# adamjorr/kbbq-py

Measured on AMD Instinct MI355X. Metric: bases/sec recalibrated (2x150 bp), higher is better.
Workload: dtype u8

## Files before the change

include/kbbq_hip.h:

```cpp
#ifndef KBBQ_HIP_H
#define KBBQ_HIP_H

#include <stddef.h>
#include <stdint.h>

#ifdef __cplusplus
extern "C" {
#endif

#define KBBQ_OK          0
#define KBBQ_E_HIP      -1
#define KBBQ_E_INDEX    -2
#define KBBQ_E_TYPE     -3
#define KBBQ_E_ARG      -4
#define KBBQ_E_RANGE    -5
#define KBBQ_E_NAME     -6
#define KBBQ_E_LUT      -7
#define KBBQ_E_MEANQ    -8
#define KBBQ_E_FULL     -9

#define KBBQ_APPLY_CHECKED 0
#define KBBQ_APPLY_FAST    1

#define KBBQ_NQ         43
// ... 131 lines not shown
                           uint8_t* d_flagplane, int R, int minscore, int dinuc_minscore, int64_t* d_tables);
int kbbq_count_q_dev(kbbq_ctx* ctx, const uint8_t* d_qual, const uint8_t* d_err, const uint8_t* d_skip,
                     const uint32_t* d_len, int64_t nreads, int pitch, int qoffset, int64_t* d_counts512);
#define KBBQ_CONFUSION_MAX_BASES 4294967295ull
int kbbq_flag_confusion_dev(kbbq_ctx* ctx, const uint8_t* d_qual, const uint8_t* d_truth, const uint8_t* d_kflags,
                            const uint32_t* d_len, int64_t nreads, int pitch, int qoffset, int64_t* d_counts1536);

int    kbbq_pair_pitch(int S2);
size_t kbbq_pair_lut_bytes(int R, int Qt, int S2);
int    kbbq_pack_pairs_dev(kbbq_ctx* ctx, const uint8_t* d_seq, const uint8_t* d_cseq, const uint8_t* d_qual,
                           const uint32_t* d_meta, int64_t npairs, int pitch, int S2,
                           uint8_t* d_pseq, uint8_t* d_pcseq, uint8_t* d_pqual, uint32_t* d_pmeta);
int    kbbq_unpack_pairs_dev(kbbq_ctx* ctx, const uint8_t* d_pplane, int64_t npairs, int S2, int pitch, uint8_t* d_plane);
int    kbbq_accumulate_pairs_dev(kbbq_ctx* ctx, const uint8_t* d_pseq, const uint8_t* d_pcseq, const uint8_t* d_pqual,
                                 const uint32_t* d_pmeta, int64_t npairs, int R, int S2, int minscore,
                                 int dinuc_minscore, int64_t* d_tables);
int    kbbq_pair_lut_dev(kbbq_ctx* ctx, const void* d_lut_blob, int R, int S2, int minscore, void* d_pair_lut);
int    kbbq_pair_lut_rows_dev(kbbq_ctx* ctx, const void* d_lut_blob, int R, int S2, int minscore, int flags, void* d_pair_lut);
int    kbbq_apply_pairs_dev(kbbq_ctx* ctx, const uint8_t* d_pseq, const uint8_t* d_pqual, const uint32_t* d_pmeta,
                            int64_t npairs, int R, int S2, int minscore, const void* d_lut_blob,
                            const void* d_pair_lut, uint8_t* d_pout);

int    kbbq_accumulate_grouped_dev(kbbq_ctx* ctx, const uint8_t* d_seq, const uint8_t* d_cseq, const uint8_t* d_qual,
                                   const uint32_t* d_meta, int64_t nrows, int pitch, int pairs, int R, int S2,
                                   int S_band, int S_min, int minscore, int dinuc_minscore, const int64_t* d_seg,
                                   int64_t* d_tables);
int    kbbq_apply_grouped_dev(kbbq_ctx* ctx, const uint8_t* d_seq, const uint8_t* d_qual, const uint32_t* d_meta,
                              int64_t nrows, int pitch, int pairs, int R, int S2, int minscore,
                              const void* d_lut_blob, const void* d_pair_lut, const int64_t* d_seg, uint8_t* d_out);

#define KBBQ_ROWS_PAIRS    1
#define KBBQ_ROWS_NIBBLES  2
#define KBBQ_ROWS_TWINS    4
int    kbbq_accumulate_rows_dev(kbbq_ctx* ctx, const uint8_t* d_seq, const uint8_t* d_cseq, const uint8_t* d_qual,
                                const uint32_t* d_meta, int64_t nrows, int pitch, int flags, int R, int S2, int S_band,
                                int S_min, int minscore, int dinuc_minscore, const int64_t* d_seg, int64_t* d_tables);
int    kbbq_apply_rows_dev(kbbq_ctx* ctx, const uint8_t* d_seq, const uint8_t* d_qual, const uint32_t* d_meta, int64_t nrows,
                           int pitch, int flags, int R, int S2, int minscore, const void* d_lut_blob, const void* d_pair_lut,
                           const int64_t* d_seg, const int64_t* d_perm, uint8_t* d_out);
int    kbbq_meta_stats_dev(kbbq_ctx* ctx, const uint32_t* d_meta, int64_t nreads, int32_t* h_stats8);
typedef struct kbbq_band {
    const uint8_t* d_seq; const uint8_t* d_cseq; const uint8_t* d_qual; const uint32_t* d_meta;
    int64_t nrows; int32_t pitch; int32_t flags;
    int32_t S_band; int32_t S_min;
    const int64_t* d_seg; const int64_t* d_perm;
    uint8_t* d_out; const void* d_pair_lut;
} kbbq_band;
int    kbbq_accumulate_bands_dev(kbbq_ctx* ctx, const kbbq_band* bands, int nbands, int R, int S2, int minscore,
                                 int dinuc_minscore, int64_t* d_tables);
int    kbbq_apply_bands_dev(kbbq_ctx* ctx, const kbbq_band* bands, int nbands, int R, int S2, int minscore, const void* d_lut_blob);
size_t kbbq_group_rows_work_bytes(int64_t nrows, int R);
int    kbbq_group_rows_dev(kbbq_ctx* ctx, const uint32_t* d_meta, int64_t nrows, int pairs, int R, void* d_work,
                           int64_t* d_perm, int64_t* d_seg);
int    kbbq_lay_out_dev(kbbq_ctx* ctx, const uint8_t* d_seq, const uint8_t* d_cseq, const uint8_t* d_qual,
                        const uint32_t* d_meta, int64_t nreads, int pitch, int flags, int S2, const int64_t* d_perm,
                        uint8_t* d_lseq, uint8_t* d_lcseq, uint8_t* d_lqual, uint32_t* d_lmeta);
int    kbbq_unpack_nibbles_dev(kbbq_ctx* ctx, const uint8_t* d_nib, int64_t nbases, uint8_t* d_chars);
int    kbbq_tables_add_dev(kbbq_ctx* ctx, int64_t* d_dst, const int64_t* d_src, size_t n);

#define KBBQ_COMM_ID_BYTES 128
typedef struct kbbq_comm kbbq_comm;
int kbbq_comm_library(const char* path);
int kbbq_comm_unique_id(void* id128);
int kbbq_comm_create(kbbq_ctx* ctx, const void* id128, int nranks, int rank, kbbq_comm** out);
int kbbq_allreduce_tables(kbbq_comm* comm, int64_t* d_buf, size_t n);
int kbbq_comm_destroy(kbbq_comm* comm);
// ... 200 lines not shown
```

kbbq-py_amd/csrc/fastq_host.cpp:

```cpp
#include "../../include/kbbq_hip.h"
#include "host_threads.h"
#include "bam_host.h"
#include "fastq_host.h"

#include <algorithm>
#include <atomic>
#include <mutex>
#include <cstdio>
#include <cstdlib>
#include <cstring>
#include <string>
#include <thread>
#include <unordered_map>
#include <vector>

#include <fcntl.h>
#include <sys/mman.h>
#include <sys/stat.h>
#include <unistd.h>
#include <zlib.h>
#if defined(__x86_64__)
#include <immintrin.h>
#endif

// ... 645 lines not shown
    const unsigned nt = nthreads_for((size_t)nrows * 64);
    const int64_t per = (nrows + nt - 1) / std::max(nt, 1u);
    std::vector<std::vector<int64_t>> cnt(nt, std::vector<int64_t>((size_t)R, 0));
    std::atomic<int> bad(0);
    auto key = [&](int64_t i) { return (int)((meta[pairs ? 2 * i : i] >> 16) & 0x7FFFu); };
    auto over = [&](auto body) {
        kbbq_parallel(nt, [&](unsigned t) {
            const int64_t lo = std::min<int64_t>(nrows, (int64_t)t * per), hi = std::min<int64_t>(nrows, lo + per);
            body(t, lo, hi);
        });
    };
    over([&](unsigned t, int64_t lo, int64_t hi) {
        auto& c = cnt[t];
        for (int64_t i = lo; i < hi; ++i) { const int k = key(i); if (k >= R) { bad = 1; continue; } ++c[(size_t)k]; }
    });
    if (bad.load()) return kbbq_set_error_(KBBQ_E_RANGE, "kbbq_group_rows_host: a row carries a read group >= R");
    int64_t run = 0;
    for (int g = 0; g < R; ++g) {
        seg[g] = run;
        for (unsigned t = 0; t < nt; ++t) { const int64_t c = cnt[t][(size_t)g]; cnt[t][(size_t)g] = run; run += c; }
    }
    seg[R] = nrows;
    over([&](unsigned t, int64_t lo, int64_t hi) {
        auto& c = cnt[t];
        for (int64_t i = lo; i < hi; ++i) perm[c[(size_t)key(i)]++] = i;
    });
    return KBBQ_OK;
}

int kbbq_fastq_fill_rows(const kbbq_fastq* a, const kbbq_fastq* b, int64_t first, int64_t n, const uint32_t* meta, int flags,
                         int S2, int pitch, const int64_t* perm, int64_t row_lo, int64_t nrows,
                         uint8_t* seq, uint8_t* cseq, uint8_t* qual, uint32_t* dmeta, int* foreign)
{
    if (!a || (nrows > 0 && (!seq || !qual || !dmeta || !meta || (b && !cseq)))) return kbbq_set_error_(KBBQ_E_ARG, "kbbq_fastq_fill_rows: NULL argument");
    if (first < 0 || n < 0 || first + n > (int64_t)a->h0.size() || (b && first + n > (int64_t)b->h0.size()))
        return kbbq_set_error_(KBBQ_E_ARG, "kbbq_fastq_fill_rows: range out of bounds");
    if (flags & ~(KBBQ_ROWS_PAIRS | KBBQ_ROWS_NIBBLES | KBBQ_ROWS_TWINS)) return kbbq_set_error_(KBBQ_E_ARG, "kbbq_fastq_fill_rows: unknown layout flags");
    const bool pairs = (flags & KBBQ_ROWS_PAIRS) != 0, nib = (flags & KBBQ_ROWS_NIBBLES) != 0;
    const int S = S2 / 2;
    if (pairs) {
        if (S2 <= 0 || (S2 & 1) || S2 > 65534) return kbbq_set_error_(KBBQ_E_ARG, "kbbq_fastq_fill_rows: S2 must be positive and even");
        pitch = (S2 + 1 + 15) & ~15;
    }
    if (pitch <= 0 || (pitch & 15)) return kbbq_set_error_(KBBQ_E_ARG, "kbbq_fastq_fill_rows: pitch must be a positive multiple of 16");
    const int64_t total = pairs ? (n + 1) / 2 : n;
    if (row_lo < 0 || nrows < 0 || row_lo + nrows > total) return kbbq_set_error_(KBBQ_E_ARG, "kbbq_fastq_fill_rows: rows out of bounds");
    const size_t sp = nib ? (size_t)pitch / 2 : (size_t)pitch;
    std::atomic<int> bad(0); std::atomic<unsigned> odd(0);
    parallel_for(nrows, nthreads_for((size_t)nrows * (size_t)pitch * 3), [&](int64_t lo, int64_t hi) {
        std::vector<uint8_t> tmp(nib ? (size_t)pitch : 0);
        unsigned foreign_here = 0;
        for (int64_t row = lo; row < hi; ++row) {
            const int64_t s = perm ? perm[row_lo + row] : row_lo + row;
            if (s < 0 || s >= total) { bad = 3; continue; }
            uint8_t* q = qual + (size_t)row * pitch;
            uint8_t* planes[2] = {seq + (size_t)row * sp, b ? cseq + (size_t)row * sp : nullptr};
            const kbbq_fastq* src[2] = {a, b};
            if (pairs) {
                const int64_t i1 = first + 2 * s; const bool lone = 2 * s + 1 >= n; const int64_t i2 = lone ? i1 : i1 + 1;
                if ((int)a->slen[i1] != S || (int)a->slen[i2] != S || (b && ((int)b->slen[i1] != S || (int)b->slen[i2] != S))) { bad = 1; continue; }
                memcpy(q, a->buf + a->q0[i1], (size_t)S);
                if (lone) memset(q + S, 0, (size_t)(pitch - S));
                else { q[S] = 0; memcpy(q + S + 1, a->buf + a->q0[i2], (size_t)S); memset(q + 2 * S + 1, 0, (size_t)(pitch - 2 * S - 1)); }
                for (int pl = 0; pl < 2; ++pl) {
                    if (!planes[pl]) continue;
                    uint8_t* c = nib ? tmp.data() : planes[pl];
                    memcpy(c, src[pl]->buf + src[pl]->s0[i1], (size_t)S);
                    if (lone) memset(c + S, 'N', (size_t)(pitch - S));
                    else { c[S] = 'N'; memcpy(c + S + 1, src[pl]->buf + src[pl]->s0[i2], (size_t)S); memset(c + 2 * S + 1, 'N', (size_t)(pitch - 2 * S - 1)); }
                    if (nib) foreign_here |= pack_row(c, pitch, planes[pl]);
                }
                dmeta[row] = (uint32_t)(2 * S + 1) | (meta[2 * s] & 0x7FFF0000u);
            } else {
                const int64_t i = first + s;
                const uint32_t L = a->slen[i];
                if ((int)L > pitch || (b && b->slen[i] != L)) { bad = 1; continue; }
                memcpy(q, a->buf + a->q0[i], L); memset(q + L, 0, (size_t)pitch - L);
                for (int pl = 0; pl < 2; ++pl) {
                    if (!planes[pl]) continue;
                    uint8_t* c = nib ? tmp.data() : planes[pl];
                    memcpy(c, src[pl]->buf + src[pl]->s0[i], L); memset(c + L, 'N', (size_t)pitch - L);
                    if (nib) foreign_here |= pack_row(c, pitch, planes[pl]);
                }
                dmeta[row] = meta[s];
            }
        }
        if (foreign_here) odd = 1;
    });
    if (bad.load()) return kbbq_set_error_(KBBQ_E_ARG, bad.load() == 3 ? "kbbq_fastq_fill_rows: perm holds a row out of range"
                                                      : "kbbq_fastq_fill_rows: a read does not fit the layout (lengths differ from what the statistics said)");
    if (odd.load() && foreign) *foreign = 1;
    return KBBQ_OK;
}

int64_t kbbq_fastq_format(const kbbq_fastq* a, int64_t first, int64_t n, int pitch, const uint8_t* newqual,
                          char* out, int64_t cap)
{
    return kbbq_fastq_format_rows(a, first, n, 0, 0, pitch, newqual, out, cap);
}

int64_t kbbq_fastq_format_rows(const kbbq_fastq* a, int64_t first, int64_t n, int flags, int S2, int pitch,
                               const uint8_t* newqual, char* out, int64_t cap)
{
    if (!a || first < 0 || n < 0 || first + n > (int64_t)a->h0.size()) { kbbq_set_error_(KBBQ_E_ARG, "kbbq_fastq_format: bad range"); return 0; }
// ... 27 lines not shown
```

kbbq-py_amd/csrc/kbbq_hip.hip:

```cpp
#include "kbbq_kernels.h"
#include "kbbq_kernels_v3.h"
#include "kbbq_k2_tile.h"
#include "kbbq_solve_kernels.h"
#include "kbbq_lut_kernels.h"
#include "kbbq_aligned_kernels.h"
#include "kbbq_layout_kernels.h"
#include "kbbq_apply_aligned.h"
#include "kbbq_kmer.h"
#include "kbbq_kmer_set.h"
#include "kbbq_bgzf.h"
#include "kbbq_bam_out.h"
#include "../../include/kbbq_hip.h"
#include "host_threads.h"

#include <rocprim/rocprim.hpp>

#include <algorithm>
#include <climits>
#include <cstdint>
#include <cstdarg>
#include <cstdio>
#include <cstring>
#include <functional>
#include <string>
// ... 32 lines not shown
    hipStream_t own_stream = nullptr;
    hipStream_t stream = nullptr;
    u64* d_status = nullptr;
    int* d_stats = nullptr;
    DevScratch wgplan;
    DevScratch ops4;
    DevScratch tally;
    DevScratch rowlut;
    DevScratch bgzf_tok;
    DevScratch bgzf_off;
    DevScratch bgzf_blocks;
    DevScratch bam_words;
    void* stage_host[2] = {nullptr, nullptr}; void* stage_dev[2] = {nullptr, nullptr}; size_t stage_bytes = 0;
    hipStream_t stage_stream = nullptr;
    hipStream_t stage_down_stream = nullptr;
    hipEvent_t stage_up[2] = {nullptr, nullptr}, stage_used[2] = {nullptr, nullptr}, stage_down[2] = {nullptr, nullptr};
    bool timing = false;
    std::vector<std::pair<hipEvent_t, hipEvent_t>> ev[2];
    double ms_acc[2] = {0.0, 0.0};
    int64_t launches[2] = {0, 0};
};

#define KBBQ_NSTATUS 8

constexpr size_t K2T_ROW_LUT_MAX = 52 << 10;
constexpr int K2V3_FRONTS = 8;
constexpr int K2T_XCD_TILES = 1;
constexpr int K2T_XCD = 8;
constexpr int K7_FRONTS = 8;
constexpr int TALLY_K4_SHARE = 8;
static const u64 ST_INIT[KBBQ_NSTATUS] = {~0ull, ~0ull, ~0ull, ~0ull, ~0ull, ~0ull, ~0ull, ~0ull};

enum K1Form { K1_ROWS, K1_ALIGNED, K1_ALIGNED_REF, K1_BANDS };
struct K1Variant { K1Form form; int dn, nib, kj; const void* kernel[2]; };
#define K1_SPLITS(K, ...) {(const void*)(K<false, __VA_ARGS__>), (const void*)(K<true, __VA_ARGS__>)}
static const K1Variant K1_VARIANTS[] = {
    {K1_ROWS, K1V3_DNREP, 0, 0, K1_SPLITS(k1v3_accumulate, K1V3_DNREP)},
    {K1_ROWS, 8, 0, 0, K1_SPLITS(k1v3_accumulate, 8)},
    {K1_ROWS, K1V3_DNREP, 1, 0, K1_SPLITS(k1v3_accumulate, K1V3_DNREP, true)},
    {K1_ROWS, 8, 1, 0, K1_SPLITS(k1v3_accumulate, 8, true)},
    {K1_ROWS, K1V3_DNREP, 1, 13, K1_SPLITS(k1v3_accumulate, K1V3_DNREP, true, 13)},
    {K1_ROWS, K1V3_DNREP, 1, 19, K1_SPLITS(k1v3_accumulate, K1V3_DNREP, true, 19)},
    {K1_ALIGNED, K1V3_DNREP, 0, 0, K1_SPLITS(k1v3_aligned, K1V3_DNREP)},
    {K1_ALIGNED, 8, 0, 0, K1_SPLITS(k1v3_aligned, 8)},
    {K1_ALIGNED_REF, K1V3_DNREP, 0, 0, K1_SPLITS(k1v3_aligned_ref, K1V3_DNREP)},
    {K1_ALIGNED_REF, 8, 0, 0, K1_SPLITS(k1v3_aligned_ref, 8)},
    {K1_BANDS, 0, 0, 0, K1_SPLITS(k1v3_bands, false)},
    {K1_BANDS, 0, 1, 0, K1_SPLITS(k1v3_bands, true)},
};
#undef K1_SPLITS

static const void* k1_kernel(K1Form form, bool split, int dn, int nib, int kj)
{
    for (const K1Variant& v : K1_VARIANTS)
        if (v.form == form && v.dn == dn && v.nib == nib && v.kj == kj) return v.kernel[split];
    return nullptr;
}

enum LdsKernel { LK_K1_PLAIN, LK_K1_PLAIN_SPLIT, LK_K1_TILED, LK_K1_TILED_SPLIT, LK_K2V3, LK_K2V3_NIB, LK_K2T, LK_K2T_NIB, LK_K2T_BANDS, LK_K2T_PAIR19, LK_K2T_PAIR13, LK_K2_LDS16, LK_K2_LDS8, LK_BGZF, LK_COUNT };
static const void* const LDS_KERNELS[LK_COUNT] = {
    (const void*)k1_accumulate<false>, (const void*)k1_accumulate<true>,
    (const void*)k1_accumulate_tiled<false>, (const void*)k1_accumulate_tiled<true>,
    (const void*)k2v3_apply<false>, (const void*)k2v3_apply<true>,
    (const void*)k2t_apply<false>, (const void*)k2t_apply<true>, (const void*)k2t_bands,
    (const void*)k2t_apply_pair<19>, (const void*)k2t_apply_pair<13>,
    (const void*)k2_apply<int16_t, true, true>, (const void*)k2_apply<int8_t, true, false>,
    (const void*)bz_deflate,
};

extern "C" {

int kbbq_abi_version(void) { return KBBQ_ABI_VERSION; }
const char* kbbq_last_error(void) { return g_err.c_str(); }

int kbbq_device_count(int* count)
{
    int n = 0;
    hipError_t e = hipGetDeviceCount(&n);
    if (e != hipSuccess) { *count = 0; return fail(KBBQ_E_HIP, "hipGetDeviceCount: %s", hipGetErrorString(e)); }
    *count = n;
    return KBBQ_OK;
}

int kbbq_bind_host_to_device(int device, int* numa_node, int* ncpus)
{
    char busid[64] = {0};
    HIPCHK(hipDeviceGetPCIBusId(busid, (int)sizeof busid, device));
    return kbbq_bind_host_to_pci(busid, numa_node, ncpus);
}

int kbbq_ctx_create(int device, kbbq_ctx** out)
{
    if (!out) return fail(KBBQ_E_ARG, "kbbq_ctx_create: out is NULL");
    *out = nullptr;
    const bool dbg = getenv("KBBQ_CTX_DBG") != nullptr;
    auto t_prev = std::chrono::steady_clock::now();
    auto lap = [&](const char* what) {
        if (!dbg) return;
// ... 297 lines not shown
};

static int launch_lds(kbbq_ctx* c, int which, const void* kernel, dim3 grid, dim3 block, size_t lds, const void* params)
{
    if (!kernel) return fail(KBBQ_E_HIP, "libkbbq_hip has no instance of K1 for this launch (K1_VARIANTS)");
    void* args[] = {const_cast<void*>(params)};
    {
        Timed t(c, which);
        (void)hipLaunchKernel(kernel, grid, block, args, lds, c->stream);
    }
    HIPCHK(hipGetLastError());
    return KBBQ_OK;
}

static int grow_scratch(kbbq_ctx* c, DevScratch& s, size_t need)
{
    if (s.bytes >= need) return KBBQ_OK;
    if (s.p) { HIPCHK(hipStreamSynchronize(c->stream)); (void)hipFree(s.p); s.p = nullptr; s.bytes = 0; }
    HIPCHK(hipMalloc(&s.p, need));
    s.bytes = need;
    return KBBQ_OK;
}

extern "C" {

int kbbq_accumulate_dev(kbbq_ctx* c, const uint8_t* d_seq, const uint8_t* d_cseq,
                        const uint8_t* d_qual, const uint32_t* d_meta,
                        int64_t nreads, int pitch, int R, int S2, int minscore, int64_t* d_tables)
{
    return kbbq_accumulate_ex_dev(c, d_seq, d_cseq, d_qual, d_meta, nreads, pitch, R, S2,
                                  minscore, minscore, d_tables);
}

struct K1Setup { K1v3Params q; int dn = 0; int kj = 0; size_t lds = 0; };
static int accumulate_rows(kbbq_ctx* c, const char* who, const uint8_t* d_seq, const uint8_t* d_cseq, const uint8_t* d_qual,
                           const uint32_t* d_meta, int64_t nrows, int pitch, int pairs, int R, int S2, int minscore,
                           int dinuc_minscore, const int64_t* d_seg, int64_t* d_tables, bool* fits, int S_band = 0, int S_min = 0, int nib = 0,
                           int twins = 0, K1Setup* setup_only = nullptr);

int kbbq_accumulate_ex_dev(kbbq_ctx* c, const uint8_t* d_seq, const uint8_t* d_cseq,
                           const uint8_t* d_qual, const uint32_t* d_meta,
                           int64_t nreads, int pitch, int R, int S2, int minscore,
                           int dinuc_minscore, int64_t* d_tables)
{
    return kbbq_accumulate_band_dev(c, d_seq, d_cseq, d_qual, d_meta, nreads, pitch, R, S2, 0, 0, minscore, dinuc_minscore, d_tables);
}

int kbbq_accumulate_band_dev(kbbq_ctx* c, const uint8_t* d_seq, const uint8_t* d_cseq,
                             const uint8_t* d_qual, const uint32_t* d_meta,
                             int64_t nreads, int pitch, int R, int S2, int S_band, int S_min, int minscore,
                             int dinuc_minscore, int64_t* d_tables)
{
    if (!c) return fail(KBBQ_E_ARG, "ctx is NULL");
    int rc = check_planes("kbbq_accumulate_dev", nreads, pitch, d_seq, d_cseq, d_qual);
    if (rc) return rc;
    if (R <= 0 || R > 32767) return fail(KBBQ_E_ARG, "kbbq_accumulate_dev: R out of range (%d)", R);
    if (S2 <= 0 || (S2 & 1)) return fail(KBBQ_E_ARG, "kbbq_accumulate_dev: S2 must be positive and even (%d)", S2);
    if (minscore < 0 || minscore > KQ - 1) return fail(KBBQ_E_ARG, "kbbq_accumulate_dev: minscore out of range (%d)", minscore);
    if (dinuc_minscore < 0 || dinuc_minscore > 222) return fail(KBBQ_E_ARG, "kbbq_accumulate_dev: dinuc_minscore out of range (%d)", dinuc_minscore);
    if (nreads == 0) return KBBQ_OK;
    HIPCHK(hipSetDevice(c->device));

    const int64_t nblocks = (nreads + 63) / 64;
    const bool split = dinuc_minscore > minscore;
    bool fits = false;
    rc = accumulate_rows(c, "kbbq_accumulate_dev", d_seq, d_cseq, d_qual, d_meta, nreads, pitch, 0, R, S2, minscore,
                         dinuc_minscore, nullptr, d_tables, &fits, S_band, S_min);
    if (rc || fits) return rc;
    K1Params p;
    p.seq = d_seq; p.cseq = d_cseq; p.qual = d_qual; p.meta = d_meta;
    p.nreads = nreads; p.pitch = pitch; p.cpr = pitch / 16; p.cpr_magic = magic_for(p.cpr);
// ... 120 lines not shown
    return true;
}

static bool k2_tile_serves(const kbbq_ctx* c, int pairs, int nib, int R, bool grouped, int cpr, size_t rg_bytes)
{
    if (env_is("KBBQ_K2_TILE", "0") || (!nib && env_is("KBBQ_K2_TILE_CHARS", "0"))) return false;
    if ((R != 1 && !grouped) || cpr < 2 || cpr > 4096) return false;
    return pairs ? rg_bytes * 3 <= (size_t)c->lds_bytes : rg_bytes <= K2T_ROW_LUT_MAX;
}

static K2v3Params k2v3_params(kbbq_ctx* c, const uint8_t* d_seq, const uint8_t* d_qual, const uint32_t* d_meta, int64_t nrows, int pitch,
                              int pairs, int R, int Qt, int S2, int Sb, int minscore, const void* d_lut_blob, const void* d_pair_lut,
                              const int64_t* d_seg, const int64_t* d_perm, uint8_t* d_out)
{
    K2v3Params q;
    q.seq = d_seq; q.qual = d_qual; q.meta = d_meta; q.nreads = nrows; q.pitch = pitch;
    q.cpr = pitch / 16; q.cpr_magic = magic_for(q.cpr);
    q.R = R; q.Qt = Qt; q.S2 = S2; q.minscore = minscore; q.qlo = 33u + (u32)minscore;
    q.lut16 = reinterpret_cast<const int16_t*>(d_lut_blob); q.rs16 = lut_row_stride(S2);
    q.full = pairs ? reinterpret_cast<const int8_t*>(d_pair_lut)
                   : reinterpret_cast<const int8_t*>(d_lut_blob) + lut_full_offset(R, Qt, S2);
    q.rb = (u32)(pairs ? pair_lut_row_bytes(S2) : full_lut_row_bytes(Sb));
    q.full_bytes = (int)((size_t)R * (33 + Qt) * q.rb);
    if (pairs) { q.W = 0u; q.ctx_off = (u32)pair_pitch(S2); q.maxlen = S2 + 1; }
    else { q.W = (u32)full_lut_width(Sb); q.ctx_off = 2u * q.W; q.maxlen = Sb; }
    q.pairs = pairs; q.seg = reinterpret_cast<const long long*>(d_seg);
    q.perm = reinterpret_cast<const long long*>(d_perm);
    q.parts = K2V3_FRONTS;
    q.rpb = 64;
    q.out = d_out; q.status = c->d_status;
    return q;
}

static int launch_k2v3(kbbq_ctx* c, const K2v3Params& q, int nib)
{
    const int slices = q.seg ? q.R : 1;
    const size_t lds = (size_t)(33 + q.Qt) * q.rb * (size_t)(q.seg ? 1 : q.R);
    const int per_cu = std::max(1, std::min<int>((int)(c->lds_bytes / lds), (K2V3_WAVES * 4 * 64) / K2V3_THREADS));
    const int64_t nblocks = (q.nreads + q.rpb - 1) / q.rpb;
    const int64_t want = (nblocks + (K2V3_THREADS / 64) - 1) / (K2V3_THREADS / 64);
    const int gx = (int)std::min<int64_t>(want, std::max<int64_t>(1, (int64_t)c->cus * per_cu / slices));
    return launch_lds(c, 1, LDS_KERNELS[nib ? LK_K2V3_NIB : LK_K2V3], dim3((unsigned)std::max(gx, 1), (unsigned)slices, 1), dim3(K2V3_THREADS), lds, &q);
}

static int apply_rows(kbbq_ctx* c, const char* who, const uint8_t* d_seq, const uint8_t* d_qual, const uint32_t* d_meta,
                      int64_t nrows, int pitch, int pairs, int R, int S2, int minscore, const void* d_lut_blob,
                      const void* d_pair_lut, const int64_t* d_seg, uint8_t* d_out, int nib = 0, const int64_t* d_perm = nullptr);

int kbbq_apply_dev(kbbq_ctx* c, const uint8_t* d_seq, const uint8_t* d_qual, const uint32_t* d_meta,
                   int64_t nreads, int pitch, int R, int Qt, int S2, int minscore,
                   const void* d_lut, int mode, uint8_t* d_out)
{
    if (!c) return fail(KBBQ_E_ARG, "ctx is NULL");
    int rc = check_planes("kbbq_apply_dev", nreads, pitch, d_seq, d_qual, d_out);
    if (rc) return rc;
    if (R <= 0 || R > 32767 || Qt <= 0 || Qt > 95 || S2 <= 0 || S2 > 65536)
        return fail(KBBQ_E_ARG, "kbbq_apply_dev: bad table shape R=%d Qt=%d S2=%d (Qt <= 95)", R, Qt, S2);
    if (minscore < 0 || minscore > 222) return fail(KBBQ_E_ARG, "kbbq_apply_dev: minscore out of range");
    if ((uintptr_t)d_lut & 15) return fail(KBBQ_E_ARG, "kbbq_apply_dev: LUT must be 16-byte aligned");
    if (mode != KBBQ_APPLY_CHECKED && mode != KBBQ_APPLY_FAST) return fail(KBBQ_E_ARG, "kbbq_apply_dev: bad mode %d", mode);
    if (nreads == 0) return KBBQ_OK;
    HIPCHK(hipSetDevice(c->device));
    const int64_t nblocks = (nreads + 63) / 64;

    const int Sb = row_lut_width(pitch, S2);
    const size_t full_bytes = (size_t)R * (33 + Qt) * full_lut_row_bytes(Sb);
    if (mode == KBBQ_APPLY_FAST && R == 1 && Qt == KQ && !(S2 & 1) && S2 <= 65534
        && k2_tile_serves(c, 0, 0, R, false, pitch / 16, (size_t)(33 + KQ) * full_lut_row_bytes(Sb)))
        return apply_rows(c, "kbbq_apply_dev", d_seq, d_qual, d_meta, nreads, pitch, 0, R, S2, minscore, d_lut, nullptr, nullptr, d_out, 0, nullptr);
    if (mode == KBBQ_APPLY_FAST && full_bytes <= (size_t)c->lds_bytes) {
        K2v3Params q = k2v3_params(c, d_seq, d_qual, d_meta, nreads, pitch, 0, R, Qt, S2, Sb, minscore, d_lut, nullptr, nullptr, nullptr, d_out);
        if (!narrowed_row_lut(c, d_lut, R, Qt, S2, Sb, minscore, &q.full)) return fail(KBBQ_E_HIP, "kbbq_apply_dev: no scratch for the narrowed LUT");
        return launch_k2v3(c, q, 0);
    }

    K2Params p;
    p.seq = d_seq; p.qual = d_qual; p.meta = d_meta; p.nreads = nreads; p.pitch = pitch;
    p.cpr = pitch / 16; p.cpr_magic = magic_for(p.cpr);
    p.R = R; p.Qt = Qt; p.S2 = S2; p.minscore = minscore; p.qlo = 33u + (u32)minscore;
    p.lut = reinterpret_cast<const int16_t*>(d_lut); p.lut_count = (int)kbbq_lut_count(R, Qt, S2);
// ... 230 lines not shown
    auto bytes_for = [&](int nt, int pc) {
        const size_t rows = (size_t)q.nrows - 1 + nt;
        return rows * 128 * dn + (size_t)pc * (rows * q.row_bytes + q.slack_bytes);
    };
    const char* nt_env = getenv("KBBQ_K1_NTRASH");
    const char* pc_env = getenv("KBBQ_K1_POSCOPIES");
    const int most_t = nt_env ? atoi(nt_env) : 8, most = pc_env ? atoi(pc_env) : 4;
    q.ntrash = 1; q.pos_copies = 1;
    for (int nt = 8; nt >= 2; nt >>= 1)
        if (nt <= most_t && bytes_for(nt, 1) <= (size_t)c->lds_bytes) { q.ntrash = nt; break; }
    if (q.cpr <= 12)
        for (int pc = 4; pc >= 2; pc >>= 1)
            if (pc <= most && bytes_for(q.ntrash, pc) <= (size_t)c->lds_bytes) { q.pos_copies = pc; break; }
    q.pos_copy_bytes = (u32)((size_t)(q.nrows - 1 + q.ntrash) * q.row_bytes + q.slack_bytes);
    return bytes_for(q.ntrash, q.pos_copies);
}

static bool k1_geometry(K1v3Params& q, const kbbq_ctx* c, int copies, int cut, int minlen)
{
    q.row_bytes = (u32)((3 * q.S - cut) | 1) * 4u;
    q.minlen = minlen;
    q.slack_bytes = (u32)(q.S + 32) * 4u;
    q.dn_flush_iters = std::max(1, 65535 / ((K1V3_THREADS / copies) * 16 * q.cpr));
    const size_t lds = (size_t)q.nrows * 128 * copies + (size_t)q.nrows * q.row_bytes + q.slack_bytes;
    return lds <= (size_t)c->lds_bytes && (K1V3_THREADS / copies) * 16 * q.cpr <= 65535;
}

static bool k1_split(const K1v3Params& q) { return q.type_minscore > q.minscore; }
static int64_t k1_iters(const K1v3Params& q) { return ((q.nreads + 63) / 64 + (K1V3_THREADS / 64) - 1) / (K1V3_THREADS / 64); }

static int launch_k1(kbbq_ctx* c, K1Form form, const K1Setup& su, int nib)
{
    const int gx = (int)std::min<int64_t>(k1_iters(su.q), std::max(1, c->cus / su.q.R));
    return launch_lds(c, 0, k1_kernel(form, k1_split(su.q), su.dn, nib, su.kj), dim3((unsigned)gx, (unsigned)su.q.R, 1), dim3(K1V3_THREADS),
                      su.lds, &su.q);
}

static int accumulate_rows(kbbq_ctx* c, const char* who, const uint8_t* d_seq, const uint8_t* d_cseq, const uint8_t* d_qual,
                           const uint32_t* d_meta, int64_t nrows, int pitch, int pairs, int R, int S2, int minscore,
                           int dinuc_minscore, const int64_t* d_seg, int64_t* d_tables, bool* fits, int S_band, int S_min, int nib, int twins,
                           K1Setup* setup_only)
{
    if (fits) *fits = true;
    if (S_band < 0 || S_band > S2 / 2 || (pairs && S_band)) return fail(KBBQ_E_ARG, "%s: S_band out of range (%d)", who, S_band);
    if (S_min < 0 || S_min > (S_band ? S_band : S2 / 2)) return fail(KBBQ_E_ARG, "%s: S_min out of range (%d)", who, S_min);
    int rc = check_planes(who, nrows, pitch, d_seq, d_cseq, d_qual);
    if (rc) return rc;
    if (R <= 0 || R > 32767) return fail(KBBQ_E_ARG, "%s: R out of range (%d)", who, R);
    if (S2 <= 0 || (S2 & 1) || S2 > 65534) return fail(KBBQ_E_ARG, "%s: S2 must be positive and even (%d)", who, S2);
    if (minscore < 0 || minscore > KQ - 1) return fail(KBBQ_E_ARG, "%s: minscore out of range (%d)", who, minscore);
    if (dinuc_minscore < 0 || dinuc_minscore > 222) return fail(KBBQ_E_ARG, "%s: dinuc_minscore out of range (%d)", who, dinuc_minscore);
    if (pairs && pitch != pair_pitch(S2)) return fail(KBBQ_E_ARG, "%s: mate-pair rows of %d-base reads have pitch %d, not %d", who, S2 / 2, pair_pitch(S2), pitch);
    if (nrows == 0) return KBBQ_OK;
    HIPCHK(hipSetDevice(c->device));
    const int S = S_band ? S_band : S2 / 2;
    K1Setup su;
    K1v3Params& q = su.q;
    q.aflags = nullptr; q.aclip = nullptr; q.atrim = nullptr;
    q.seq = d_seq; q.cseq = d_cseq; q.qual = d_qual; q.meta = d_meta;
    q.nreads = nrows; q.pitch = pitch; q.cpr = pitch / 16; q.cpr_magic = magic_for(q.cpr);
    q.R = R; q.S = S; q.gS2 = S2; q.minscore = minscore; q.type_minscore = dinuc_minscore;
    q.qlo_m1 = 32u + (u32)minscore; q.dlo = 33u + (u32)dinuc_minscore;
    q.nrows = KQ + 1 - minscore;
    q.maxlen = pairs ? S2 + 1 : S; q.gap = pairs ? 1 : 0; q.twins = (pairs && twins) ? 1 : 0;
    q.seg = reinterpret_cast<const long long*>(d_seg);
    q.tables = reinterpret_cast<u64*>(d_tables); q.status = c->d_status;
    q.genome = nullptr; q.ag0 = nullptr;
    const int trim = (!pairs && S_min > 0) ? std::min(S_min, S) : 0;
    if (pairs && nib && (q.cpr == 19 || q.cpr == 13)) {
        q.row_bytes = (u32)((((16 * q.cpr + 31) & ~31) + 32 * K1V3_DNREP) * 4);
        q.minlen = 0; q.slack_bytes = 0; q.pos_copies = 1;
        q.dn_flush_iters = std::max(1, 65535 / ((K1V3_THREADS / K1V3_DNREP) * 16 * q.cpr));
        for (int nt = q.cpr == 19 ? 1 : 8; nt >= 1 && !su.dn; nt >>= 1) {
            const size_t rows = (size_t)q.nrows - 1 + nt;
            su.lds = rows * q.row_bytes;
            if (su.lds > (size_t)c->lds_bytes) continue;
            su.dn = K1V3_DNREP; su.kj = q.cpr;
            q.ntrash = nt; q.pos_copy_bytes = (u32)(rows * q.row_bytes);
        }
    }
    for (int attempt = 0; attempt < (trim ? 3 : 1) && !su.dn; ++attempt) {
        const int copies = attempt == 2 ? 8 : K1V3_DNREP, cut = attempt ? trim : 0;
        if (k1_geometry(q, c, copies, cut, cut)) su.dn = copies;
    }
    if (!su.dn) {
        if (fits) { *fits = false; return KBBQ_OK; }
        return fail(KBBQ_E_LUT, "%s: %d-base reads with minscore %d do not fit the LDS tables; use plain one-read-per-row planes", who, S, minscore);
    }
    if (!su.kj) su.lds = k1_lds_plan(q, su.dn, c);
    if (setup_only) { *setup_only = su; return KBBQ_OK; }
    return launch_k1(c, K1_ROWS, su, nib);
}

int kbbq_accumulate_pairs_dev(kbbq_ctx* c, const uint8_t* d_pseq, const uint8_t* d_pcseq, const uint8_t* d_pqual,
                              const uint32_t* d_pmeta, int64_t npairs, int R, int S2, int minscore,
                              int dinuc_minscore, int64_t* d_tables)
{
    if (!c) return fail(KBBQ_E_ARG, "ctx is NULL");
    int rc = check_pairs("kbbq_accumulate_pairs_dev", npairs, S2);
    if (rc) return rc;
    return accumulate_rows(c, "kbbq_accumulate_pairs_dev", d_pseq, d_pcseq, d_pqual, d_pmeta, npairs, pair_pitch(S2), 1,
                           R, S2, minscore, dinuc_minscore, nullptr, d_tables, nullptr);
}

int kbbq_accumulate_grouped_dev(kbbq_ctx* c, const uint8_t* d_seq, const uint8_t* d_cseq, const uint8_t* d_qual,
                                const uint32_t* d_meta, int64_t nrows, int pitch, int pairs, int R, int S2, int S_band,
                                int S_min, int minscore, int dinuc_minscore, const int64_t* d_seg, int64_t* d_tables)
{
    if (!c) return fail(KBBQ_E_ARG, "ctx is NULL");
    if (!d_seg) return fail(KBBQ_E_ARG, "kbbq_accumulate_grouped_dev: d_seg is NULL");
    return accumulate_rows(c, "kbbq_accumulate_grouped_dev", d_seq, d_cseq, d_qual, d_meta, nrows, pitch, pairs ? 1 : 0,
                           R, S2, minscore, dinuc_minscore, d_seg, d_tables, nullptr, S_band, S_min);
}

int kbbq_pair_lut_dev(kbbq_ctx* c, const void* d_lut_blob, int R, int S2, int minscore, void* d_pair_lut)
{
    return kbbq_pair_lut_rows_dev(c, d_lut_blob, R, S2, minscore, KBBQ_ROWS_PAIRS, d_pair_lut);
}

int kbbq_pair_lut_rows_dev(kbbq_ctx* c, const void* d_lut_blob, int R, int S2, int minscore, int flags, void* d_pair_lut)
{
    if (!c) return fail(KBBQ_E_ARG, "ctx is NULL");
    int rc = check_pairs("kbbq_pair_lut_dev", 0, S2);
    if (rc) return rc;
    if (!(flags & KBBQ_ROWS_PAIRS) || (flags & ~(KBBQ_ROWS_PAIRS | KBBQ_ROWS_NIBBLES | KBBQ_ROWS_TWINS)))
        return fail(KBBQ_E_ARG, "kbbq_pair_lut_rows_dev: flags 0x%x are not those of mate-pair rows", flags);
    if (R <= 0 || R > 32767 || !d_lut_blob || !d_pair_lut) return fail(KBBQ_E_ARG, "kbbq_pair_lut_dev: bad argument");
    HIPCHK(hipSetDevice(c->device));
    PairLutParams f;
    f.lut16 = reinterpret_cast<const int16_t*>(d_lut_blob); f.rs16 = lut_row_stride(S2); f.R = R; f.Qt = KQ; f.S2 = S2;
    f.minscore = std::min(std::max(minscore, 0), KQ);
    f.twins = (flags & KBBQ_ROWS_TWINS) ? 1 : 0;
    f.out = reinterpret_cast<int8_t*>(d_pair_lut);
    hipLaunchKernelGGL(k3_fill_pair_lut, dim3((unsigned)(R * (33 + KQ))), dim3(256), 0, c->stream, f);
    HIPCHK(hipGetLastError());
    return KBBQ_OK;
}

static K2tParams k2t_params(const K2v3Params& q)
{
    K2tParams t;
    t.seq = q.seq; t.qual = q.qual; t.meta = q.meta; t.nchunks = q.nreads * q.cpr; t.cpr = q.cpr; t.cpr_magic = q.cpr_magic;
    t.Qt = q.Qt; t.S2 = q.S2; t.maxlen = q.maxlen; t.lut = q.full; t.lut_bytes = (int)(((size_t)(33 + q.Qt) * q.rb + 15) & ~(size_t)15);
    t.rb = q.rb; t.ctx_off = q.ctx_off; t.W = q.W; t.seg = q.seg; t.R = q.R; t.wg_start = nullptr; t.order = nullptr;
    t.perm = q.perm; t.pitch = q.pitch; t.out = q.out; t.status = q.status;
    t.xcd_tiles = K2T_XCD_TILES;
    return t;
}

static int apply_rows(kbbq_ctx* c, const char* who, const uint8_t* d_seq, const uint8_t* d_qual, const uint32_t* d_meta,
                      int64_t nrows, int pitch, int pairs, int R, int S2, int minscore, const void* d_lut_blob,
                      const void* d_pair_lut, const int64_t* d_seg, uint8_t* d_out, int nib, const int64_t* d_perm)
{
    int rc = check_planes(who, nrows, pitch, d_seq, d_qual, d_out);
    if (rc) return rc;
    if (R <= 0 || R > 32767 || !d_lut_blob || (pairs && (!d_pair_lut || ((uintptr_t)d_pair_lut & 15)))) return fail(KBBQ_E_ARG, "%s: bad argument", who);
    if (S2 <= 0 || (S2 & 1) || S2 > 65534) return fail(KBBQ_E_ARG, "%s: S2 must be positive and even (%d)", who, S2);
    if (minscore < 0 || minscore > 222) return fail(KBBQ_E_ARG, "%s: minscore out of range", who);
    if (pairs && pitch != pair_pitch(S2)) return fail(KBBQ_E_ARG, "%s: mate-pair rows of %d-base reads have pitch %d, not %d", who, S2 / 2, pair_pitch(S2), pitch);
    const int Sb = pairs ? S2 : row_lut_width(pitch, S2);
    K2v3Params q = k2v3_params(c, d_seq, d_qual, d_meta, nrows, pitch, pairs, R, KQ, S2, Sb, minscore, d_lut_blob, d_pair_lut, d_seg, d_perm, d_out);
    const size_t rg_bytes = (size_t)(33 + KQ) * q.rb;
    const size_t lds = d_seg ? rg_bytes : rg_bytes * (size_t)R;
    if (lds > (size_t)c->lds_bytes)
        return fail(KBBQ_E_LUT, "%s: the apply LUT (%zu B) does not fit the LDS; group the rows by read group or use kbbq_apply_dev", who, lds);
    if (nrows == 0) return KBBQ_OK;
    HIPCHK(hipSetDevice(c->device));
    if (!pairs && !narrowed_row_lut(c, d_lut_blob, R, KQ, S2, Sb, minscore, &q.full)) return fail(KBBQ_E_HIP, "%s: no scratch for the narrowed LUT", who);
    if (!k2_tile_serves(c, pairs, nib, R, d_seg != nullptr, q.cpr, rg_bytes)) return launch_k2v3(c, q, nib);

    K2tParams t = k2t_params(q);
    const int64_t per_wg = (int64_t)(K2T_THREADS / 64) * 64 * K2T_STEPS;
    int64_t gt = (t.nchunks + per_wg - 1) / per_wg;
    if (d_seg) {
        gt += R;
        const bool interleave = d_perm && R > 1;
        const int64_t ints = (int64_t)(R + 1) + 1 + (interleave ? 2 * gt : 0);
        if (ints > 0x7FFFFFFF) return fail(KBBQ_E_ARG, "%s: too many workgroups", who);
        rc = grow_scratch(c, c->wgplan, (size_t)ints * sizeof(int));
        if (rc) return rc;
        int* wg_start = reinterpret_cast<int*>(c->wgplan.p);
        K2tPlanParams pl; pl.seg = t.seg; pl.R = R; pl.cpr = q.cpr; pl.wg_start = wg_start;
        hipLaunchKernelGGL(k2t_plan, dim3(1), dim3(64), 0, c->stream, pl);
        t.wg_start = wg_start;
        if (interleave) {
            K2tOrderParams op; op.wg_start = wg_start; op.R = R;
            op.xcd = K2T_XCD;
            op.order = reinterpret_cast<int2*>(wg_start + ((R + 2) & ~1));
            hipLaunchKernelGGL(k2t_order, dim3((unsigned)((gt + 255) / 256)), dim3(256), 0, c->stream, op);
            t.order = op.order;
        }
    }
    const int kj = (pairs && nib) ? k2t_pair_form(t) : 0;
    if (kj < 0) return fail(KBBQ_E_ARG, "%s: mate-pair rows of %d chunks do not have the geometry k2t_apply_pair was compiled for", who, q.cpr);
    const LdsKernel k = kj == 19 ? LK_K2T_PAIR19 : kj == 13 ? LK_K2T_PAIR13 : nib ? LK_K2T_NIB : LK_K2T;
    return launch_lds(c, 1, LDS_KERNELS[k], dim3((unsigned)gt), dim3(K2T_THREADS), (size_t)t.lut_bytes, &t);
}

int kbbq_apply_pairs_dev(kbbq_ctx* c, const uint8_t* d_pseq, const uint8_t* d_pqual, const uint32_t* d_pmeta,
                         int64_t npairs, int R, int S2, int minscore, const void* d_lut_blob, const void* d_pair_lut,
                         uint8_t* d_pout)
{
    if (!c) return fail(KBBQ_E_ARG, "ctx is NULL");
    int rc = check_pairs("kbbq_apply_pairs_dev", npairs, S2);
    if (rc) return rc;
    return apply_rows(c, "kbbq_apply_pairs_dev", d_pseq, d_pqual, d_pmeta, npairs, pair_pitch(S2), 1, R, S2, minscore,
                      d_lut_blob, d_pair_lut, nullptr, d_pout);
}

int kbbq_apply_grouped_dev(kbbq_ctx* c, const uint8_t* d_seq, const uint8_t* d_qual, const uint32_t* d_meta,
                           int64_t nrows, int pitch, int pairs, int R, int S2, int minscore, const void* d_lut_blob,
                           const void* d_pair_lut, const int64_t* d_seg, uint8_t* d_out)
{
    if (!c) return fail(KBBQ_E_ARG, "ctx is NULL");
    if (!d_seg) return fail(KBBQ_E_ARG, "kbbq_apply_grouped_dev: d_seg is NULL");
    return apply_rows(c, "kbbq_apply_grouped_dev", d_seq, d_qual, d_meta, nrows, pitch, pairs ? 1 : 0, R, S2, minscore,
                      d_lut_blob, d_pair_lut, d_seg, d_out);
}


static int layout_flags_ok(const char* who, int flags)
{
    if (flags & ~(KBBQ_ROWS_PAIRS | KBBQ_ROWS_NIBBLES | KBBQ_ROWS_TWINS)) return fail(KBBQ_E_ARG, "%s: unknown layout flags 0x%x", who, flags);
    if ((flags & KBBQ_ROWS_TWINS) && !(flags & KBBQ_ROWS_PAIRS)) return fail(KBBQ_E_ARG, "%s: KBBQ_ROWS_TWINS describes mate-pair rows (add KBBQ_ROWS_PAIRS)", who);
    return KBBQ_OK;
}

int kbbq_accumulate_rows_dev(kbbq_ctx* c, const uint8_t* d_seq, const uint8_t* d_cseq, const uint8_t* d_qual,
                             const uint32_t* d_meta, int64_t nrows, int pitch, int flags, int R, int S2, int S_band,
                             int S_min, int minscore, int dinuc_minscore, const int64_t* d_seg, int64_t* d_tables)
{
    if (!c) return fail(KBBQ_E_ARG, "ctx is NULL");
    int rc = layout_flags_ok("kbbq_accumulate_rows_dev", flags);
    if (rc) return rc;
    const int pairs = (flags & KBBQ_ROWS_PAIRS) ? 1 : 0;
    if (pairs) { rc = check_pairs("kbbq_accumulate_rows_dev", nrows, S2); if (rc) return rc; }
    return accumulate_rows(c, "kbbq_accumulate_rows_dev", d_seq, d_cseq, d_qual, d_meta, nrows, pitch, pairs, R, S2, minscore,
                           dinuc_minscore, d_seg, d_tables, nullptr, pairs ? 0 : S_band, pairs ? 0 : S_min,
                           (flags & KBBQ_ROWS_NIBBLES) ? 1 : 0, (flags & KBBQ_ROWS_TWINS) ? 1 : 0);
}

int kbbq_apply_rows_dev(kbbq_ctx* c, const uint8_t* d_seq, const uint8_t* d_qual, const uint32_t* d_meta, int64_t nrows,
                        int pitch, int flags, int R, int S2, int minscore, const void* d_lut_blob, const void* d_pair_lut,
                        const int64_t* d_seg, const int64_t* d_perm, uint8_t* d_out)
{
    if (!c) return fail(KBBQ_E_ARG, "ctx is NULL");
    int rc = layout_flags_ok("kbbq_apply_rows_dev", flags);
    if (rc) return rc;
    const int pairs = (flags & KBBQ_ROWS_PAIRS) ? 1 : 0;
    if (pairs) { rc = check_pairs("kbbq_apply_rows_dev", nrows, S2); if (rc) return rc; }
    return apply_rows(c, "kbbq_apply_rows_dev", d_seq, d_qual, d_meta, nrows, pitch, pairs, R, S2, minscore, d_lut_blob,
                      d_pair_lut, d_seg, d_out, (flags & KBBQ_ROWS_NIBBLES) ? 1 : 0, d_perm);
}

static int band_accumulate_alone(kbbq_ctx* c, const kbbq_band& b, int R, int S2, int minscore, int dinuc_minscore, int64_t* d_tables)
{
    if (b.flags || b.d_seg)
        return kbbq_accumulate_rows_dev(c, b.d_seq, b.d_cseq, b.d_qual, b.d_meta, b.nrows, b.pitch, b.flags, R, S2, b.S_band, b.S_min,
                                        minscore, dinuc_minscore, b.d_seg, d_tables);
    return kbbq_accumulate_band_dev(c, b.d_seq, b.d_cseq, b.d_qual, b.d_meta, b.nrows, b.pitch, R, S2, b.S_band, b.S_min, minscore,
                                    dinuc_minscore, d_tables);
}

static void share_workgroups(const std::vector<double>& weight, const std::vector<int64_t>& cap, int total, std::vector<int>& out)
{
    const size_t n = weight.size();
    out.assign(n, 1);
    int left = total - (int)n;
    double sum = 0; for (double w : weight) sum += w;
    for (int round = 0; round < 4 && left > 0 && sum > 0; ++round) {
        std::vector<std::pair<double, size_t>> frac;
        int given = 0; double open_sum = 0;
        for (size_t i = 0; i < n; ++i) if (out[i] < cap[i]) open_sum += weight[i];
        if (open_sum <= 0) break;
        const int pool = left;
        for (size_t i = 0; i < n; ++i) {
            if (out[i] >= cap[i]) continue;
            const double want = pool * weight[i] / open_sum;
            int add = (int)std::min<int64_t>((int64_t)want, cap[i] - out[i]);
            out[i] += add; given += add;
            if (out[i] < cap[i]) frac.push_back({want - (int64_t)want, i});
        }
        left -= given;
        std::sort(frac.begin(), frac.end(), [](const auto& a, const auto& b) { return a.first > b.first; });
        for (auto& f : frac) { if (left <= 0) break; if (out[f.second] < cap[f.second]) { ++out[f.second]; --left; } }
    }
}

int kbbq_accumulate_bands_dev(kbbq_ctx* c, const kbbq_band* bands, int nbands, int R, int S2, int minscore, int dinuc_minscore,
                              int64_t* d_tables)
{
    if (!c) return fail(KBBQ_E_ARG, "ctx is NULL");
    if (nbands < 0 || (nbands > 0 && !bands)) return fail(KBBQ_E_ARG, "kbbq_accumulate_bands_dev: bad band list");
    std::vector<K1Setup> setups; std::vector<int> merged, alone;
    const bool merge = !env_is("KBBQ_K1_BANDS", "0");
    int nib_of_merge = -1;
    for (int i = 0; i < nbands; ++i) {
        const kbbq_band& b = bands[i];
        if (b.nrows == 0) continue;
        int rc = layout_flags_ok("kbbq_accumulate_bands_dev", b.flags);
        if (rc) return rc;
        const int pairs = (b.flags & KBBQ_ROWS_PAIRS) ? 1 : 0, nib = (b.flags & KBBQ_ROWS_NIBBLES) ? 1 : 0;
        K1Setup su; bool fits = false;
        bool can = merge && (int)merged.size() < K1V3_MAX_BANDS;
        if (can) {
            if (pairs) { rc = check_pairs("kbbq_accumulate_bands_dev", b.nrows, S2); if (rc) return rc; }
            rc = accumulate_rows(c, "kbbq_accumulate_bands_dev", b.d_seq, b.d_cseq, b.d_qual, b.d_meta, b.nrows, b.pitch, pairs, R, S2, minscore,
                                 dinuc_minscore, b.d_seg, d_tables, &fits, pairs ? 0 : b.S_band, pairs ? 0 : b.S_min, nib,
                                 (b.flags & KBBQ_ROWS_TWINS) ? 1 : 0, &su);
            if (rc) return rc;
            can = fits && !su.kj && (nib_of_merge < 0 || nib_of_merge == nib);
        }
        if (can) { nib_of_merge = nib; merged.push_back(i); setups.push_back(su); }
        else alone.push_back(i);
    }
    const int G = std::max(1, c->cus / std::max(R, 1));
    if (merged.size() < 2 || (int)merged.size() > G) { for (int i : merged) alone.push_back(i); merged.clear(); }
    for (int i : alone) {
        int rc = band_accumulate_alone(c, bands[i], R, S2, minscore, dinuc_minscore, d_tables);
        if (rc) return rc;
    }
    HIPCHK(hipSetDevice(c->device));
    if (merged.empty()) return KBBQ_OK;
    constexpr double row_cost = 1.25;
    constexpr double slope = 0.01;
    constexpr double dn8_cost = 1.06;
    K1BandsParams t;
    memset(&t, 0, sizeof t);
    t.nbands = (int)merged.size();
    std::vector<double> weight; std::vector<int64_t> cap; std::vector<int> share;
    size_t lds = 0;
    for (const K1Setup& su : setups) {
        weight.push_back((double)su.q.nreads * (su.q.cpr + row_cost) * (1.0 + slope * su.q.cpr) * (su.dn == K1V3_DNREP ? 1.0 : dn8_cost));
        cap.push_back(std::max<int64_t>(1, k1_iters(su.q)));
        lds = std::max(lds, su.lds);
    }
    share_workgroups(weight, cap, G, share);
    int run = 0;
    for (size_t j = 0; j < setups.size(); ++j) {
        t.wg_start[j] = run; run += share[j];
        t.dn[j] = setups[j].dn; t.band[j] = setups[j].q;
    }
// ... 9 lines not shown
        HIPCHK(hipMemcpy(h.data(), dbg, h.size() * sizeof h[0], hipMemcpyDeviceToHost));
        (void)hipFree(dbg);
        unsigned long long t0 = ~0ull;
        for (int w = 0; w < run; ++w) t0 = std::min(t0, h[(size_t)w]);
        for (int j = 0; j < t.nbands; ++j) {
            unsigned long long s1 = 0, e0 = ~0ull, e1 = 0;
            for (int w = t.wg_start[j]; w < t.wg_start[j + 1]; ++w) {
                s1 = std::max(s1, h[(size_t)w] - t0); e0 = std::min(e0, h[(size_t)run + w] - t0); e1 = std::max(e1, h[(size_t)run + w] - t0);
            }
            fprintf(stderr, "[k1v3_bands] band %d pitch %3d rows %9lld: %3d workgroups, last start %7.1f us, ends %7.1f .. %7.1f us\n", j, t.band[j].pitch,
                    (long long)t.band[j].nreads, t.wg_start[j + 1] - t.wg_start[j], s1 / 100.0, e0 / 100.0, e1 / 100.0);
        }
    }
    return KBBQ_OK;
}

static int band_apply_alone(kbbq_ctx* c, const kbbq_band& b, int R, int S2, int minscore, const void* d_lut_blob)
{
    if (b.flags || b.d_seg)
        return kbbq_apply_rows_dev(c, b.d_seq, b.d_qual, b.d_meta, b.nrows, b.pitch, b.flags, R, S2, minscore, d_lut_blob, b.d_pair_lut,
                                   b.d_seg, b.d_perm, b.d_out);
    return kbbq_apply_dev(c, b.d_seq, b.d_qual, b.d_meta, b.nrows, b.pitch, R, KQ, S2, minscore, d_lut_blob, KBBQ_APPLY_FAST, b.d_out);
}

int kbbq_apply_bands_dev(kbbq_ctx* c, const kbbq_band* bands, int nbands, int R, int S2, int minscore, const void* d_lut_blob)
{
    if (!c) return fail(KBBQ_E_ARG, "ctx is NULL");
    if (nbands < 0 || (nbands > 0 && !bands) || !d_lut_blob) return fail(KBBQ_E_ARG, "kbbq_apply_bands_dev: bad argument");
    if (R <= 0 || R > 32767 || S2 <= 0 || (S2 & 1) || S2 > 65534 || minscore < 0 || minscore > 222) return fail(KBBQ_E_ARG, "kbbq_apply_bands_dev: bad shape");
    std::vector<int> merged, alone;
    for (int i = 0; i < nbands; ++i) {
        const kbbq_band& b = bands[i];
        if (b.nrows == 0) continue;
        int rc = layout_flags_ok("kbbq_apply_bands_dev", b.flags);
        if (rc) return rc;
        const int Sb = std::min(b.pitch, S2);
        const bool can = (int)merged.size() < K2T_MAX_BANDS && R == 1
                         && b.flags == KBBQ_ROWS_NIBBLES && !b.d_seg && !b.d_perm && b.pitch > 0 && !(b.pitch & 15)
                         && k2_tile_serves(c, 0, 1, R, false, b.pitch / 16, (size_t)(33 + KQ) * full_lut_row_bytes(Sb))
                         && !(((uintptr_t)b.d_seq | (uintptr_t)b.d_qual | (uintptr_t)b.d_out) & 15) && b.d_seq && b.d_qual && b.d_meta && b.d_out;
        (can ? merged : alone).push_back(i);
    }
    if (merged.size() < 2) { for (int i : merged) alone.push_back(i); merged.clear(); }
    for (int i : alone) {
        int rc = band_apply_alone(c, bands[i], R, S2, minscore, d_lut_blob);
        if (rc) return rc;
    }
    if (merged.empty()) return KBBQ_OK;
    HIPCHK(hipSetDevice(c->device));
    std::vector<size_t> lut_off; size_t need = 0;
    for (int i : merged) { lut_off.push_back(need); need += ((size_t)R * (33 + KQ) * full_lut_row_bytes(std::min(bands[i].pitch, S2)) + 255) & ~(size_t)255; }
    int rc = grow_scratch(c, c->rowlut, need);
    if (rc) return rc;
    K2tBandsParams t;
    memset(&t, 0, sizeof t);
    t.nbands = (int)merged.size();
    const int64_t per_wg = (int64_t)(K2T_THREADS / 64) * 64 * K2T_STEPS;
    int64_t run = 0; size_t lds = 0;
    for (size_t k = 0; k < merged.size(); ++k) {
        const kbbq_band& b = bands[merged[k]];
        const int Sb = std::min(b.pitch, S2);
        K2v3Params rows = k2v3_params(c, b.d_seq, b.d_qual, b.d_meta, b.nrows, b.pitch, 0, R, KQ, S2, Sb, minscore, d_lut_blob, nullptr, nullptr, nullptr, b.d_out);
        rows.full = fill_row_lut(c, d_lut_blob, R, KQ, S2, Sb, minscore, reinterpret_cast<char*>(c->rowlut.p) + lut_off[k]);
        const K2tParams& q = t.band[k] = k2t_params(rows);
        lds = std::max(lds, (size_t)q.lut_bytes);
        t.wg_start[k] = (int)run;
        run += (q.nchunks + per_wg - 1) / per_wg;
// ... 26 lines not shown
size_t kbbq_group_rows_work_bytes(int64_t nrows, int R)
{
    const int64_t nblocks = (nrows + K7_SORT_ROWS - 1) / K7_SORT_ROWS;
    return (size_t)std::max<int64_t>(nblocks, 1) * (size_t)std::max(R, 1) * sizeof(u32);
}

int kbbq_group_rows_dev(kbbq_ctx* c, const uint32_t* d_meta, int64_t nrows, int pairs, int R, void* d_work,
                        int64_t* d_perm, int64_t* d_seg)
{
    if (!c) return fail(KBBQ_E_ARG, "ctx is NULL");
    if (nrows < 0 || nrows >= (1ll << 32)) return fail(KBBQ_E_ARG, "kbbq_group_rows_dev: nrows out of range");
    if (R <= 0 || R > K7_SORT_MAXR) return fail(KBBQ_E_ARG, "kbbq_group_rows_dev: 1 <= R <= %d (got %d)", K7_SORT_MAXR, R);
    if (!d_meta || !d_work || !d_perm || !d_seg) return fail(KBBQ_E_ARG, "kbbq_group_rows_dev: NULL pointer");
    HIPCHK(hipSetDevice(c->device));
    if (nrows == 0) { HIPCHK(hipMemsetAsync(d_seg, 0, (size_t)(R + 1) * 8, c->stream)); return KBBQ_OK; }
    RgSortParams p;
    p.meta = d_meta; p.nrows = nrows; p.pairs = pairs ? 1 : 0; p.R = R;
    p.nblocks = (nrows + K7_SORT_ROWS - 1) / K7_SORT_ROWS;
    p.hist = reinterpret_cast<u32*>(d_work); p.perm = reinterpret_cast<long long*>(d_perm); p.status = c->d_status;
    hipLaunchKernelGGL(k7_rg_sort<false>, dim3((unsigned)p.nblocks), dim3(K7_SORT_THREADS), 0, c->stream, p);
    RgScanParams s;
    s.hist = p.hist; s.count = p.nblocks * R; s.nblocks = p.nblocks; s.R = R; s.nrows = nrows; s.seg = reinterpret_cast<long long*>(d_seg);
    hipLaunchKernelGGL(k7_rg_scan, dim3(1), dim3(1024), 0, c->stream, s);
    hipLaunchKernelGGL(k7_rg_sort<true>, dim3((unsigned)p.nblocks), dim3(K7_SORT_THREADS), 0, c->stream, p);
    HIPCHK(hipGetLastError());
    return KBBQ_OK;
}

int kbbq_lay_out_dev(kbbq_ctx* c, const uint8_t* d_seq, const uint8_t* d_cseq, const uint8_t* d_qual, const uint32_t* d_meta,
                     int64_t nreads, int pitch, int flags, int S2, const int64_t* d_perm,
                     uint8_t* d_lseq, uint8_t* d_lcseq, uint8_t* d_lqual, uint32_t* d_lmeta)
{
    if (!c) return fail(KBBQ_E_ARG, "ctx is NULL");
    int rc = layout_flags_ok("kbbq_lay_out_dev", flags);
    if (rc) return rc;
    const int pairs = (flags & KBBQ_ROWS_PAIRS) ? 1 : 0, nib = (flags & KBBQ_ROWS_NIBBLES) ? 1 : 0;
    rc = check_planes("kbbq_lay_out_dev", nreads, pitch, d_seq, d_cseq, d_qual);
    if (rc) return rc;
    if (!d_seq || !d_qual || !d_meta || !d_lseq || !d_lqual || !d_lmeta || (d_cseq && !d_lcseq)) return fail(KBBQ_E_ARG, "kbbq_lay_out_dev: NULL pointer");
    if (((uintptr_t)d_lseq | (uintptr_t)d_lcseq | (uintptr_t)d_lqual) & 15) return fail(KBBQ_E_ARG, "kbbq_lay_out_dev: planes must be 16-byte aligned");
    if (pairs) {
        rc = check_pairs("kbbq_lay_out_dev", (nreads + 1) / 2, S2);
        if (rc) return rc;
        if ((nreads & 1) && !(flags & KBBQ_ROWS_TWINS)) return fail(KBBQ_E_ARG, "kbbq_lay_out_dev: mate-pair rows need an even number of reads");
        if (pitch < S2 / 2) return fail(KBBQ_E_ARG, "kbbq_lay_out_dev: pitch %d < read length %d", pitch, S2 / 2);
    }
    if (nreads == 0) return KBBQ_OK;
    HIPCHK(hipSetDevice(c->device));
    LayOutParams p;
    p.src[0] = d_seq; p.src[1] = d_cseq; p.src[2] = d_qual; p.dst[0] = d_lseq; p.dst[1] = d_lcseq; p.dst[2] = d_lqual;
    p.meta = d_meta; p.dmeta = d_lmeta; p.perm = reinterpret_cast<const long long*>(d_perm);
    p.nrows = pairs ? (nreads + 1) / 2 : nreads; p.nsrc = nreads; p.pitch = pitch; p.dpitch = pairs ? pair_pitch(S2) : pitch; p.S = pairs ? S2 / 2 : 0;
    p.pairs = pairs; p.nib = nib; p.status = c->d_status;
    const int rpb7 = (p.dpitch / 16) <= 256 ? 256 / (p.dpitch / 16) : 1;
    const int gx = bounded_grid((p.nrows + rpb7 - 1) / rpb7, c, 256);
    p.parts = K7_FRONTS;
    hipLaunchKernelGGL(k7_lay_out, dim3((unsigned)std::max(gx, 1)), dim3(256), 0, c->stream, p);
    HIPCHK(hipGetLastError());
    return KBBQ_OK;
}

int kbbq_tables_add_dev(kbbq_ctx* c, int64_t* d_dst, const int64_t* d_src, size_t n)
{
    if (!c) return fail(KBBQ_E_ARG, "ctx is NULL");
    if (n && (!d_dst || !d_src)) return fail(KBBQ_E_ARG, "kbbq_tables_add_dev: NULL pointer");
    if (n == 0) return KBBQ_OK;
    HIPCHK(hipSetDevice(c->device));
    AddTablesParams p; p.dst = (long long*)d_dst; p.src = (const long long*)d_src; p.n = (long long)n;
    int gx = (int)std::min<size_t>((n + 255) / 256, (size_t)c->cus * 8);
    hipLaunchKernelGGL(k7_add_tables, dim3((unsigned)std::max(gx, 1)), dim3(256), 0, c->stream, p);
    HIPCHK(hipGetLastError());
    return KBBQ_OK;
}

int kbbq_unpack_nibbles_dev(kbbq_ctx* c, const uint8_t* d_nib, int64_t nbases, uint8_t* d_chars)
{
    if (!c) return fail(KBBQ_E_ARG, "ctx is NULL");
    if (nbases < 0 || (nbases & 15) || ((uintptr_t)d_nib & 7) || ((uintptr_t)d_chars & 15)) return fail(KBBQ_E_ARG, "kbbq_unpack_nibbles_dev: bad size or alignment");
    if (nbases == 0) return KBBQ_OK;
    HIPCHK(hipSetDevice(c->device));
    UnNibParams p; p.src = d_nib; p.dst = d_chars; p.nchunks = nbases / 16;
    int gx = (int)std::min<int64_t>((p.nchunks + 255) / 256, (int64_t)c->cus * 16);
    hipLaunchKernelGGL(k7_unpack_nibbles, dim3((unsigned)std::max(gx, 1)), dim3(256), 0, c->stream, p);
    HIPCHK(hipGetLastError());
    return KBBQ_OK;
}
// ... 39 lines not shown
    const K4Params p = k4_params(c, d_seq, d_len, nreads, pitch, d_ref_start, d_ref_len, d_cig_off, d_cig_n, d_cigar, d_genome, d_skipmask,
                                 genome_len, d_flip, d_err, d_skip);
    if (((uintptr_t)d_seq | (uintptr_t)d_err | (uintptr_t)d_skip) & 15)
        return fail(KBBQ_E_ARG, "kbbq_find_errors_dev: planes must be 16-byte aligned");
    const int rpb4 = (pitch / 16) <= 256 ? 256 / (pitch / 16) : 1;
    const int gx = bounded_grid((nreads + rpb4 - 1) / rpb4, c, 64);
    int rc4 = k4_records(c, p, nullptr, nullptr, nullptr, nullptr, 0);
    if (rc4) return rc4;
    K4v2Params q; q.base = p; q.recs = (const K4Rec*)c->ops4.p; q.idle16 = reinterpret_cast<const uint8_t*>(c->d_status);
    q.rows = nullptr; q.nrows = nullptr;
    if (d_skipmask) hipLaunchKernelGGL(k4v2_find_errors<false>, dim3((unsigned)std::max(gx, 1)), dim3(256), 0, c->stream, q);
    else hipLaunchKernelGGL(k4v2_find_errors<true>, dim3((unsigned)std::max(gx, 1)), dim3(256), 0, c->stream, q);
    HIPCHK(hipGetLastError());
    return KBBQ_OK;
}

int kbbq_canonical_reads_dev(kbbq_ctx* c, const uint8_t* d_seq, const uint8_t* d_oq, const uint8_t* d_err,
                             const uint8_t* d_skip, const uint32_t* d_len, const uint32_t* d_clip,
                             const uint32_t* d_trim, const uint32_t* d_flags, int64_t nreads, int pitch, int S,
                             int minscore, int dinuc_minscore, uint8_t* d_out_seq, uint8_t* d_out_cseq,
                             uint8_t* d_out_qual, uint32_t* d_out_meta)
{
    return kbbq_canonical_reads_rows_dev(c, d_seq, d_oq, d_err, d_skip, d_len, d_clip, d_trim, d_flags, nreads, pitch, S,
                                         minscore, dinuc_minscore, 0, d_out_seq, d_out_cseq, d_out_qual, d_out_meta);
}

int kbbq_canonical_reads_rows_dev(kbbq_ctx* c, const uint8_t* d_seq, const uint8_t* d_oq, const uint8_t* d_err,
                                  const uint8_t* d_skip, const uint32_t* d_len, const uint32_t* d_clip,
                                  const uint32_t* d_trim, const uint32_t* d_flags, int64_t nreads, int pitch, int S,
                                  int minscore, int dinuc_minscore, int layout, uint8_t* d_out_seq, uint8_t* d_out_cseq,
                                  uint8_t* d_out_qual, uint32_t* d_out_meta)
{
    if (!c) return fail(KBBQ_E_ARG, "ctx is NULL");
    if (layout & ~KBBQ_ROWS_NIBBLES) return fail(KBBQ_E_ARG, "kbbq_canonical_reads_rows_dev: the output is one read per row (layout 0 or KBBQ_ROWS_NIBBLES)");
    if (nreads < 0 || pitch <= 0 || (pitch & 15) || S <= 0 || S > pitch || S > 65535)
        return fail(KBBQ_E_ARG, "kbbq_canonical_reads_dev: bad nreads/pitch/S");
    if (minscore < 0 || minscore > 94 || dinuc_minscore < 0 || dinuc_minscore > 94)
        return fail(KBBQ_E_ARG, "kbbq_canonical_reads_dev: minscore out of range");
    if (nreads == 0) return KBBQ_OK;
    if (!d_seq || !d_oq || !d_err) return fail(KBBQ_E_ARG, "kbbq_canonical_reads_dev: NULL plane");
    if (((uintptr_t)d_seq | (uintptr_t)d_oq | (uintptr_t)d_err | (uintptr_t)d_skip | (uintptr_t)d_out_seq
         | (uintptr_t)d_out_cseq | (uintptr_t)d_out_qual) & 15)
        return fail(KBBQ_E_ARG, "kbbq_canonical_reads_dev: planes must be 16-byte aligned");
    HIPCHK(hipSetDevice(c->device));
    K6Params p;
    p.seq = d_seq; p.oq = d_oq; p.err = d_err; p.skip = d_skip; p.len = d_len; p.clip = d_clip; p.trim = d_trim;
    p.flags = d_flags; p.nreads = nreads; p.pitch = pitch; p.S = S;
    p.qlo = 33u + (u32)minscore; p.dlo = 33u + (u32)dinuc_minscore;
    p.out_seq = d_out_seq; p.out_cseq = d_out_cseq; p.out_qual = d_out_qual; p.out_meta = d_out_meta;
    p.status = c->d_status;
    const int rpb6 = (pitch / 16) <= 256 ? 256 / (pitch / 16) : 1;
    const int gx = bounded_grid((nreads + rpb6 - 1) / rpb6, c, 64);
    if (layout & KBBQ_ROWS_NIBBLES) hipLaunchKernelGGL(k6_canonical_reads<true>, dim3((unsigned)std::max(gx, 1)), dim3(256), 0, c->stream, p);
    else hipLaunchKernelGGL(k6_canonical_reads<false>, dim3((unsigned)std::max(gx, 1)), dim3(256), 0, c->stream, p);
    HIPCHK(hipGetLastError());
    return KBBQ_OK;
}

static int accumulate_aligned(kbbq_ctx* c, const uint8_t* d_seq, const uint8_t* d_oq, const uint8_t* d_flagplane,
                              const uint32_t* d_clip, const uint32_t* d_trim, const uint32_t* d_flags, int64_t nreads,
                              int pitch, int S, int R, int minscore, int dinuc_minscore, int64_t* d_tables,
                              const uint8_t* d_genome, const int64_t* d_g0, bool dry_run = false)
{
    if (!c) return fail(KBBQ_E_ARG, "ctx is NULL");
    int rc = check_planes("kbbq_accumulate_aligned_dev", nreads, pitch, d_seq, d_oq, d_flagplane);
    if (rc) return rc;
// ... 1429 lines not shown
```

kbbq-py_amd/csrc/kbbq_k2_tile.h:

```cpp
#pragma once
#include "kbbq_kernels_v3.h"
#include <type_traits>

#define K2T_THREADS 1024
#define K2T_STEPS 4

struct K2tParams {
    const uint8_t* seq; const uint8_t* qual; const u32* meta;
    int xcd_tiles;
    long long nchunks;
    int cpr; u32 cpr_magic;
    int Qt; int S2; int maxlen;
    const int8_t* lut; int lut_bytes; u32 rb; u32 ctx_off;
    u32 W;
    const long long* seg;
    const int* wg_start;
    const int2* order;
    int R;
    const long long* perm;
    int pitch;
    uint8_t* out; u64* status;
};

struct K2tPlanParams { const long long* seg; int R; int cpr; int* wg_start; };
// ... 194 lines not shown
}
static inline int k2t_pair_form(const K2tParams& t)
{
    if (t.cpr == 19) return k2t_pair_geometry<19>(t) ? 19 : -1;
    if (t.cpr == 13) return k2t_pair_geometry<13>(t) ? 13 : -1;
    return 0;
}

template <int B> __device__ __forceinline__ u32 k2t_mul24_byte(u32 w, u32 k)
{
    u32 r;
    if constexpr (B == 0) asm("v_mul_u32_u24_sdwa %0, %1, %2 dst_sel:DWORD dst_unused:UNUSED_PAD src0_sel:BYTE_0 src1_sel:DWORD" : "=v"(r) : "v"(w), "v"(k));
    else if constexpr (B == 1) asm("v_mul_u32_u24_sdwa %0, %1, %2 dst_sel:DWORD dst_unused:UNUSED_PAD src0_sel:BYTE_1 src1_sel:DWORD" : "=v"(r) : "v"(w), "v"(k));
    else if constexpr (B == 2) asm("v_mul_u32_u24_sdwa %0, %1, %2 dst_sel:DWORD dst_unused:UNUSED_PAD src0_sel:BYTE_2 src1_sel:DWORD" : "=v"(r) : "v"(w), "v"(k));
    else asm("v_mul_u32_u24_sdwa %0, %1, %2 dst_sel:DWORD dst_unused:UNUSED_PAD src0_sel:BYTE_3 src1_sel:DWORD" : "=v"(r) : "v"(w), "v"(k));
    return r;
}
template <int B> __device__ __forceinline__ u32 k2t_add_byte(u32 a, u32 w)
{
    u32 r;
    if constexpr (B == 0) asm("v_add_u32_sdwa %0, %1, %2 dst_sel:DWORD dst_unused:UNUSED_PAD src0_sel:DWORD src1_sel:BYTE_0" : "=v"(r) : "v"(a), "v"(w));
    else if constexpr (B == 1) asm("v_add_u32_sdwa %0, %1, %2 dst_sel:DWORD dst_unused:UNUSED_PAD src0_sel:DWORD src1_sel:BYTE_1" : "=v"(r) : "v"(a), "v"(w));
    else if constexpr (B == 2) asm("v_add_u32_sdwa %0, %1, %2 dst_sel:DWORD dst_unused:UNUSED_PAD src0_sel:DWORD src1_sel:BYTE_2" : "=v"(r) : "v"(a), "v"(w));
    else asm("v_add_u32_sdwa %0, %1, %2 dst_sel:DWORD dst_unused:UNUSED_PAD src0_sel:DWORD src1_sel:BYTE_3" : "=v"(r) : "v"(a), "v"(w));
    return r;
}
template <class F> __device__ __forceinline__ void k2t_unroll4(F f)
{
    f(std::integral_constant<int, 0>()); f(std::integral_constant<int, 1>()); f(std::integral_constant<int, 2>()); f(std::integral_constant<int, 3>());
}

typedef unsigned short k2t_u16x2 __attribute__((ext_vector_type(2)));

template <int KJ>
__global__ __launch_bounds__(K2T_THREADS) void k2t_apply_pair(K2tParams p)
{
    extern __shared__ __attribute__((aligned(16))) u32 lds[];
    typedef K2tPair<KJ> G;
    const u32 lane = (u32)lane_id();
    const u32 wave = (u32)__builtin_amdgcn_readfirstlane((int)(threadIdx.x >> 6));
    const int bx = (int)blockIdx.x;
    int g = 0;
    long long row_lo = 0, chunk_hi = p.nchunks;
    u32 wg = (u32)bx, tiles = gridDim.x;
    if (p.seg) {
        if (bx >= p.wg_start[p.R]) return;
        if (p.order) {
            const int2 o = p.order[bx];
            g = o.x; wg = (u32)o.y; tiles = 0u;
        } else {
            int lo = 0, hi = p.R;
            while (hi - lo > 1) { const int mid = (lo + hi) >> 1; if (p.wg_start[mid] <= bx) lo = mid; else hi = mid; }
            g = lo;
            wg = (u32)(bx - p.wg_start[g]);
            tiles = (u32)(p.wg_start[g + 1] - p.wg_start[g]);
        }
        row_lo = p.seg[g]; chunk_hi = p.seg[g + 1] * KJ;
    }
    tiles &= ~7u;
    if (wg < tiles) wg = (wg & 7u) * (tiles >> 3) + (wg >> 3);
    const long long chunk_lo = row_lo * KJ;
    const long long base = chunk_lo + ((long long)wg * (K2T_THREADS / 64) + wave) * (64 * K2T_STEPS);
    const bool has = base < chunk_hi;
    const long long base_c = has ? base : chunk_hi - 1;
    const unsigned long long off0 = (unsigned long long)(base_c - chunk_lo);
    const unsigned long long rowd = off0 / (unsigned)KJ;
    const u32 rem0 = (u32)(off0 - rowd * (unsigned)KJ);
    const long long last = chunk_hi - 1 - base_c;
    const u32 limit = last < 64 * K2T_STEPS - 1 ? (u32)last : (u32)(64 * K2T_STEPS - 1);
    const uint8_t* qbase = p.qual + 16 * base_c;
    const uint8_t* sbase = p.seq + 8 * base_c;
    const u32* mbase = p.meta + (row_lo + (long long)rowd);
    u32 sq[K2T_STEPS][2], ql[K2T_STEPS][4], mk[K2T_STEPS], a16[K2T_STEPS];
#pragma unroll
    for (int s = 0; s < K2T_STEPS; ++s) {
        const u32 d = (u32)(64 * s) + lane;
        const u32 dc = d < limit ? d : limit;
        const uint2 sv = *reinterpret_cast<const uint2*>(sbase + 8u * dc);
        sq[s][0] = sv.x; sq[s][1] = sv.y;
        const uint4 qv = *reinterpret_cast<const uint4*>(qbase + 16u * dc);
        ql[s][0] = qv.x; ql[s][1] = qv.y; ql[s][2] = qv.z; ql[s][3] = qv.w;
        const u32 rel = rem0 + dc;
        const u32 drow = __umulhi(rel, G::MAGIC);
        a16[s] = 16u * (rel - drow * (u32)KJ);
        mk[s] = mbase[drow];
    }
    u32 before = 4u;
    if (base_c > 0) before = (u32)sbase[-1] >> 4;
    {
        const uint4* src = reinterpret_cast<const uint4*>(p.lut + (size_t)g * (size_t)(33 + p.Qt) * p.rb);
        const int n16 = p.lut_bytes >> 4;
        for (int i = threadIdx.x; i < n16; i += K2T_THREADS) reinterpret_cast<uint4*>(lds)[i] = src[i];
        __syncthreads();
    }
    const uint8_t* L = reinterpret_cast<const uint8_t*>(lds);
    const u32 rbv = G::RB;
    const u32 hi_add = (u32)(0x80 - (p.Qt + 33)) * 0x01010101u;
    u32 carry_code = 5u * before;
#pragma unroll
    for (int s = 0; s < K2T_STEPS; ++s) {
        const u32 d = (u32)(64 * s) + lane;
        const bool act0 = has && d <= limit;
        const int len = (int)(mk[s] & 0xFFFFu);
        const int nb = act0 ? len - (int)a16[s] : 0;
        u32 code[4], code5[4], hiq = 0u;
        code[0] = nib_lo(sq[s][0]); code[1] = nib_hi(sq[s][0]); code[2] = nib_lo(sq[s][1]); code[3] = nib_hi(sq[s][1]);
        const u32 badbits = nib_invalid(sq[s][0]) | nib_invalid(sq[s][1]);
#pragma unroll
        for (int wd = 0; wd < 4; ++wd) {
            code5[wd] = (code[wd] << 2) + code[wd];
            hiq |= ((ql[s][wd] & 0x7F7F7F7Fu) + hi_add) | ql[s][wd];
        }
        hiq &= 0x80808080u;
        const u32 last_code5 = code5[3] >> 24;
        u32 prev_code5 = wave_shr1(last_code5, carry_code);
        carry_code = (u32)__builtin_amdgcn_readlane((int)last_code5, 63);
        if (a16[s] == 0u) prev_code5 = 20u;
        if (act0) {
            u32 o[4] = {0u, 0u, 0u, 0u};
            if (nb > 0) {
                const int rg = (int)((mk[s] >> 16) & 0x7FFFu);
                if (hiq != 0u || rg != g || len > p.maxlen || badbits) {
                    flag(p.status, ST_LUT, 0);
                } else {
                    u32 d5[4];
                    u32 pc5 = prev_code5 << 24;
#pragma unroll
                    for (int wd = 0; wd < 4; ++wd) {
                        d5[wd] = __builtin_amdgcn_alignbyte(code5[wd], pc5, 3) + code[wd];
                        pc5 = code5[wd];
                    }
                    k2t_u16x2 cy[8], cx[8];
#pragma unroll
                    for (int wd = 0; wd < 4; ++wd) {
                        k2t_unroll4([&](auto bc) {
                            constexpr int b = decltype(bc)::value;
                            const u32 t = k2t_mul24_byte<b>(ql[s][wd], rbv);
                            cy[2 * wd + (b >> 1)][b & 1] = L[t + a16[s] + (u32)(4 * wd + b)];
                            cx[2 * wd + (b >> 1)][b & 1] = L[k2t_add_byte<b>(t, d5[wd]) + G::CTX];
                        });
// ... 34 lines not shown
```

kbbq-py_amd/csrc/kbbq_kernels_v3.h:

```cpp
#pragma once
#include "kbbq_kernels.h"
#include <type_traits>

#define K1V3_THREADS 1024
#define K1V3_DNREP 16
#define K2V3_THREADS 512
#define K2V3_NBUF 2
#define K2V3_WAVES 4
#define K1V3_FLUSH_ITERS 48

struct K1v3Params {
    const uint8_t* seq; const uint8_t* cseq; const uint8_t* qual; const u32* meta;
    long long nreads; int pitch; int cpr; u32 cpr_magic; int R; int S;
    int minscore;
    int type_minscore;
    u32 qlo_m1;
    u32 dlo;
    int nrows;
    u32 row_bytes;
    u32 slack_bytes;
    int minlen;
    int dn_flush_iters;
    int maxlen;
    int gap;
// ... 36 lines not shown
    else if (B == 1) asm("v_min_u32_sdwa %0, %1, %2 dst_sel:DWORD dst_unused:UNUSED_PAD src0_sel:BYTE_1 src1_sel:DWORD" : "=v"(tq) : "v"(qn), "v"(tcl));
    else if (B == 2) asm("v_min_u32_sdwa %0, %1, %2 dst_sel:DWORD dst_unused:UNUSED_PAD src0_sel:BYTE_2 src1_sel:DWORD" : "=v"(tq) : "v"(qn), "v"(tcl));
    else             asm("v_min_u32_sdwa %0, %1, %2 dst_sel:DWORD dst_unused:UNUSED_PAD src0_sel:BYTE_3 src1_sel:DWORD" : "=v"(tq) : "v"(qn), "v"(tcl));
    return tq;
}
template <int B>
__device__ __forceinline__ void k1_joint_increment(u32& inc, u32 xw, u32 one)
{
    if (B == 0)      asm("v_min_u32_sdwa %0, %1, %2 dst_sel:WORD_1 dst_unused:UNUSED_PRESERVE src0_sel:BYTE_0 src1_sel:DWORD" : "+v"(inc) : "v"(xw), "v"(one));
    else if (B == 1) asm("v_min_u32_sdwa %0, %1, %2 dst_sel:WORD_1 dst_unused:UNUSED_PRESERVE src0_sel:BYTE_1 src1_sel:DWORD" : "+v"(inc) : "v"(xw), "v"(one));
    else if (B == 2) asm("v_min_u32_sdwa %0, %1, %2 dst_sel:WORD_1 dst_unused:UNUSED_PRESERVE src0_sel:BYTE_2 src1_sel:DWORD" : "+v"(inc) : "v"(xw), "v"(one));
    else             asm("v_min_u32_sdwa %0, %1, %2 dst_sel:WORD_1 dst_unused:UNUSED_PRESERVE src0_sel:BYTE_3 src1_sel:DWORD" : "+v"(inc) : "v"(xw), "v"(one));
}
__device__ __forceinline__ u32 k1_shl6_add(u32 x, u32 y)
{
    u32 r;
    asm("v_lshl_add_u32 %0, %1, 6, %2" : "=v"(r) : "v"(x), "v"(y));
    return r;
}
template <int H>
__device__ __forceinline__ u32 k1_joint_delta(u32 a, u32 e)
{
    u32 ad;
    if (H == 0) asm("v_add_u32_sdwa %0, %1, %2 dst_sel:DWORD dst_unused:UNUSED_PAD src0_sel:DWORD src1_sel:WORD_0" : "=v"(ad) : "v"(a), "v"(e));
    else        asm("v_add_u32_sdwa %0, %1, %2 dst_sel:DWORD dst_unused:UNUSED_PAD src0_sel:DWORD src1_sel:WORD_1" : "=v"(ad) : "v"(a), "v"(e));
    return ad;
}


#define NIBM 0x0F0F0F0Fu
__device__ __forceinline__ u32 nib_lo(u32 w) { return w & NIBM; }
__device__ __forceinline__ u32 nib_hi(u32 w) { return (w >> 4) & NIBM; }
__device__ __forceinline__ u32 nib_invalid(u32 w) { return (((w & 0x77777777u) + 0x33333333u) | w) & 0x88888888u; }
__device__ __forceinline__ u32 chars_to_codes(u32 w, u32& bad)
{
    const u32 h = (w >> 1) & 0x07070707u;
    bad |= __builtin_amdgcn_perm(0x4E000000u, 0x47544341u, h) ^ w;
    return __builtin_amdgcn_perm(0x04040404u, 0x02010300u, h);
}
__device__ __forceinline__ u32 codes_to_chars(u32 c) { return __builtin_amdgcn_perm(0x4E4E4E4Eu, 0x43475441u, c & 0x07070707u); }

__device__ __forceinline__ u32 nonzero_bytes(u32 x)
{
    return ((x | ((x & 0x7F7F7F7Fu) + 0x7F7F7F7Fu)) >> 7) & 0x01010101u;
}

__device__ __forceinline__ void load16_any(const uint8_t* base, long long off, u32 out[4])
{
    uint4 v;
    __builtin_memcpy(&v, base + off, 16);
    out[0] = v.x; out[1] = v.y; out[2] = v.z; out[3] = v.w;
}

__device__ __forceinline__ void reverse16(u32 v[4])
{
    const u32 a0 = v[0], a1 = v[1], a2 = v[2], a3 = v[3];
    v[0] = __builtin_amdgcn_perm(0u, a3, 0x00010203u); v[1] = __builtin_amdgcn_perm(0u, a2, 0x00010203u);
    v[2] = __builtin_amdgcn_perm(0u, a1, 0x00010203u); v[3] = __builtin_amdgcn_perm(0u, a0, 0x00010203u);
}

typedef __attribute__((address_space(3))) u32 lds_u32;
typedef u32 u32x4 __attribute__((ext_vector_type(4)));
typedef __attribute__((address_space(3))) u32x4 lds_u32x4;

struct K1Chunk { u32 s[4], c[4], q[4]; u32 mk; u32 off; int k; int j; int nb; u32 fl, clip, trim; int jj; u32 g0lo, g0hi; };

template <bool SPLIT, int DN, bool NIB, int KJ, bool ALN = false, bool REF = false>
__device__ __forceinline__ void k1v3_body(const K1v3Params& p, u32* lds, const int bx, const int gx, const int g)
{
    static_assert(!ALN || (!NIB && KJ == 0), "the aligned-read form reads character planes");
    static_assert(!REF || ALN, "the reference comparison belongs to the aligned-read form");
    constexpr bool JOINT = KJ > 0;
    constexpr int CYC = (16 * KJ + 31) & ~31;
    constexpr u32 JROW = (u32)(CYC + 32 * DN) * 4u;
    static_assert(!JOINT || (NIB && DN == 16), "joint rows: 4-bit planes, 64 bytes per context slot");
    const int ntrash = p.ntrash;
    const int dn_words = JOINT ? 0 : (p.nrows - 1 + ntrash) * 32 * DN;
    const int ncopies = KJ > 0 ? 1 : p.pos_copies;
    const int pos_words = KJ > 0 ? (p.nrows - 1 + ntrash) * (int)(JROW >> 2) : ncopies * (int)(p.pos_copy_bytes >> 2);
    u32* dnt = JOINT ? lds + CYC : lds;
    u32* pos = lds + dn_words;
    for (int i = threadIdx.x; i < dn_words + pos_words; i += blockDim.x) lds[i] = 0u;
    __syncthreads();

    const int lane = lane_id();
    const int wave = __builtin_amdgcn_readfirstlane((int)(threadIdx.x >> 6));
    const int nwaves = blockDim.x >> 6;
    const long long seg_lo = p.seg ? p.seg[g] : 0ll, seg_hi = p.seg ? p.seg[g + 1] : p.nreads;
    const long long nblocks = (seg_hi - seg_lo + 63) >> 6;
    const long long iters = (nblocks + nwaves - 1) / nwaves;
    const int S = p.S, S2 = 2 * p.S;
    const u32 row_bytes = JOINT ? JROW : p.row_bytes;
    const u32 tclamp = 255u - p.qlo_m1;
    const u32 pos_base = (u32)dn_words * 4u - 180u * row_bytes;
    const u32 dnt_row = JOINT ? JROW : 128u * DN;
    const u32 dnt_base = (u32)reinterpret_cast<size_t>(lds) - 180u * dnt_row + 4u * (u32)(lane_id() & (DN - 1)) + (JOINT ? 4u * CYC : 0u);
    int since_flush = 0, since_dn_flush = 0;
    const int lane_k0 = p.cpr == 1 ? lane : (int)__umulhi((u32)lane, p.cpr_magic);
    const int lane_j0 = lane - lane_k0 * p.cpr;
    const int dk1 = 64 / p.cpr, dj1 = 64 - dk1 * p.cpr;
    const int dk2 = 128 / p.cpr, dj2 = 128 - dk2 * p.cpr;

    u64* pos_errs = p.tables;
    u64* pos_total = p.tables + (size_t)p.R * KQ * p.gS2;
// ... 108 lines not shown
                aclip = myread < seg_hi ? p.aclip[myread] : 0u;
                atrim = myread < seg_hi ? p.atrim[myread] : 0u;
                if constexpr (REF) {
                    const long long g0 = myread < seg_hi ? p.ag0[myread] : 0ll;
                    ag0lo = (u32)g0; ag0hi = (u32)((u64)g0 >> 32);
                }
                m = myread < seg_hi ? ((u32)p.S | ((afl >> 16) << 16) | ((afl & 2u) << 30)) : 0u;
            } else if (fed) {
                m = m_next;
            } else {
                m = myread < seg_hi ? p.meta[myread] : 0u;
            }
            ahead = false;
            const bool match = myread < seg_hi && (int)((m >> 16) & 0x7FFFu) == g && (m & 0xFFFFu) != 0u;
            const u64 mask = __ballot(match);
            const int n = __popcll(mask);
            u32 cm = m, coff = (u32)lane;
            if (n != 64 && n > 0) {
                const int rank = __popcll(mask & ((1ull << lane) - 1ull));
                const int dst = match ? rank : 63;
                cm = (u32)__builtin_amdgcn_ds_permute(dst << 2, (int)(match ? m : 0u));
                coff = (u32)__builtin_amdgcn_ds_permute(dst << 2, (int)(match ? (u32)lane : 0u));
                if constexpr (ALN) {
                    afl = (u32)__builtin_amdgcn_ds_permute(dst << 2, (int)(match ? afl : 0u));
                    aclip = (u32)__builtin_amdgcn_ds_permute(dst << 2, (int)(match ? aclip : 0u));
                    atrim = (u32)__builtin_amdgcn_ds_permute(dst << 2, (int)(match ? atrim : 0u));
                    if constexpr (REF) {
                        ag0lo = (u32)__builtin_amdgcn_ds_permute(dst << 2, (int)(match ? ag0lo : 0u));
                        ag0hi = (u32)__builtin_amdgcn_ds_permute(dst << 2, (int)(match ? ag0hi : 0u));
                    }
                }
            }
            const uint8_t* bseq = p.seq + (size_t)read0 * (NIB ? p.pitch >> 1 : p.pitch);
            const uint8_t* bcseq = p.cseq + (size_t)read0 * (NIB ? p.pitch >> 1 : p.pitch);
            const uint8_t* bqual = p.qual + (size_t)read0 * p.pitch;
            const int total = n * p.cpr;
            u32 carry_code = 20u, carry_char = 0u;

            auto advance = [&](K1Chunk& ch, int dk, int dj) {
                const int jj = ch.j + dj;
                const bool wrap = jj >= p.cpr;
                ch.j = wrap ? jj - p.cpr : jj;
                ch.k = ch.k + dk + (wrap ? 1 : 0);
            };
            auto fetch = [&](K1Chunk& ch) {
                const bool act0 = ch.k < n;
                const int k = act0 ? ch.k : 0;
                ch.mk = bperm(cm, k);
                ch.off = n == 64 ? (u32)k : bperm(coff, k);
                ch.nb = act0 ? ((int)(ch.mk & 0xFFFFu) - 16 * ch.j) : 0;
                ch.jj = ch.j;
                if constexpr (ALN) {
                    ch.fl = bperm(afl, k); ch.clip = bperm(aclip, k); ch.trim = bperm(atrim, k);
                    if (ch.fl & 1u) ch.jj = p.cpr - 1 - ch.j;
                    if constexpr (REF) { ch.g0lo = bperm(ag0lo, k); ch.g0hi = bperm(ag0hi, k); }
                }
                const u32 rowoff = ch.nb > 0 ? __umul24(ch.off, (u32)p.pitch) + (u32)(16 * ch.jj) : 0u;
                if constexpr (NIB) {
                    const uint2 sv = *reinterpret_cast<const uint2*>(bseq + (rowoff >> 1));
                    const uint2 cv = *reinterpret_cast<const uint2*>(bcseq + (rowoff >> 1));
                    ch.s[0] = sv.x; ch.s[1] = sv.y; ch.c[0] = cv.x; ch.c[1] = cv.y;
                } else if constexpr (REF) {
                    const uint4 sv = *reinterpret_cast<const uint4*>(bseq + rowoff);
                    const bool inref = ch.nb > 0 && (ch.fl & 4u) != 0u;
                    const long long g0 = (long long)(((u64)ch.g0hi << 32) | (u64)ch.g0lo);
                    const uint8_t* src = inref ? p.genome + g0 + 16 * ch.jj : bcseq + rowoff;
                    load16_any(src, 0, ch.c);
                    ch.s[0] = sv.x; ch.s[1] = sv.y; ch.s[2] = sv.z; ch.s[3] = sv.w;
                } else {
                    const uint4 sv = *reinterpret_cast<const uint4*>(bseq + rowoff);
                    const uint4 cv = *reinterpret_cast<const uint4*>(bcseq + rowoff);
                    ch.s[0] = sv.x; ch.s[1] = sv.y; ch.s[2] = sv.z; ch.s[3] = sv.w;
                    ch.c[0] = cv.x; ch.c[1] = cv.y; ch.c[2] = cv.z; ch.c[3] = cv.w;
                }
                const uint4 qv = *reinterpret_cast<const uint4*>(bqual + rowoff);
                ch.q[0] = qv.x; ch.q[1] = qv.y; ch.q[2] = qv.z; ch.q[3] = qv.w;
            };
            auto process = [&](const K1Chunk& ch) {
                const int j = ch.j, nb = ch.nb;
                const bool act = nb > 0;
                const int len = (int)(ch.mk & 0xFFFFu);
                const bool second = (ch.mk >> 31) != 0u;
                const int pos0 = 16 * j;
                u32 code[4], code5[4], xw[4], qv[4], badbits = 0u, hiq = 0u;
                int c0 = pos0;
                if constexpr (ALN) {
                    const bool rev = (ch.fl & 1u) != 0u;
                    const int qs = (int)(ch.clip & 0xFFFFu), qe = (int)(ch.clip >> 16);
                    const int tlo = (int)(ch.trim & 0xFFFFu), thi = (int)(ch.trim >> 16);
                    const int i0 = 16 * ch.jj;
                    auto bits = [](int lo, int hi) -> u32 {
// ... 7 lines not shown
                    if constexpr (REF) {
                        if (ch.fl & 4u) {
#pragma unroll
                            for (int wd = 0; wd < 4; ++wd)
                                fv[wd] = nonzero_bytes(sv[wd] ^ (fv[wd] & 0x7F7F7F7Fu)) | ((fv[wd] >> 6) & 0x02020202u);
                        }
                    }
                    if (rev) {
                        reverse16(sv); reverse16(fv); reverse16(ov);
                        aligned = __brev(aligned) >> 16; counted = __brev(counted) >> 16;
                    }
                    c0 = rev ? qe - i0 - 16 : i0 - qs;
                    const u32 rev1 = rev ? 0x01010101u : 0u;
#pragma unroll
                    for (int wd = 0; wd < 4; ++wd) {
                        const u32 am = (((aligned >> (4 * wd)) & 0xFu) * 0x00204081u & 0x01010101u) * 0xFFu;
                        const u32 cm_ = (((counted >> (4 * wd)) & 0xFu) * 0x00204081u & 0x01010101u) * 0xFFu;
                        u32 cd, cd5, expect;
                        decode4x(sv[wd], cd, cd5, expect);
                        const u32 odd = nonzero_bytes(expect ^ sv[wd]) * 0xFFu;
                        badbits |= rev ? 0u : (odd & am);
                        cd = (cd & ~odd) | (0x04040404u & odd);
                        const u32 not_n = nonzero_bytes(sv[wd] ^ 0x4E4E4E4Eu);
                        const u32 skipped = ((fv[wd] >> 1) & 0x01010101u) | (not_n ^ 0x01010101u);
                        cd ^= (~cd >> 2) & rev1;
                        cd = (cd & am) | (0x04040404u & ~am);
                        code[wd] = cd; code5[wd] = (cd << 2) + cd;
                        xw[wd] = fv[wd] & 0x01010101u;
                        qv[wd] = ov[wd] & cm_ & ~(skipped * 0xFFu);
                    }
                } else {
                    qv[0] = ch.q[0]; qv[1] = ch.q[1]; qv[2] = ch.q[2]; qv[3] = ch.q[3];
                }
                if constexpr (NIB) {
                    code[0] = nib_lo(ch.s[0]); code[1] = nib_hi(ch.s[0]); code[2] = nib_lo(ch.s[1]); code[3] = nib_hi(ch.s[1]);
                    const u32 x0 = ch.s[0] ^ ch.c[0], x1 = ch.s[1] ^ ch.c[1];
                    xw[0] = nib_lo(x0); xw[1] = nib_hi(x0); xw[2] = nib_lo(x1); xw[3] = nib_hi(x1);
                    badbits = nib_invalid(ch.s[0]) | nib_invalid(ch.s[1]);
                }
#pragma unroll
                for (int wd = 0; wd < 4; ++wd) {
                    if constexpr (NIB) {
                        code5[wd] = (code[wd] << 2) + code[wd];
                    } else if constexpr (!ALN) {
                        u32 expect;
                        decode4x(ch.s[wd], code[wd], code5[wd], expect);
                        badbits |= expect ^ ch.s[wd];
                        xw[wd] = ch.s[wd] ^ ch.c[wd];
                    }
                    hiq |= (qv[wd] + 0x34343434u) | qv[wd];
                }
                hiq &= 0x80808080u;
                const u32 last_code5 = code5[3] >> 24;
                u32 prev_code5 = wave_shr1(last_code5, carry_code);
                carry_code = (u32)__builtin_amdgcn_readlane((int)last_code5, 63);
                u32 prev_char = 0u;
                if constexpr (!NIB && !ALN) {
                    const u32 last_char = ch.s[3] >> 24;
                    prev_char = wave_shr1(last_char, carry_char);
                    carry_char = (u32)__builtin_amdgcn_readlane((int)last_char, 63);
                }
                if (j == 0) { prev_code5 = 20u; prev_char = 0u; }
                if (act) {
                    const long long read = read0 + ch.off;
                    const bool fits_tables = (u32)(len - p.minlen) <= (u32)(p.maxlen - p.minlen);
                    if (hiq || !fits_tables) flag(p.status, ST_INDEX, read);
                    if constexpr (NIB || ALN) {
// ... 31 lines not shown
                                } else {
                                    a = __umul24(tq, row_bytes) + A + (u32)(KJ > 0 ? 4 * KJ * (4 * wd + b) : 4 * (4 * wd + b));
                                }
                                atomicAdd(reinterpret_cast<u32*>(reinterpret_cast<char*>(lds) + a), inc);
                                u32 slot = (d5 >> (8 * b)) & 0xFFu;
                                if (SPLIT) slot = qi <= 255u - p.dlo ? slot : 24u;
                                const u32 trow = tq * dnt_row + dnt_base;
                                const u32 ad = slot * (4u * DN) + trow;
                                __hip_atomic_fetch_add(reinterpret_cast<lds_u32*>(ad), inc, __ATOMIC_RELAXED,
                                                       __HIP_MEMORY_SCOPE_WORKGROUP);
                            };
                            one_base(std::integral_constant<int, 0>{}); one_base(std::integral_constant<int, 1>{});
                            one_base(std::integral_constant<int, 2>{}); one_base(std::integral_constant<int, 3>{});
                        }
                    }
                }
            };

            bool walk = total > 0;
            if constexpr (NIB && KJ > 0) {
                static_assert((KJ & 1) != 0, "the loop below fetches steps in twos and bins the last one alone");
                if (__ballot(myread < seg_hi && m == ((u32)p.maxlen | ((u32)g << 16))) == ~0ull) {
                    walk = false;
                    constexpr int DK = 64 / KJ, DJ = 64 - DK * KJ;
                    int j4 = 4 * lane_j0, k = lane_k0;
                    const u32 at = 16u * (u32)lane;
                    const u32 lds_at = (u32)reinterpret_cast<size_t>(lds);
                    const u32 ctx_at = 4u * CYC + 4u * (u32)(lane & (DN - 1));
                    const u32 dlo4 = (p.dlo < 128u ? p.dlo : 128u) * 0x01010101u;
                    const u32 one = 1u;
                    u32 inc_a = 1u, inc_b = 1u;
                    auto fetch_at = [&](K1Chunk& ch, const uint8_t* fseq, const uint8_t* fcseq, const uint8_t* fqual, u32 o) {
                        const uint2 sv = *reinterpret_cast<const uint2*>(fseq + (o >> 1));
                        const uint2 cv = *reinterpret_cast<const uint2*>(fcseq + (o >> 1));
                        const uint4 qv = *reinterpret_cast<const uint4*>(fqual + o);
                        ch.s[0] = sv.x; ch.s[1] = sv.y; ch.c[0] = cv.x; ch.c[1] = cv.y;
                        ch.q[0] = qv.x; ch.q[1] = qv.y; ch.q[2] = qv.z; ch.q[3] = qv.w;
                    };
                    auto fetch_u = [&](K1Chunk& ch, int s) { fetch_at(ch, bseq, bcseq, bqual, at + 1024u * (u32)s); };
                    auto process_u = [&](const K1Chunk& ch) {
                        u32 code[4], code5[4], xw[4], hiq = 0u;
                        code[0] = nib_lo(ch.s[0]); code[1] = nib_hi(ch.s[0]); code[2] = nib_lo(ch.s[1]); code[3] = nib_hi(ch.s[1]);
                        const u32 x0 = ch.s[0] ^ ch.c[0], x1 = ch.s[1] ^ ch.c[1];
                        xw[0] = nib_lo(x0); xw[1] = nib_hi(x0); xw[2] = nib_lo(x1); xw[3] = nib_hi(x1);
                        const u32 badbits = nib_invalid(ch.s[0]) | nib_invalid(ch.s[1]);
#pragma unroll
                        for (int wd = 0; wd < 4; ++wd) {
                            code5[wd] = (code[wd] << 2) + code[wd];
                            hiq |= (ch.q[wd] + 0x34343434u) | ch.q[wd];
                        }
                        hiq &= 0x80808080u;
                        const u32 last_code5 = code5[3] >> 24;
                        u32 prev_code5 = wave_shr1(last_code5, carry_code);
                        carry_code = (u32)__builtin_amdgcn_readlane((int)last_code5, 63);
                        if (j4 == 0) prev_code5 = 20u;
                        if (hiq | badbits) {
                            if (hiq) flag(p.status, ST_INDEX, read0 + k);
                            if (badbits) flag(p.status, ST_LUT, 0);
                        } else {
                            const u32 A = lds_at + pos_base + (u32)j4;
                            const u32 tcl = tclamp + (u32)(k & (ntrash - 1));
                            const u32 (&qv)[4] = ch.q;
                            const u32 kd = ctx_at - (u32)j4;
                            const u32 kd2 = kd | (kd << 16);
                            u32 pc5 = prev_code5 << 24;
#pragma unroll
                            for (int wd = 0; wd < 4; ++wd) {
                                const u32 pw5 = __builtin_amdgcn_alignbyte(code5[wd], pc5, 3);
                                u32 d5 = pw5 + code[wd];
                                pc5 = code5[wd];
                                if (SPLIT) {
                                    const u32 t = ((qv[wd] | 0x80808080u) - dlo4) & 0x80808080u;
                                    d5 = (d5 & (t - (t >> 7))) | (0x18181818u & ~(t - (t >> 7)));
                                }
                                const u32 e02 = k1_shl6_add(d5 & 0x00FF00FFu, kd2);
                                const u32 e13 = k1_shl6_add(__builtin_amdgcn_perm(0u, d5, 0x0C030C01u), kd2);
                                const u32 xwd = xw[wd];
                                const u32 qn = ~qv[wd];
                                auto one_base = [&](auto bsel) {
                                    constexpr int b = decltype(bsel)::value;
                                    const u32 tq = k1_joint_row<b>(qn, tcl);
                                    u32& inc = (b & 1) ? inc_b : inc_a;
                                    k1_joint_increment<b>(inc, xwd, one);
                                    const u32 a = __umul24(tq, JROW) + A;
                                    __hip_atomic_fetch_add(reinterpret_cast<lds_u32*>(a + (u32)(4 * KJ * (4 * wd + b))), inc, __ATOMIC_RELAXED,
                                                           __HIP_MEMORY_SCOPE_WORKGROUP);
                                    const u32 ad = k1_joint_delta<(b >> 1)>(a, (b & 1) ? e13 : e02);
                                    __hip_atomic_fetch_add(reinterpret_cast<lds_u32*>(ad), inc, __ATOMIC_RELAXED,
                                                           __HIP_MEMORY_SCOPE_WORKGROUP);
                                };
                                one_base(std::integral_constant<int, 0>{}); one_base(std::integral_constant<int, 1>{});
                                one_base(std::integral_constant<int, 2>{}); one_base(std::integral_constant<int, 3>{});
                            }
                        }
                        const int jn = j4 + 4 * DJ;
                        const bool wrap = jn >= 4 * KJ;
                        j4 = wrap ? jn - 4 * KJ : jn;
                        k += DK + (wrap ? 1 : 0);
                    };
                    if (fed) {
                        ua.s[0] = ub.s[0]; ua.s[1] = ub.s[1]; ua.c[0] = ub.c[0]; ua.c[1] = ub.c[1];
                        ua.q[0] = ub.q[0]; ua.q[1] = ub.q[1]; ua.q[2] = ub.q[2]; ua.q[3] = ub.q[3];
                    } else {
                        fetch_u(ua, 0);
                    }
#pragma unroll 1
                    for (int s = 0; s + 1 < KJ; s += 2) {
                        fetch_u(ub, s + 1);
                        process_u(ua);
                        fetch_u(ua, s + 2);
                        process_u(ub);
                    }
                    const long long nblk = blk + (long long)gx * nwaves;
                    ahead = ((nblk + 1) << 6) <= seg_hi - seg_lo;
                    const long long nread0 = ahead ? seg_lo + (nblk << 6) : read0;
                    m_next = p.meta[nread0 + lane];
                    fetch_at(ub, p.seq + (size_t)nread0 * (p.pitch >> 1), p.cseq + (size_t)nread0 * (p.pitch >> 1),
                             p.qual + (size_t)nread0 * p.pitch, at);
                    process_u(ua);
                }
            }
            if (walk) {
                K1Chunk ca, cb;
                ca.k = lane_k0; ca.j = lane_j0;
                cb.k = lane_k0; cb.j = lane_j0; advance(cb, dk1, dj1);
                fetch(ca);
                for (int w0 = 0; w0 < total; w0 += 128) {
                    fetch(cb);
                    process(ca);
                    if (w0 + 64 < total) {
                        advance(ca, dk2, dj2);
                        fetch(ca);
                        process(cb);
                        advance(cb, dk2, dj2);
                    }
                }
                if constexpr (JOINT) __builtin_amdgcn_s_waitcnt(0x0F70);
            }
        }
        ++since_flush; ++since_dn_flush;
        if (since_flush == K1V3_FLUSH_ITERS || since_dn_flush == p.dn_flush_iters) {
            __syncthreads();
            flush_dn(); since_dn_flush = 0;
            if (since_flush == K1V3_FLUSH_ITERS) { flush_pos(); since_flush = 0; }
            __syncthreads();
        }
    }
    __syncthreads();
    flush_dn(); flush_pos();
}

template <bool SPLIT, int DN = K1V3_DNREP, bool NIB = false, int KJ = 0>
__global__ __launch_bounds__(K1V3_THREADS) void k1v3_accumulate(K1v3Params p)
{
    extern __shared__ __attribute__((aligned(16))) u32 lds[];
    k1v3_body<SPLIT, DN, NIB, KJ>(p, lds, (int)blockIdx.x, (int)gridDim.x, (int)blockIdx.y);
}

template <bool SPLIT, int DN>
__global__ __launch_bounds__(K1V3_THREADS) void k1v3_aligned(K1v3Params p)
{
    extern __shared__ __attribute__((aligned(16))) u32 lds[];
    k1v3_body<SPLIT, DN, false, 0, true>(p, lds, (int)blockIdx.x, (int)gridDim.x, (int)blockIdx.y);
}

template <bool SPLIT, int DN>
__global__ __launch_bounds__(K1V3_THREADS) void k1v3_aligned_ref(K1v3Params p)
{
    extern __shared__ __attribute__((aligned(16))) u32 lds[];
    k1v3_body<SPLIT, DN, false, 0, true, true>(p, lds, (int)blockIdx.x, (int)gridDim.x, (int)blockIdx.y);
}

#define K1V3_MAX_BANDS 16
struct K1BandsParams {
    int nbands;
    int wg_start[K1V3_MAX_BANDS + 1];
    int dn[K1V3_MAX_BANDS];
    unsigned long long* dbg;
    K1v3Params band[K1V3_MAX_BANDS];
};

template <bool SPLIT, bool NIB>
__global__ __launch_bounds__(K1V3_THREADS) void k1v3_bands(K1BandsParams t)
{
    extern __shared__ __attribute__((aligned(16))) u32 lds[];
    int b = 0;
    while (b + 1 < t.nbands && (int)blockIdx.x >= t.wg_start[b + 1]) ++b;
    const K1v3Params& p = t.band[b];
    const int bx = (int)blockIdx.x - t.wg_start[b], gx = t.wg_start[b + 1] - t.wg_start[b];
// ... 9 lines not shown
    int rb = (2 * full_lut_width(S2) + 32 + 3) & ~3;
    if (((rb >> 2) & 1) == 0) rb += 4;
    return rb;
}

__host__ __device__ __forceinline__ int pair_pitch(int S2) { return (S2 + 1 + 15) & ~15; }
__host__ __device__ __forceinline__ int pair_lut_row_bytes(int S2)
{
    int rb = pair_pitch(S2) + 32;
    if (((rb >> 2) & 1) == 0) rb += 4;
    return rb;
}

struct K2Chunk { u32 s[4], q[4]; u32 mk; u32 dlo, dhi; int kk; int k; int j; int nb; bool act0; };

struct K2v3Params {
    const uint8_t* seq; const uint8_t* qual; const u32* meta;
    long long nreads; int pitch; int cpr; u32 cpr_magic; int R; int Qt; int S2; int minscore; u32 qlo;
    const int16_t* lut16;
    const int8_t* full;
    int full_bytes; int rs16;
    u32 rb;
    u32 W;
    u32 ctx_off;
    int maxlen;
    int pairs;
    const long long* seg;
    int rpb;
    int parts;
    const long long* perm;
    uint8_t* out; u64* status;
};

template <bool NIB = false>
__global__ __launch_bounds__(K2V3_THREADS) __attribute__((amdgpu_waves_per_eu(K2V3_WAVES, 8))) void k2v3_apply(K2v3Params p)
{
    extern __shared__ __attribute__((aligned(16))) u32 lds[];
    const u32 rb = p.rb;
    const u32 rg_bytes = (u32)(33 + p.Qt) * rb;
    const int g = blockIdx.y;
    {
        const u32* src = reinterpret_cast<const u32*>(p.full + (p.seg ? (size_t)g * rg_bytes : 0));
        const int nw = (int)((p.seg ? rg_bytes : (u32)p.full_bytes) >> 2);
        for (int i = threadIdx.x; i < nw; i += blockDim.x) lds[i] = src[i];
        __syncthreads();
    }
    const int lane = lane_id();
    const int wave = __builtin_amdgcn_readfirstlane((int)(threadIdx.x >> 6));
    const int nwaves = blockDim.x >> 6;
    const long long seg_lo = p.seg ? p.seg[g] : 0ll, seg_hi = p.seg ? p.seg[g + 1] : p.nreads;
    const long long nblocks = (seg_hi - seg_lo + p.rpb - 1) / p.rpb;
    const u32 hi_add = (u32)(0x80 - (p.Qt + 33)) * 0x01010101u;
    const int lane_k0 = p.cpr == 1 ? lane : (int)__umulhi((u32)lane, p.cpr_magic);
    const int lane_j0 = lane - lane_k0 * p.cpr;
    const int dk1 = 64 / p.cpr, dj1 = 64 - dk1 * p.cpr;
    const int dkn = (64 * K2V3_NBUF) / p.cpr, djn = 64 * K2V3_NBUF - dkn * p.cpr;

    long long blk0 = (long long)blockIdx.x * nwaves + wave, blk_step = (long long)gridDim.x * nwaves, blk_end = nblocks;
    if (p.parts > 1 && (int)gridDim.x % p.parts == 0) {
        const long long per = (nblocks + p.parts - 1) / p.parts;
        const int part = (int)blockIdx.x % p.parts;
        blk0 = part * per + (long long)((int)blockIdx.x / p.parts) * nwaves + wave;
        blk_step = (long long)((int)gridDim.x / p.parts) * nwaves;
        blk_end = (part + 1) * per < nblocks ? (part + 1) * per : nblocks;
    }
    for (long long blk = blk0; blk < blk_end; blk += blk_step) {
        const long long read0 = seg_lo + blk * p.rpb;
// ... 9 lines not shown

        auto advance = [&](K2Chunk& ch, int dk, int dj) {
            const int jj = ch.j + dj;
            const bool wrap = jj >= p.cpr;
            ch.j = wrap ? jj - p.cpr : jj;
            ch.kk = ch.kk + dk + (wrap ? 1 : 0);
        };
        auto fetch = [&](K2Chunk& ch) {
            ch.act0 = ch.kk < n;
            ch.k = ch.act0 ? ch.kk : 0;
            ch.mk = bperm(m, ch.k);
            if (p.perm) { ch.dlo = bperm((u32)pm, ch.k); ch.dhi = bperm((u32)(pm >> 32), ch.k); }
            ch.nb = ch.act0 ? ((int)(ch.mk & 0xFFFFu) - 16 * ch.j) : 0;
            const u32 rowoff = ch.nb > 0 ? __umul24((u32)ch.k, (u32)p.pitch) + (u32)(16 * ch.j) : 0u;
            if constexpr (NIB) {
                const uint2 sv = *reinterpret_cast<const uint2*>(bseq + (rowoff >> 1));
                ch.s[0] = sv.x; ch.s[1] = sv.y;
            } else {
                const uint4 sv = *reinterpret_cast<const uint4*>(bseq + rowoff);
                ch.s[0] = sv.x; ch.s[1] = sv.y; ch.s[2] = sv.z; ch.s[3] = sv.w;
            }
            const uint4 qv = *reinterpret_cast<const uint4*>(bqual + rowoff);
            ch.q[0] = qv.x; ch.q[1] = qv.y; ch.q[2] = qv.z; ch.q[3] = qv.w;
        };
        auto process = [&](const K2Chunk& ch) {
            const int j = ch.j, nb = ch.nb, k = ch.k;
            const bool act = nb > 0;
            const int len = (int)(ch.mk & 0xFFFFu);
            const int rg = (int)((ch.mk >> 16) & 0x7FFFu);
            const bool second = (ch.mk >> 31) != 0u;
            const int pos0 = 16 * j;
            u32 code[4], code5[4], badbits = 0u, hiq = 0u;
            if constexpr (NIB) {
                code[0] = nib_lo(ch.s[0]); code[1] = nib_hi(ch.s[0]); code[2] = nib_lo(ch.s[1]); code[3] = nib_hi(ch.s[1]);
                badbits = nib_invalid(ch.s[0]) | nib_invalid(ch.s[1]);
            }
#pragma unroll
            for (int wd = 0; wd < 4; ++wd) {
                if constexpr (NIB) {
                    code5[wd] = (code[wd] << 2) + code[wd];
                } else {
                    u32 expect;
                    decode4x(ch.s[wd], code[wd], code5[wd], expect);
                    badbits |= expect ^ ch.s[wd];
                }
                hiq |= ((ch.q[wd] & 0x7F7F7F7Fu) + hi_add) | ch.q[wd];
            }
            hiq &= 0x80808080u;
            const u32 last_code5 = code5[3] >> 24;
            u32 prev_code5 = wave_shr1(last_code5, carry_code);
            carry_code = (u32)__builtin_amdgcn_readlane((int)last_code5, 63);
            u32 prev_char = 0u;
            if constexpr (!NIB) {
                const u32 last_char = ch.s[3] >> 24;
                prev_char = wave_shr1(last_char, carry_char);
                carry_char = (u32)__builtin_amdgcn_readlane((int)last_char, 63);
            }
            if (j == 0) { prev_code5 = 20u; prev_char = 0u; }
            if (ch.act0) {
                u32 o[4] = {0u, 0u, 0u, 0u};
                if (act) {
                    const long long read = read0 + k;
                    if constexpr (NIB) {
                        if (badbits) flag(p.status, ST_LUT, 0);
                    } else {
                        if (badbits && chunk_type_error(ch.s[0], ch.s[1], ch.s[2], ch.s[3], ch.q[0], ch.q[1], ch.q[2], ch.q[3],
                                                        prev_char, nb, pos0, p.minscore))
                            flag(p.status, ST_TYPE, read);
// ... 66 lines not shown
```

kbbq-py_amd/csrc/kbbq_layout_kernels.h:

```cpp
#pragma once
#include "kbbq_kernels_v3.h"
#include "kbbq_aligned_kernels.h"

#define K7_NSTATS 8
struct MetaStatsParams { const u32* meta; long long n; int* stats; };

__global__ __launch_bounds__(256) void k7_meta_stats(MetaStatsParams p)
{
    int mn = 0x7FFFFFFF, mx = 0, rgmax = 0, viol = 0, empty = 0, tviol = 0;
    const u32 len0 = p.n > 0 ? (p.meta[0] & 0xFFFFu) : 0u;
    const long long npairs = (p.n + 1) >> 1;
    for (long long pr = (long long)blockIdx.x * blockDim.x + threadIdx.x; pr < npairs; pr += (long long)gridDim.x * blockDim.x) {
        const bool has2 = 2 * pr + 1 < p.n;
        const uint2 mm = make_uint2(p.meta[2 * pr], has2 ? p.meta[2 * pr + 1] : 0xFFFFFFFFu);
        const u32 m[2] = {mm.x, mm.y};
        for (int k = 0; k < (has2 ? 2 : 1); ++k) {
            const int len = (int)(m[k] & 0xFFFFu), rg = (int)((m[k] >> 16) & 0x7FFFu);
            if (len) { mn = len < mn ? len : mn; } else ++empty;
            mx = len > mx ? len : mx;
            rgmax = rg > rgmax ? rg : rgmax;
            if ((m[k] & 0xFFFFu) != len0) { ++viol; ++tviol; }
            if ((m[k] >> 31) != 0u) ++tviol;
        }
        if ((mm.x >> 31) != 0u) ++viol;
// ... 96 lines not shown
__global__ __launch_bounds__(1024) void k7_rg_scan(RgScanParams p)
{
    __shared__ u64 part[1024];
    const long long per = (p.count + blockDim.x - 1) / blockDim.x;
    const long long lo = (long long)threadIdx.x * per, hi = lo + per < p.count ? lo + per : p.count;
    u64 s = 0;
    for (long long i = lo; i < hi; ++i) s += p.hist[i];
    part[threadIdx.x] = s;
    __syncthreads();
    if (threadIdx.x == 0) {
        u64 run = 0;
        for (int t = 0; t < (int)blockDim.x; ++t) { const u64 c = part[t]; part[t] = run; run += c; }
    }
    __syncthreads();
    u64 run = part[threadIdx.x];
    for (long long i = lo; i < hi; ++i) {
        const u32 c = p.hist[i];
        p.hist[i] = (u32)run;
        run += c;
    }
    __threadfence_block();
    __syncthreads();
    for (int v = threadIdx.x; v < p.R; v += blockDim.x) p.seg[v] = (long long)p.hist[(size_t)v * p.nblocks];
    if (threadIdx.x == 0) p.seg[p.R] = p.nrows;
}

struct LayOutParams {
    const uint8_t* src[3]; uint8_t* dst[3];
    const u32* meta; u32* dmeta;
    const long long* perm;
    long long nrows;
    long long nsrc;
    int pitch, dpitch, S, pairs, nib;
    int parts;
    u64* status;
};

__device__ __forceinline__ void shl_bytes16(u32 v[4], int nb)
{
    const int ws = nb >> 2; const u32 bs = (u32)(nb & 3) * 8u;
    const u32 a3 = ws == 0 ? v[3] : ws == 1 ? v[2] : ws == 2 ? v[1] : v[0];
    const u32 a2 = ws == 0 ? v[2] : ws == 1 ? v[1] : ws == 2 ? v[0] : 0u;
    const u32 a1 = ws == 0 ? v[1] : ws == 1 ? v[0] : 0u;
    const u32 a0 = ws == 0 ? v[0] : 0u;
    v[3] = bs ? __builtin_amdgcn_alignbit(a3, a2, 32u - bs) : a3;
    v[2] = bs ? __builtin_amdgcn_alignbit(a2, a1, 32u - bs) : a2;
    v[1] = bs ? __builtin_amdgcn_alignbit(a1, a0, 32u - bs) : a1;
    v[0] = a0 << bs;
}

__device__ __forceinline__ void load16_clamped(const uint8_t* plane, long long at, long long limit, u32 out[4])
{
    const long long hi = limit - 16;
    const long long c = at < 0 ? 0 : (at > hi ? hi : at);
    load16_any(plane, c, out);
    if (at < 0) shl_bytes16(out, (int)(-at));
    else if (at > hi) shr_bytes16(out, (int)(at - hi));
}

__global__ __launch_bounds__(256) void k7_lay_out(LayOutParams p)
{
    const int cpr = p.dpitch >> 4;
    const int S = p.S;
    const int rpb = cpr <= 256 ? 256 / cpr : 1;
    const int slot = cpr <= 256 ? (int)threadIdx.x / cpr : 0;
    const int j0 = (int)threadIdx.x - slot * cpr;
// ... 21 lines not shown
#pragma unroll
                for (int pl = 0; pl < 3; ++pl) {
                    if (!p.src[pl]) continue;
                    const u32 f4 = pl == 2 ? 0u : 0x4E4E4E4Eu;
                    u32 a[4], b[4];
                    load16_any(p.src[pl], at1, a);
                    load16_clamped(p.src[pl], at2, limit, b);
#pragma unroll
                    for (int w = 0; w < 4; ++w) {
                        const u32 m1 = 16 * j < p.pitch ? byte_mask(S - 16 * j, w) : 0u;
                        const u32 m2 = lone ? 0u : range_mask(S + 1 - 16 * j, 2 * S + 1 - 16 * j, w);
                        o[pl][w] = (a[w] & m1) | (b[w] & m2) | (f4 & ~(m1 | m2));
                    }
                }
            } else {
                const u32 m = p.meta[r];
                const int len = (int)(m & 0xFFFFu);
                if (j == 0) p.dmeta[d] = m;
                const size_t off = (size_t)r * p.pitch + (size_t)16 * j;
#pragma unroll
                for (int pl = 0; pl < 3; ++pl) {
                    if (!p.src[pl]) continue;
                    const u32 f4 = pl == 2 ? 0u : 0x4E4E4E4Eu;
                    const uint4 v = *reinterpret_cast<const uint4*>(p.src[pl] + off);
                    const u32 a[4] = {v.x, v.y, v.z, v.w};
#pragma unroll
                    for (int w = 0; w < 4; ++w) {
                        const u32 m1 = byte_mask(len - 16 * j, w);
                        o[pl][w] = (a[w] & m1) | (f4 & ~m1);
                    }
                }
            }
            *reinterpret_cast<uint4*>(p.dst[2] + (size_t)d * p.dpitch + (size_t)16 * j) = make_uint4(o[2][0], o[2][1], o[2][2], o[2][3]);
#pragma unroll
            for (int pl = 0; pl < 2; ++pl) {
                if (!p.src[pl]) continue;
                if (p.nib) {
                    u32 bad = 0u;
                    const u32 c0 = chars_to_codes(o[pl][0], bad), c1 = chars_to_codes(o[pl][1], bad);
                    const u32 c2 = chars_to_codes(o[pl][2], bad), c3 = chars_to_codes(o[pl][3], bad);
                    if (bad) flag(p.status, ST_LUT, 0);
                    *reinterpret_cast<uint2*>(p.dst[pl] + (size_t)d * (p.dpitch >> 1) + (size_t)8 * j) = make_uint2(c0 | (c1 << 4), c2 | (c3 << 4));
                } else {
                    *reinterpret_cast<uint4*>(p.dst[pl] + (size_t)d * p.dpitch + (size_t)16 * j) = make_uint4(o[pl][0], o[pl][1], o[pl][2], o[pl][3]);
                }
            }
        }
    }
}

struct UnNibParams { const uint8_t* src; uint8_t* dst; long long nchunks; };
__global__ __launch_bounds__(256) void k7_unpack_nibbles(UnNibParams p)
{
    for (long long ch = (long long)blockIdx.x * blockDim.x + threadIdx.x; ch < p.nchunks; ch += (long long)gridDim.x * blockDim.x) {
        const uint2 v = *reinterpret_cast<const uint2*>(p.src + 8 * ch);
        *reinterpret_cast<uint4*>(p.dst + 16 * ch) = make_uint4(codes_to_chars(nib_lo(v.x)), codes_to_chars(nib_hi(v.x)),
                                                                 codes_to_chars(nib_lo(v.y)), codes_to_chars(nib_hi(v.y)));
    }
}

struct AddTablesParams { long long* dst; const long long* src; long long n; };
__global__ __launch_bounds__(256) void k7_add_tables(AddTablesParams p)
{
    for (long long i = (long long)blockIdx.x * blockDim.x + threadIdx.x; i < p.n; i += (long long)gridDim.x * blockDim.x) p.dst[i] += p.src[i];
}

// ... 61 lines not shown
```

kbbq-py_amd/kbbq/_device.py:

```python
import ctypes
import os

import numpy as np

from . import _native as N

MINSCORE = 6
MAXSCORE = 42
NQ = MAXSCORE + 1

_contexts = {}


_backend = None


def use_native_memory():
    global _backend
    from . import _hipmem
    if _backend is not None and _backend is not _hipmem:
        raise RuntimeError('use_native_memory(): this process already uses torch for device memory')
    if not _hipmem.cuda.is_available():
        raise N.KbbqHipError('no HIP device available: kbbq needs an MI355X (gfx950); there is no CPU fallback')
    _backend = _hipmem
# ... 127 lines not shown
_pinned = {}
_pinned_lock = __import__('threading').RLock()


def pinned(tag, index, nbytes):
    torch = _torch()
    key = (tag, index)
    with _pinned_lock:
        buf = _pinned.get(key)
        if buf is None or buf.shape[0] < nbytes:
            for other, cand in list(_pinned.items()):
                if other[0] == '' and cand.shape[0] >= nbytes:
                    buf = _pinned.pop(other)
                    break
            else:
                buf = torch.empty(int(nbytes), dtype=torch.uint8, pin_memory=True)
            _pinned[key] = buf
    return buf


_released = [0]


def release_pinned(tag):
    with _pinned_lock:
        for key in [k for k in _pinned if k[0] == tag]:
            _released[0] += 1
            _pinned[('', _released[0])] = _pinned.pop(key)


class ReadBatch:

    nib = False
    seg = None
    perm = None
    tally_qual = None

    def __init__(self, n, pitch, with_corrected=True, device=None, nib=False):
        torch = _torch()
        dev = 'cuda' if device is None else device
        self.n, self.pitch, self.nib = int(n), int(pitch), bool(nib)
        rows = max(self.n, 1)
        sp = pitch // 2 if nib else pitch
        self.seq = torch.empty((rows, sp), dtype=torch.uint8, device=dev)
        self.qual = torch.empty((rows, pitch), dtype=torch.uint8, device=dev)
        self.cseq = torch.empty((rows, sp), dtype=torch.uint8, device=dev) if with_corrected else None
        self.meta = torch.empty(rows, dtype=torch.int32, device=dev)

    def describe(self):
        return _describe(self, 'one read per row, pitch %d' % self.pitch)

    def layout_key(self):
        return 'reads_nib' if self.nib else 'reads'

    def chars(self, name='seq'):
        return _plane_chars(self, name)

    @classmethod
    def from_host(cls, seq, qual, meta, cseq=None, device=None):
        torch = _torch()
        n, pitch = seq.shape
        b = cls(n, pitch, with_corrected=cseq is not None, device=device)
        if n:
            b.seq[:n].copy_(torch.from_numpy(np.ascontiguousarray(seq)))
            b.qual[:n].copy_(torch.from_numpy(np.ascontiguousarray(qual)))
            if cseq is not None:
# ... 24 lines not shown
                b.qual[lo:lo + m].copy_(h_qual, non_blocking=True)
                if other is not None:
                    b.cseq[lo:lo + m].copy_(h_cseq, non_blocking=True)
                b.meta[lo:lo + m].copy_(h_meta, non_blocking=True)
                events[slot] = torch.cuda.Event()
                events[slot].record()
            for e in events.values():
                e.synchronize()
        if not keep_pinned:
            release_pinned('ingest')
        b.h2d_bytes = n * (planes * pitch + 4)
        return b

    @classmethod
    def synthetic(cls, first, n, total, seed, len_lo=150, len_hi=150, nrg=1, qlo=0, qhi=41,
                  pitch=None, device=None):
        from ._synth import SYNTH_THR
        if pitch is None:
            pitch = max(16, (len_hi + 15) // 16 * 16)
        b = cls(n, pitch, with_corrected=True, device=device)
        ctx = context(b.seq.device.index)
        N.check(N.load().kbbq_synth_dev(ctx.handle, N.ptr(b.seq), N.ptr(b.cseq), N.ptr(b.qual),
                                        N.ptr(b.meta), first, n, total, pitch, seed,
                                        len_lo, len_hi, nrg, qlo, qhi, N.ptr(SYNTH_THR)))
        return b

    def lengths_host(self):
        return (self.meta[:self.n].cpu().numpy().view(np.uint32) & 0xFFFF).astype(np.int64)


class PairBatch:

    nib = False
    seg = None
    perm = None
    tally_qual = None
    twins = False

    def __init__(self, npairs, S, with_corrected=True, device=None, nib=False):
        torch = _torch()
        dev = 'cuda' if device is None else device
        self.n, self.S, self.nib = int(npairs), int(S), bool(nib)
        self.pitch = int(N.load().kbbq_pair_pitch(2 * self.S))
        rows = max(self.n, 1)
        sp = self.pitch // 2 if nib else self.pitch
        self.seq = torch.empty((rows, sp), dtype=torch.uint8, device=dev)
        self.qual = torch.empty((rows, self.pitch), dtype=torch.uint8, device=dev)
        self.cseq = torch.empty((rows, sp), dtype=torch.uint8, device=dev) if with_corrected else None
        self.meta = torch.empty(rows, dtype=torch.int32, device=dev)
        self.read_pitch = None

    def describe(self):
        return _describe(self, ('two single-end reads per row, pitch %d' if self.twins else 'mate-pair rows, pitch %d per pair') % self.pitch)

    def layout_key(self):
        return 'pairs_nib' if self.nib else 'pairs'

    def chars(self, name='seq'):
        return _plane_chars(self, name)

    @staticmethod
    def worthwhile(S, pitch):
        return int(N.load().kbbq_pair_pitch(2 * int(S))) < 2 * int(pitch)

    @classmethod
    def from_reads(cls, batch):
# ... 5 lines not shown
        st = meta_stats(batch)
        S = st['longest']
        if st['pair_violations'] or S == 0:
            raise ValueError('reads are not uniform first/second pairs of one length and read group')
        pb = cls(n // 2, S, with_corrected=batch.cseq is not None, device=batch.seq.device)
        pb.read_pitch = batch.pitch
        ctx = context(batch.seq.device.index)
        N.check(N.load().kbbq_pack_pairs_dev(ctx.handle, N.ptr(batch.seq), N.ptr(batch.cseq), N.ptr(batch.qual),
                                             N.ptr(batch.meta), pb.n, batch.pitch, 2 * S,
                                             N.ptr(pb.seq), N.ptr(pb.cseq), N.ptr(pb.qual), N.ptr(pb.meta)))
        return pb

    def unpack(self, plane, pitch=None):
        torch = _torch()
        pitch = int(pitch or self.read_pitch or (self.S + 15) // 16 * 16)
        out = torch.empty((max(2 * self.n, 1), pitch), dtype=torch.uint8, device=plane.device)
        ctx = context(plane.device.index)
        N.check(N.load().kbbq_unpack_pairs_dev(ctx.handle, N.ptr(plane), self.n, 2 * self.S, pitch, N.ptr(out)))
        return out


def meta_stats(batch):
    ctx = context(batch.meta.device.index)
    st = np.zeros(8, dtype=np.int32)
    N.check(N.load().kbbq_meta_stats_dev(ctx.handle, N.ptr(batch.meta), batch.n, N.ptr(st)))
    shortest = int(st[0]) if st[0] != 0x7FFFFFFF else 0
    return {'shortest': shortest, 'longest': int(st[1]), 'max_rg': int(st[2]), 'pair_violations': int(st[3]), 'empty': int(st[4]),
            'twin_violations': int(st[5])}


def _describe(batch, base):
    if batch.nib:
        base += ', 4-bit sequence planes'
    if batch.seg is not None:
        base += ', rows grouped by read group'
    return base


def _plane_chars(batch, name):
    torch = _torch()
    plane = getattr(batch, name)
    if not batch.nib:
        return plane
    out = torch.empty((plane.shape[0], batch.pitch), dtype=torch.uint8, device=plane.device)
    ctx = context(plane.device.index)
    N.check(N.load().kbbq_unpack_nibbles_dev(ctx.handle, N.ptr(plane), plane.shape[0] * batch.pitch, N.ptr(out)))
    return out


GROUP_NATIVE_MAX_R = 256


def _group_perm(meta, nrows, pairs, R):
    torch = _torch()
    dev_ = meta.device
    if R <= GROUP_NATIVE_MAX_R:
        lib = N.load()
        ctx = context(dev_.index)
        work = torch.empty(lib.kbbq_group_rows_work_bytes(nrows, R), dtype=torch.uint8, device=dev_)
        perm = torch.empty(max(nrows, 1), dtype=torch.int64, device=dev_)
        seg = torch.empty(R + 1, dtype=torch.int64, device=dev_)
        N.check(lib.kbbq_group_rows_dev(ctx.handle, N.ptr(meta), nrows, 1 if pairs else 0, R, N.ptr(work), N.ptr(perm), N.ptr(seg)))
        try:
            ctx.status()
        except ValueError as e:
            raise ValueError('a row carries a read group >= R = %d (%s)' % (R, e)) from None
        return perm[:nrows], seg
    rg = ((meta[:2 * nrows:2] if pairs else meta[:nrows]) >> 16) & 0x7FFF
    if nrows and int(rg.max().item()) >= R:
        raise ValueError('a row carries read group %d but R = %d' % (int(rg.max().item()), R))
    perm = torch.argsort(rg, stable=True)
    seg = torch.zeros(R + 1, dtype=torch.int64, device=dev_)
    seg[1:] = torch.cumsum(torch.bincount(rg, minlength=R), 0)
    return perm, seg


def _lay_out_rows(batch, flags, S2, perm, seg):
    pairs, nib = bool(flags & N.ROWS_PAIRS), bool(flags & N.ROWS_NIBBLES)
    if pairs:
        laid = PairBatch((batch.n + 1) // 2, S2 // 2, with_corrected=batch.cseq is not None, device=batch.seq.device, nib=nib)
        laid.read_pitch, laid.twins = batch.pitch, bool(flags & N.ROWS_TWINS)
    elif isinstance(batch, PairBatch):
        laid = PairBatch(batch.n, batch.S, with_corrected=batch.cseq is not None, device=batch.seq.device, nib=nib)
        laid.read_pitch, laid.twins = batch.read_pitch, batch.twins
        flags &= ~N.ROWS_TWINS
    else:
        laid = ReadBatch(batch.n, batch.pitch, with_corrected=batch.cseq is not None, device=batch.seq.device, nib=nib)
    ctx = context(batch.seq.device.index)
    N.check(N.load().kbbq_lay_out_dev(ctx.handle, N.ptr(batch.seq), N.ptr(batch.cseq), N.ptr(batch.qual), N.ptr(batch.meta),
                                      batch.n, batch.pitch, flags, S2, N.ptr(perm),
                                      N.ptr(laid.seq), N.ptr(laid.cseq), N.ptr(laid.qual), N.ptr(laid.meta)))
    laid.seg, laid.perm = seg, perm
    return laid


def layout_flags(st, n, pitch, packed=True, pairs=None):
    S_ = st['longest']
    fits = n % 2 == 0 and S_ > 0
    twin_fits = S_ > 0 and n >= 2 and st['twin_violations'] == 0
    twins = False
    if pairs is None:
        pairs = fits and st['pair_violations'] == 0 and PairBatch.worthwhile(S_, pitch)
        if not pairs and twin_fits and PairBatch.worthwhile(S_, pitch):
            pairs = twins = True
    elif pairs and not (fits and st['pair_violations'] == 0):
        if not twin_fits:
            raise ValueError('reads are not uniform first/second pairs (or single-end neighbours) of one length and read group')
        twins = True
    return (N.ROWS_PAIRS if pairs else 0) | (N.ROWS_NIBBLES if packed else 0) | (N.ROWS_TWINS if twins else 0)


def lay_out(batch, R, S=None, packed=True, pairs=None, stats=None):
    if batch.nib or batch.seg is not None or isinstance(batch, PairBatch):
        raise ValueError('lay_out takes input-order rows of characters')
    if batch.n == 0:
        return batch
    st = stats or meta_stats(batch)
    S_ = st['longest']
    flags = layout_flags(st, batch.n, batch.pitch, packed, pairs)
    pairs = bool(flags & N.ROWS_PAIRS)
    perm = seg = None
    if R > 1:
        perm, seg = _group_perm(batch.meta, (batch.n + 1) // 2 if pairs else batch.n, pairs, R)
    if not flags and perm is None:
        return batch
    ctx = context(batch.seq.device.index)
    laid = _lay_out_rows(batch, flags, 2 * S_, perm, seg)
    if packed:
        try:
            ctx.status()
        except N.LutNeedsCheckedApply:
            if not (flags & ~N.ROWS_NIBBLES) and perm is None:
                return batch
            laid = _lay_out_rows(batch, flags & ~N.ROWS_NIBBLES, 2 * S_, perm, seg)
    return laid


def laid_from_reader(text, other, infer_rg_flag, first, n, pitch, R, packed=True, pairs=None, slab=1 << 17, device=None, pair_S=None,
                     keep_pinned=False, with_out=False):
    torch = _torch()
    if n == 0:
        return None
    meta, st = text.meta(infer_rg_flag, first, n)
    S_ = st['longest']
    if pair_S is not None and S_ != pair_S and pairs is None:
        pairs = False
    flags = layout_flags(st, n, pitch, packed, pairs)
    two = bool(flags & N.ROWS_PAIRS)
    nrows = (n + 1) // 2 if two else n
    perm = seg = None
    if R > 1:
        if st['max_rg'] >= R:
            raise ValueError('a row carries read group %d but R = %d' % (st['max_rg'], R))
        perm, seg = np.empty(nrows, dtype=np.int64), np.empty(R + 1, dtype=np.int64)
        N.check(N.load().kbbq_group_rows_host(N.ptr(meta), nrows, 1 if two else 0, R, N.ptr(perm), N.ptr(seg)))
    while True:
        if not flags and perm is None:
            return None
        nib = bool(flags & N.ROWS_NIBBLES)
        if two:
            laid = PairBatch(nrows, S_, with_corrected=other is not None, device=device, nib=nib)
            laid.read_pitch, laid.twins = pitch, bool(flags & N.ROWS_TWINS)
        else:
            laid = ReadBatch(n, pitch, with_corrected=other is not None, device=device, nib=nib)
        if with_out:
            laid.out_plane = torch.empty_like(laid.qual)
        dp = laid.pitch
        sp = dp // 2 if nib else dp
        nseq = 2 if other is not None else 1
        step = max(slab // 2 if two else slab, 1)
        row_bytes = nseq * sp + dp + 4
        events, foreign = {}, False
        with torch.cuda.device(laid.seq.device):
            for k, lo in enumerate(range(0, nrows, step)):
                m = min(step, nrows - lo)
                slot = k % 3
                if slot in events:
                    events[slot].synchronize()
                buf = pinned('ingest', slot, step * row_bytes)
                at = [0]

                def view(width, rows=m, cap=step):
                    v = buf[at[0]:at[0] + rows * width].view(rows, width)
                    at[0] += cap * width
                    return v
                h_seq = view(sp)
                h_cseq = view(sp) if other is not None else None
                h_qual = view(dp)
                h_meta = buf[at[0]:at[0] + 4 * m].view(torch.int32)
                foreign |= text.fill_rows(other, first, n, meta, flags, 2 * S_, dp, perm, lo, m, h_seq.numpy(),
                                          None if h_cseq is None else h_cseq.numpy(), h_qual.numpy(), h_meta.numpy().view(np.uint32))
                if foreign:
                    break
                laid.seq[lo:lo + m].copy_(h_seq, non_blocking=True)
                laid.qual[lo:lo + m].copy_(h_qual, non_blocking=True)
                if other is not None:
                    laid.cseq[lo:lo + m].copy_(h_cseq, non_blocking=True)
                laid.meta[lo:lo + m].copy_(h_meta, non_blocking=True)
                events[slot] = torch.cuda.Event()
                events[slot].record()
            for e in events.values():
                e.synchronize()
        if not keep_pinned:
            release_pinned('ingest')
        if not foreign:
            break
        flags &= ~N.ROWS_NIBBLES
    laid.h2d_bytes = nrows * row_bytes
    if perm is not None:
        laid.perm = torch.from_numpy(perm).to(laid.seq.device)
        laid.seg = torch.from_numpy(seg).to(laid.seq.device)
        laid.h2d_bytes += perm.nbytes + seg.nbytes
    return laid


def group_by_rg(batch, R):
    import copy
    if batch.nib:
        raise ValueError('group_by_rg takes character planes (lay_out groups and packs in one pass)')
    n = batch.n
    perm, seg = _group_perm(batch.meta, n, False, R)
    if n == 0:
        g = copy.copy(batch)
        g.seg, g.perm = seg, perm
        return g
    return _lay_out_rows(batch, 0, 2 * getattr(batch, 'S', 0), perm, seg)


def ungroup(batch, plane):
    torch = _torch()
    n = batch.n
    out = torch.empty_like(plane[:max(n, 1)])
    if n:
        out.index_copy_(0, batch.perm, plane[:n])
    return out


_pair_luts = {}


def _row_flags(batch):
    pairs = isinstance(batch, PairBatch)
    return (N.ROWS_PAIRS if pairs else 0) | (N.ROWS_NIBBLES if batch.nib else 0) | (N.ROWS_TWINS if pairs and batch.twins else 0)


LONG_READS = 160
PACKED_READS = int(os.environ.get('KBBQ_PACKED_READS', '320'))


def accumulate(batch, tables, minscore=MINSCORE, check=True, dinuc_minscore=None, s_band=0, s_min=0):
    ctx = context(batch.seq.device.index)
    pairs = isinstance(batch, PairBatch)
    if pairs and tables.S2 != 2 * batch.S:
        raise ValueError('mate-pair rows of %d-base reads need tables with 2S = %d columns' % (batch.S, 2 * batch.S))
    if not pairs and not s_min and batch.n and (s_band or tables.S2 // 2) > LONG_READS:
        st = meta_stats(batch)
        s_min = st['shortest']
        s_band = s_band or min(max(st['longest'], 1), tables.S2 // 2)
    dm = minscore if dinuc_minscore is None else dinuc_minscore
    if batch.seg is not None or batch.nib or pairs:
        N.check(N.load().kbbq_accumulate_rows_dev(ctx.handle, N.ptr(batch.seq), N.ptr(batch.cseq), N.ptr(batch.qual),
                                                  N.ptr(batch.meta), batch.n, batch.pitch, _row_flags(batch),
                                                  tables.R, tables.S2, int(s_band), int(s_min), minscore, dm,
                                                  N.ptr(batch.seg), N.ptr(tables.buf)))
    else:
        N.check(N.load().kbbq_accumulate_band_dev(ctx.handle, N.ptr(batch.seq), N.ptr(batch.cseq),
                                                  N.ptr(batch.qual), N.ptr(batch.meta), batch.n, batch.pitch,
                                                  tables.R, tables.S2, int(s_band), int(s_min), minscore, dm,
                                                  N.ptr(tables.buf)))
    if check:
        ctx.status()


def _addr(x):
    return None if x is None else x.data_ptr()

# ... 333 lines not shown
```

kbbq-py_amd/kbbq/_native.py:

```python
import ctypes
import os

HERE = os.path.dirname(os.path.abspath(__file__))
LIB_PATH = os.environ.get('KBBQ_HIP_LIB') or os.path.join(HERE, 'libkbbq_hip.so')

KBBQ_OK = 0
KBBQ_E_HIP = -1
KBBQ_E_INDEX = -2
KBBQ_E_TYPE = -3
KBBQ_E_ARG = -4
KBBQ_E_RANGE = -5
KBBQ_E_NAME = -6
KBBQ_E_LUT = -7
KBBQ_E_MEANQ = -8
KBBQ_E_FULL = -9
APPLY_CHECKED, APPLY_FAST = 0, 1
ALIGNED_LUT, ALIGNED_F64 = 0, 1
ROWS_PAIRS, ROWS_NIBBLES, ROWS_TWINS = 1, 2, 4
KMER_FIX_N = 1
KMER_MAX_PASSES = 8
KMER_FLAG_UNRESOLVED = 2
CONFUSION_MAX_BASES = (1 << 32) - 1
BGZF_BLOCK_MAX, BGZF_SLOT, BGZF_EOF_BYTES = 65280, 65536, 28
BAM_QUAL_PLANE, BAM_QUAL_SKELETON = 0, 1
BAM_DESC_WORDS = 6

NQ = 43
NDINUC = 16

_c = ctypes
_vp, _i, _i64, _u64, _sz = _c.c_void_p, _c.c_int, _c.c_int64, _c.c_uint64, _c.c_size_t

PROTOTYPES = {
    'kbbq_abi_version': (_i, []),
    'kbbq_last_error': (_c.c_char_p, []),
    'kbbq_device_count': (_i, [_c.POINTER(_i)]),
    'kbbq_host_threads': (_i, [_sz]),
    'kbbq_host_advise_huge': (_i, [_vp, _sz]),
    'kbbq_bind_host_to_pci': (_i, [_c.c_char_p, _c.POINTER(_i), _c.POINTER(_i)]),
    'kbbq_bind_host_to_device': (_i, [_i, _c.POINTER(_i), _c.POINTER(_i)]),
    'kbbq_ctx_create': (_i, [_i, _c.POINTER(_vp)]),
    'kbbq_ctx_destroy': (_i, [_vp]),
    'kbbq_ctx_set_stream': (_i, [_vp, _vp]),
    'kbbq_ctx_sync': (_i, [_vp]),
    'kbbq_ctx_status': (_i, [_vp, _c.POINTER(_i64)]),
    'kbbq_ctx_info': (_i, [_vp, _c.POINTER(_i), _c.POINTER(_i), _c.c_char_p, _i]),
    'kbbq_dev_alloc': (_i, [_vp, _sz, _c.POINTER(_vp)]),
    'kbbq_dev_free': (_i, [_vp, _vp]),
    'kbbq_dev_zero': (_i, [_vp, _vp, _sz]),
    'kbbq_dev_upload': (_i, [_vp, _vp, _vp, _sz]),
    'kbbq_dev_download': (_i, [_vp, _vp, _vp, _sz]),
# ... 335 lines not shown
```

kbbq-py_amd/kbbq/_stream.py:

```python
from . import _device as dev
from . import fastx
from ._trace import stage

REFUSALS = (IndexError, TypeError, ValueError, dev.N.LutNeedsCheckedApply)


def resident_bytes(n, S):
    return int(n) * (4 * fastx.pitch_for(S) + 4)


def slab_reads(budget, bytes_per_read):
    return max(2, int(budget * 0.8) // max(int(bytes_per_read), 1) & ~1)


class Peak:

    def __init__(self, budget):
        self.budget = int(budget)
        torch = dev._torch()
        torch.cuda.synchronize()
        torch.cuda.empty_cache()
        dev.memory_peak(reset=True)
        self.before = int(torch.cuda.memory_allocated()) if hasattr(torch.cuda, 'memory_allocated') else 0
        if hasattr(torch.cuda, 'set_reserve_limit'):
            torch.cuda.set_reserve_limit(self.before + self.budget)

    def report(self):
        return {'device_budget_bytes': self.budget, 'resident_before_bytes': self.before,
                'peak_device_bytes': max(dev.memory_peak() - self.before, 0)}

    def close(self):
        torch = dev._torch()
        if hasattr(torch.cuda, 'set_reserve_limit'):
            torch.cuda.set_reserve_limit(None)


def _slab_band(A, B, infer_rg, origin, s_lo, m, longest, shortest, pitch):
    return dict(first=s_lo, n=m, S=longest, Smin=shortest, pitch=pitch, source=(A, B, infer_rg, origin + s_lo), batch=None, laid=None,
                keep_pinned=True)


def _tally_slabs(A, B, infer_rg, lo, hi, tables, minscore, budget, careful):
    R, S2 = tables.R, tables.S2
    for b_lo, b_hi, longest, shortest in A.length_bands(lo, hi - lo):
        pitch = fastx.pitch_for(longest)
        step = slab_reads(budget, 3 * pitch + 4)
        hints = dict(s_band=longest, s_min=shortest)
        for s_lo in range(b_lo, b_hi, step):
            m = min(step, b_hi - s_lo)
            band = _slab_band(A, B, infer_rg, lo, s_lo, m, longest, shortest, pitch)
            with stage('fill'):
                laid = dev.laid_from_reader(A, B, infer_rg, lo + s_lo, m, pitch, max(R, 1), packed=longest <= dev.PACKED_READS,
                                            pair_S=S2 // 2, keep_pinned=True)
            try:
                done = False
                if laid is not None:
                    try:
                        with stage('K1'):
                            if careful:
                                part = dev.Tables(R, S2)
                                dev.accumulate(laid, part, minscore, **hints)
                                tables.add(part)
                            else:
                                dev.accumulate(laid, tables, minscore, check=False, **hints)
                        done = True
                    except REFUSALS:
                        pass
                    laid = None
                if not done:
                    with stage('fill'):
                        rows = fastx.band_rows(band)
                    with stage('K1'):
                        dev.accumulate(rows, tables, minscore, check=careful, **hints)
                    rows = None
            except (IndexError, TypeError) as e:
                if hasattr(e, 'read_index'):
                    e.read_index = s_lo + max(e.read_index, 0)
                raise
            finally:
                band['batch'] = None


def tally_range(A, B, infer_rg, lo, hi, tables, minscore, budget):
    if hi <= lo:
        return
    ctx = dev.context(tables.buf.device.index)
# ... 68 lines not shown
```

Baseline: 1214 billion.

## Fold corrected-read mismatch into spare nibble bit to drop corrected plane

Adds a KBBQ_ROWS_ERRBIT layout for 4-bit mate-pair rows (2x150 and 2x100). The host fill ORs a per-base mismatch bit (seq vs corrected) into the high bit of each nibble, and the tally stream no longer transfers or reads the separate corrected-sequence plane. New K1 and K2 kernel instances are templated on the error-bit form. This cuts host-to-device bytes and device reads in accumulate. In exchange it adds host-side packing work and more kernel variants to maintain.

```diff
diff --git a/include/kbbq_hip.h b/include/kbbq_hip.h
--- a/include/kbbq_hip.h
+++ b/include/kbbq_hip.h
@@ -187,6 +187,7 @@
 #define KBBQ_ROWS_PAIRS    1
 #define KBBQ_ROWS_NIBBLES  2
 #define KBBQ_ROWS_TWINS    4
+#define KBBQ_ROWS_ERRBIT   8
 int    kbbq_accumulate_rows_dev(kbbq_ctx* ctx, const uint8_t* d_seq, const uint8_t* d_cseq, const uint8_t* d_qual,
                                 const uint32_t* d_meta, int64_t nrows, int pitch, int flags, int R, int S2, int S_band,
                                 int S_min, int minscore, int dinuc_minscore, const int64_t* d_seg, int64_t* d_tables);
diff --git a/kbbq-py_amd/csrc/fastq_host.cpp b/kbbq-py_amd/csrc/fastq_host.cpp
--- a/kbbq-py_amd/csrc/fastq_host.cpp
+++ b/kbbq-py_amd/csrc/fastq_host.cpp
@@ -701,10 +701,14 @@
                          int S2, int pitch, const int64_t* perm, int64_t row_lo, int64_t nrows,
                          uint8_t* seq, uint8_t* cseq, uint8_t* qual, uint32_t* dmeta, int* foreign)
 {
-    if (!a || (nrows > 0 && (!seq || !qual || !dmeta || !meta || (b && !cseq)))) return kbbq_set_error_(KBBQ_E_ARG, "kbbq_fastq_fill_rows: NULL argument");
+    const bool errbit = (flags & KBBQ_ROWS_ERRBIT) != 0;
+    if (!a || (nrows > 0 && (!seq || !qual || !dmeta || !meta || (b && !cseq && !errbit)))) return kbbq_set_error_(KBBQ_E_ARG, "kbbq_fastq_fill_rows: NULL argument");
     if (first < 0 || n < 0 || first + n > (int64_t)a->h0.size() || (b && first + n > (int64_t)b->h0.size()))
         return kbbq_set_error_(KBBQ_E_ARG, "kbbq_fastq_fill_rows: range out of bounds");
-    if (flags & ~(KBBQ_ROWS_PAIRS | KBBQ_ROWS_NIBBLES | KBBQ_ROWS_TWINS)) return kbbq_set_error_(KBBQ_E_ARG, "kbbq_fastq_fill_rows: unknown layout flags");
+    if (flags & ~(KBBQ_ROWS_PAIRS | KBBQ_ROWS_NIBBLES | KBBQ_ROWS_TWINS | KBBQ_ROWS_ERRBIT)) return kbbq_set_error_(KBBQ_E_ARG, "kbbq_fastq_fill_rows: unknown layout flags");
+    if (errbit && (!b || (flags & (KBBQ_ROWS_PAIRS | KBBQ_ROWS_NIBBLES)) != (KBBQ_ROWS_PAIRS | KBBQ_ROWS_NIBBLES)
+                   || (((S2 + 1 + 15) & ~15) != 16 * 19 && ((S2 + 1 + 15) & ~15) != 16 * 13)))
+        return kbbq_set_error_(KBBQ_E_ARG, "kbbq_fastq_fill_rows: KBBQ_ROWS_ERRBIT needs the corrected reads and 4-bit mate-pair rows of 19 or 13 chunks");
     const bool pairs = (flags & KBBQ_ROWS_PAIRS) != 0, nib = (flags & KBBQ_ROWS_NIBBLES) != 0;
     const int S = S2 / 2;
     if (pairs) {
@@ -717,13 +721,13 @@
     const size_t sp = nib ? (size_t)pitch / 2 : (size_t)pitch;
     std::atomic<int> bad(0); std::atomic<unsigned> odd(0);
     parallel_for(nrows, nthreads_for((size_t)nrows * (size_t)pitch * 3), [&](int64_t lo, int64_t hi) {
-        std::vector<uint8_t> tmp(nib ? (size_t)pitch : 0);
+        std::vector<uint8_t> tmp(nib ? (size_t)pitch : 0), cnib(errbit ? sp : 0);
         unsigned foreign_here = 0;
         for (int64_t row = lo; row < hi; ++row) {
             const int64_t s = perm ? perm[row_lo + row] : row_lo + row;
             if (s < 0 || s >= total) { bad = 3; continue; }
             uint8_t* q = qual + (size_t)row * pitch;
-            uint8_t* planes[2] = {seq + (size_t)row * sp, b ? cseq + (size_t)row * sp : nullptr};
+            uint8_t* planes[2] = {seq + (size_t)row * sp, b ? (cseq ? cseq + (size_t)row * sp : cnib.data()) : nullptr};
             const kbbq_fastq* src[2] = {a, b};
             if (pairs) {
                 const int64_t i1 = first + 2 * s; const bool lone = 2 * s + 1 >= n; const int64_t i2 = lone ? i1 : i1 + 1;
@@ -739,6 +743,13 @@
                     else { c[S] = 'N'; memcpy(c + S + 1, src[pl]->buf + src[pl]->s0[i2], (size_t)S); memset(c + 2 * S + 1, 'N', (size_t)(pitch - 2 * S - 1)); }
                     if (nib) foreign_here |= pack_row(c, pitch, planes[pl]);
                 }
+                if (errbit)
+                    for (size_t i = 0; i < sp; i += 8) {
+                        uint64_t s8, c8;
+                        memcpy(&s8, planes[0] + i, 8); memcpy(&c8, planes[1] + i, 8);
+                        s8 |= (((s8 ^ c8) & 0x7777777777777777ull) + 0x7777777777777777ull) & 0x8888888888888888ull;
+                        memcpy(planes[0] + i, &s8, 8);
+                    }
                 dmeta[row] = (uint32_t)(2 * S + 1) | (meta[2 * s] & 0x7FFF0000u);
             } else {
                 const int64_t i = first + s;
diff --git a/kbbq-py_amd/csrc/kbbq_hip.hip b/kbbq-py_amd/csrc/kbbq_hip.hip
--- a/kbbq-py_amd/csrc/kbbq_hip.hip
+++ b/kbbq-py_amd/csrc/kbbq_hip.hip
@@ -88,38 +88,40 @@
 static const u64 ST_INIT[KBBQ_NSTATUS] = {~0ull, ~0ull, ~0ull, ~0ull, ~0ull, ~0ull, ~0ull, ~0ull};
 
 enum K1Form { K1_ROWS, K1_ALIGNED, K1_ALIGNED_REF, K1_BANDS };
-struct K1Variant { K1Form form; int dn, nib, kj; const void* kernel[2]; };
+struct K1Variant { K1Form form; int dn, nib, kj, eb; const void* kernel[2]; };
 #define K1_SPLITS(K, ...) {(const void*)(K<false, __VA_ARGS__>), (const void*)(K<true, __VA_ARGS__>)}
 static const K1Variant K1_VARIANTS[] = {
-    {K1_ROWS, K1V3_DNREP, 0, 0, K1_SPLITS(k1v3_accumulate, K1V3_DNREP)},
-    {K1_ROWS, 8, 0, 0, K1_SPLITS(k1v3_accumulate, 8)},
-    {K1_ROWS, K1V3_DNREP, 1, 0, K1_SPLITS(k1v3_accumulate, K1V3_DNREP, true)},
-    {K1_ROWS, 8, 1, 0, K1_SPLITS(k1v3_accumulate, 8, true)},
-    {K1_ROWS, K1V3_DNREP, 1, 13, K1_SPLITS(k1v3_accumulate, K1V3_DNREP, true, 13)},
-    {K1_ROWS, K1V3_DNREP, 1, 19, K1_SPLITS(k1v3_accumulate, K1V3_DNREP, true, 19)},
-    {K1_ALIGNED, K1V3_DNREP, 0, 0, K1_SPLITS(k1v3_aligned, K1V3_DNREP)},
-    {K1_ALIGNED, 8, 0, 0, K1_SPLITS(k1v3_aligned, 8)},
-    {K1_ALIGNED_REF, K1V3_DNREP, 0, 0, K1_SPLITS(k1v3_aligned_ref, K1V3_DNREP)},
-    {K1_ALIGNED_REF, 8, 0, 0, K1_SPLITS(k1v3_aligned_ref, 8)},
-    {K1_BANDS, 0, 0, 0, K1_SPLITS(k1v3_bands, false)},
-    {K1_BANDS, 0, 1, 0, K1_SPLITS(k1v3_bands, true)},
+    {K1_ROWS, K1V3_DNREP, 0, 0, 0, K1_SPLITS(k1v3_accumulate, K1V3_DNREP)},
+    {K1_ROWS, 8, 0, 0, 0, K1_SPLITS(k1v3_accumulate, 8)},
+    {K1_ROWS, K1V3_DNREP, 1, 0, 0, K1_SPLITS(k1v3_accumulate, K1V3_DNREP, true)},
+    {K1_ROWS, 8, 1, 0, 0, K1_SPLITS(k1v3_accumulate, 8, true)},
+    {K1_ROWS, K1V3_DNREP, 1, 13, 0, K1_SPLITS(k1v3_accumulate, K1V3_DNREP, true, 13)},
+    {K1_ROWS, K1V3_DNREP, 1, 19, 0, K1_SPLITS(k1v3_accumulate, K1V3_DNREP, true, 19)},
+    {K1_ROWS, K1V3_DNREP, 1, 13, 1, K1_SPLITS(k1v3_accumulate, K1V3_DNREP, true, 13, true)},
+    {K1_ROWS, K1V3_DNREP, 1, 19, 1, K1_SPLITS(k1v3_accumulate, K1V3_DNREP, true, 19, true)},
+    {K1_ALIGNED, K1V3_DNREP, 0, 0, 0, K1_SPLITS(k1v3_aligned, K1V3_DNREP)},
+    {K1_ALIGNED, 8, 0, 0, 0, K1_SPLITS(k1v3_aligned, 8)},
+    {K1_ALIGNED_REF, K1V3_DNREP, 0, 0, 0, K1_SPLITS(k1v3_aligned_ref, K1V3_DNREP)},
+    {K1_ALIGNED_REF, 8, 0, 0, 0, K1_SPLITS(k1v3_aligned_ref, 8)},
+    {K1_BANDS, 0, 0, 0, 0, K1_SPLITS(k1v3_bands, false)},
+    {K1_BANDS, 0, 1, 0, 0, K1_SPLITS(k1v3_bands, true)},
 };
 #undef K1_SPLITS
 
-static const void* k1_kernel(K1Form form, bool split, int dn, int nib, int kj)
+static const void* k1_kernel(K1Form form, bool split, int dn, int nib, int kj, int eb = 0)
 {
     for (const K1Variant& v : K1_VARIANTS)
-        if (v.form == form && v.dn == dn && v.nib == nib && v.kj == kj) return v.kernel[split];
+        if (v.form == form && v.dn == dn && v.nib == nib && v.kj == kj && v.eb == eb) return v.kernel[split];
     return nullptr;
 }
 
-enum LdsKernel { LK_K1_PLAIN, LK_K1_PLAIN_SPLIT, LK_K1_TILED, LK_K1_TILED_SPLIT, LK_K2V3, LK_K2V3_NIB, LK_K2T, LK_K2T_NIB, LK_K2T_BANDS, LK_K2T_PAIR19, LK_K2T_PAIR13, LK_K2_LDS16, LK_K2_LDS8, LK_BGZF, LK_COUNT };
+enum LdsKernel { LK_K1_PLAIN, LK_K1_PLAIN_SPLIT, LK_K1_TILED, LK_K1_TILED_SPLIT, LK_K2V3, LK_K2V3_NIB, LK_K2V3_NIB_EB, LK_K2T, LK_K2T_NIB, LK_K2T_BANDS, LK_K2T_PAIR19, LK_K2T_PAIR13, LK_K2T_PAIR19_EB, LK_K2T_PAIR13_EB, LK_K2_LDS16, LK_K2_LDS8, LK_BGZF, LK_COUNT };
 static const void* const LDS_KERNELS[LK_COUNT] = {
     (const void*)k1_accumulate<false>, (const void*)k1_accumulate<true>,
     (const void*)k1_accumulate_tiled<false>, (const void*)k1_accumulate_tiled<true>,
-    (const void*)k2v3_apply<false>, (const void*)k2v3_apply<true>,
+    (const void*)k2v3_apply<false>, (const void*)k2v3_apply<true>, (const void*)k2v3_apply<true, true>,
     (const void*)k2t_apply<false>, (const void*)k2t_apply<true>, (const void*)k2t_bands,
-    (const void*)k2t_apply_pair<19>, (const void*)k2t_apply_pair<13>,
+    (const void*)k2t_apply_pair<19>, (const void*)k2t_apply_pair<13>, (const void*)k2t_apply_pair<19, true>, (const void*)k2t_apply_pair<13, true>,
     (const void*)k2_apply<int16_t, true, true>, (const void*)k2_apply<int8_t, true, false>,
     (const void*)bz_deflate,
 };
@@ -483,11 +485,11 @@
                                   minscore, minscore, d_tables);
 }
 
-struct K1Setup { K1v3Params q; int dn = 0; int kj = 0; size_t lds = 0; };
+struct K1Setup { K1v3Params q; int dn = 0; int kj = 0; int eb = 0; size_t lds = 0; };
 static int accumulate_rows(kbbq_ctx* c, const char* who, const uint8_t* d_seq, const uint8_t* d_cseq, const uint8_t* d_qual,
                            const uint32_t* d_meta, int64_t nrows, int pitch, int pairs, int R, int S2, int minscore,
                            int dinuc_minscore, const int64_t* d_seg, int64_t* d_tables, bool* fits, int S_band = 0, int S_min = 0, int nib = 0,
-                           int twins = 0, K1Setup* setup_only = nullptr);
+                           int twins = 0, K1Setup* setup_only = nullptr, int errbit = 0);
 
 int kbbq_accumulate_ex_dev(kbbq_ctx* c, const uint8_t* d_seq, const uint8_t* d_cseq,
                            const uint8_t* d_qual, const uint32_t* d_meta,
@@ -674,7 +676,7 @@
     return q;
 }
 
-static int launch_k2v3(kbbq_ctx* c, const K2v3Params& q, int nib)
+static int launch_k2v3(kbbq_ctx* c, const K2v3Params& q, int nib, int errbit = 0)
 {
     const int slices = q.seg ? q.R : 1;
     const size_t lds = (size_t)(33 + q.Qt) * q.rb * (size_t)(q.seg ? 1 : q.R);
@@ -682,12 +684,12 @@
     const int64_t nblocks = (q.nreads + q.rpb - 1) / q.rpb;
     const int64_t want = (nblocks + (K2V3_THREADS / 64) - 1) / (K2V3_THREADS / 64);
     const int gx = (int)std::min<int64_t>(want, std::max<int64_t>(1, (int64_t)c->cus * per_cu / slices));
-    return launch_lds(c, 1, LDS_KERNELS[nib ? LK_K2V3_NIB : LK_K2V3], dim3((unsigned)std::max(gx, 1), (unsigned)slices, 1), dim3(K2V3_THREADS), lds, &q);
+    return launch_lds(c, 1, LDS_KERNELS[errbit ? LK_K2V3_NIB_EB : nib ? LK_K2V3_NIB : LK_K2V3], dim3((unsigned)std::max(gx, 1), (unsigned)slices, 1), dim3(K2V3_THREADS), lds, &q);
 }
 
 static int apply_rows(kbbq_ctx* c, const char* who, const uint8_t* d_seq, const uint8_t* d_qual, const uint32_t* d_meta,
                       int64_t nrows, int pitch, int pairs, int R, int S2, int minscore, const void* d_lut_blob,
-                      const void* d_pair_lut, const int64_t* d_seg, uint8_t* d_out, int nib = 0, const int64_t* d_perm = nullptr);
+                      const void* d_pair_lut, const int64_t* d_seg, uint8_t* d_out, int nib = 0, const int64_t* d_perm = nullptr, int errbit = 0);
 
 int kbbq_apply_dev(kbbq_ctx* c, const uint8_t* d_seq, const uint8_t* d_qual, const uint32_t* d_meta,
                    int64_t nreads, int pitch, int R, int Qt, int S2, int minscore,
@@ -984,18 +986,21 @@
 static int launch_k1(kbbq_ctx* c, K1Form form, const K1Setup& su, int nib)
 {
     const int gx = (int)std::min<int64_t>(k1_iters(su.q), std::max(1, c->cus / su.q.R));
-    return launch_lds(c, 0, k1_kernel(form, k1_split(su.q), su.dn, nib, su.kj), dim3((unsigned)gx, (unsigned)su.q.R, 1), dim3(K1V3_THREADS),
+    return launch_lds(c, 0, k1_kernel(form, k1_split(su.q), su.dn, nib, su.kj, su.eb), dim3((unsigned)gx, (unsigned)su.q.R, 1), dim3(K1V3_THREADS),
                       su.lds, &su.q);
 }
 
 static int accumulate_rows(kbbq_ctx* c, const char* who, const uint8_t* d_seq, const uint8_t* d_cseq, const uint8_t* d_qual,
                            const uint32_t* d_meta, int64_t nrows, int pitch, int pairs, int R, int S2, int minscore,
                            int dinuc_minscore, const int64_t* d_seg, int64_t* d_tables, bool* fits, int S_band, int S_min, int nib, int twins,
-                           K1Setup* setup_only)
+                           K1Setup* setup_only, int errbit)
 {
     if (fits) *fits = true;
     if (S_band < 0 || S_band > S2 / 2 || (pairs && S_band)) return fail(KBBQ_E_ARG, "%s: S_band out of range (%d)", who, S_band);
     if (S_min < 0 || S_min > (S_band ? S_band : S2 / 2)) return fail(KBBQ_E_ARG, "%s: S_min out of range (%d)", who, S_min);
+    if (errbit) d_cseq = nullptr;
+    if (errbit && !(pairs && nib && (pitch == 16 * 19 || pitch == 16 * 13)))
+        return fail(KBBQ_E_ARG, "%s: KBBQ_ROWS_ERRBIT describes 4-bit mate-pair rows of 19 or 13 chunks (pitch %d)", who, pitch);
     int rc = check_planes(who, nrows, pitch, d_seq, d_cseq, d_qual);
     if (rc) return rc;
     if (R <= 0 || R > 32767) return fail(KBBQ_E_ARG, "%s: R out of range (%d)", who, R);
@@ -1027,10 +1032,11 @@
             const size_t rows = (size_t)q.nrows - 1 + nt;
             su.lds = rows * q.row_bytes;
             if (su.lds > (size_t)c->lds_bytes) continue;
-            su.dn = K1V3_DNREP; su.kj = q.cpr;
+            su.dn = K1V3_DNREP; su.kj = q.cpr; su.eb = errbit ? 1 : 0;
             q.ntrash = nt; q.pos_copy_bytes = (u32)(rows * q.row_bytes);
         }
     }
+    if (errbit && !su.kj) return fail(KBBQ_E_ARG, "%s: the joint-row tables of KBBQ_ROWS_ERRBIT rows do not fit the LDS (%d bytes)", who, c->lds_bytes);
     for (int attempt = 0; attempt < (trim ? 3 : 1) && !su.dn; ++attempt) {
         const int copies = attempt == 2 ? 8 : K1V3_DNREP, cut = attempt ? trim : 0;
         if (k1_geometry(q, c, copies, cut, cut)) su.dn = copies;
@@ -1075,7 +1081,7 @@
     if (!c) return fail(KBBQ_E_ARG, "ctx is NULL");
     int rc = check_pairs("kbbq_pair_lut_dev", 0, S2);
     if (rc) return rc;
-    if (!(flags & KBBQ_ROWS_PAIRS) || (flags & ~(KBBQ_ROWS_PAIRS | KBBQ_ROWS_NIBBLES | KBBQ_ROWS_TWINS)))
+    if (!(flags & KBBQ_ROWS_PAIRS) || (flags & ~(KBBQ_ROWS_PAIRS | KBBQ_ROWS_NIBBLES | KBBQ_ROWS_TWINS | KBBQ_ROWS_ERRBIT)))
         return fail(KBBQ_E_ARG, "kbbq_pair_lut_rows_dev: flags 0x%x are not those of mate-pair rows", flags);
     if (R <= 0 || R > 32767 || !d_lut_blob || !d_pair_lut) return fail(KBBQ_E_ARG, "kbbq_pair_lut_dev: bad argument");
     HIPCHK(hipSetDevice(c->device));
@@ -1102,10 +1108,12 @@
 
 static int apply_rows(kbbq_ctx* c, const char* who, const uint8_t* d_seq, const uint8_t* d_qual, const uint32_t* d_meta,
                       int64_t nrows, int pitch, int pairs, int R, int S2, int minscore, const void* d_lut_blob,
-                      const void* d_pair_lut, const int64_t* d_seg, uint8_t* d_out, int nib, const int64_t* d_perm)
+                      const void* d_pair_lut, const int64_t* d_seg, uint8_t* d_out, int nib, const int64_t* d_perm, int errbit)
 {
     int rc = check_planes(who, nrows, pitch, d_seq, d_qual, d_out);
     if (rc) return rc;
+    if (errbit && !(pairs && nib && (pitch == 16 * 19 || pitch == 16 * 13)))
+        return fail(KBBQ_E_ARG, "%s: KBBQ_ROWS_ERRBIT describes 4-bit mate-pair rows of 19 or 13 chunks (pitch %d)", who, pitch);
     if (R <= 0 || R > 32767 || !d_lut_blob || (pairs && (!d_pair_lut || ((uintptr_t)d_pair_lut & 15)))) return fail(KBBQ_E_ARG, "%s: bad argument", who);
     if (S2 <= 0 || (S2 & 1) || S2 > 65534) return fail(KBBQ_E_ARG, "%s: S2 must be positive and even (%d)", who, S2);
     if (minscore < 0 || minscore > 222) return fail(KBBQ_E_ARG, "%s: minscore out of range", who);
@@ -1119,7 +1127,7 @@
     if (nrows == 0) return KBBQ_OK;
     HIPCHK(hipSetDevice(c->device));
     if (!pairs && !narrowed_row_lut(c, d_lut_blob, R, KQ, S2, Sb, minscore, &q.full)) return fail(KBBQ_E_HIP, "%s: no scratch for the narrowed LUT", who);
-    if (!k2_tile_serves(c, pairs, nib, R, d_seg != nullptr, q.cpr, rg_bytes)) return launch_k2v3(c, q, nib);
+    if (!k2_tile_serves(c, pairs, nib, R, d_seg != nullptr, q.cpr, rg_bytes)) return launch_k2v3(c, q, nib, errbit);
 
     K2tParams t = k2t_params(q);
     const int64_t per_wg = (int64_t)(K2T_THREADS / 64) * 64 * K2T_STEPS;
@@ -1145,7 +1153,9 @@
     }
     const int kj = (pairs && nib) ? k2t_pair_form(t) : 0;
     if (kj < 0) return fail(KBBQ_E_ARG, "%s: mate-pair rows of %d chunks do not have the geometry k2t_apply_pair was compiled for", who, q.cpr);
-    const LdsKernel k = kj == 19 ? LK_K2T_PAIR19 : kj == 13 ? LK_K2T_PAIR13 : nib ? LK_K2T_NIB : LK_K2T;
+    if (errbit && kj <= 0) return fail(KBBQ_E_ARG, "%s: no instance of K2 reads KBBQ_ROWS_ERRBIT rows of %d chunks", who, q.cpr);
+    const LdsKernel k = kj == 19 ? (errbit ? LK_K2T_PAIR19_EB : LK_K2T_PAIR19) : kj == 13 ? (errbit ? LK_K2T_PAIR13_EB : LK_K2T_PAIR13)
+                        : nib ? LK_K2T_NIB : LK_K2T;
     return launch_lds(c, 1, LDS_KERNELS[k], dim3((unsigned)gt), dim3(K2T_THREADS), (size_t)t.lut_bytes, &t);
 }
 
@@ -1171,9 +1181,14 @@
 }
 
 
-static int layout_flags_ok(const char* who, int flags)
-{
-    if (flags & ~(KBBQ_ROWS_PAIRS | KBBQ_ROWS_NIBBLES | KBBQ_ROWS_TWINS)) return fail(KBBQ_E_ARG, "%s: unknown layout flags 0x%x", who, flags);
+static int layout_flags_ok(const char* who, int flags, bool errbit_ok = false)
+{
+    if (flags & ~(KBBQ_ROWS_PAIRS | KBBQ_ROWS_NIBBLES | KBBQ_ROWS_TWINS | KBBQ_ROWS_ERRBIT)) return fail(KBBQ_E_ARG, "%s: unknown layout flags 0x%x", who, flags);
+    if (flags & KBBQ_ROWS_ERRBIT) {
+        if (!errbit_ok) return fail(KBBQ_E_ARG, "%s: layout flags 0x%x: KBBQ_ROWS_ERRBIT planes are read by kbbq_accumulate_rows_dev / kbbq_apply_rows_dev only", who, flags);
+        if ((flags & (KBBQ_ROWS_PAIRS | KBBQ_ROWS_NIBBLES)) != (KBBQ_ROWS_PAIRS | KBBQ_ROWS_NIBBLES))
+            return fail(KBBQ_E_ARG, "%s: KBBQ_ROWS_ERRBIT describes 4-bit mate-pair rows (KBBQ_ROWS_PAIRS | KBBQ_ROWS_NIBBLES)", who);
+    }
     if ((flags & KBBQ_ROWS_TWINS) && !(flags & KBBQ_ROWS_PAIRS)) return fail(KBBQ_E_ARG, "%s: KBBQ_ROWS_TWINS describes mate-pair rows (add KBBQ_ROWS_PAIRS)", who);
     return KBBQ_OK;
 }
@@ -1183,13 +1198,13 @@
                              int S_min, int minscore, int dinuc_minscore, const int64_t* d_seg, int64_t* d_tables)
 {
     if (!c) return fail(KBBQ_E_ARG, "ctx is NULL");
-    int rc = layout_flags_ok("kbbq_accumulate_rows_dev", flags);
+    int rc = layout_flags_ok("kbbq_accumulate_rows_dev", flags, true);
     if (rc) return rc;
     const int pairs = (flags & KBBQ_ROWS_PAIRS) ? 1 : 0;
     if (pairs) { rc = check_pairs("kbbq_accumulate_rows_dev", nrows, S2); if (rc) return rc; }
     return accumulate_rows(c, "kbbq_accumulate_rows_dev", d_seq, d_cseq, d_qual, d_meta, nrows, pitch, pairs, R, S2, minscore,
                            dinuc_minscore, d_seg, d_tables, nullptr, pairs ? 0 : S_band, pairs ? 0 : S_min,
-                           (flags & KBBQ_ROWS_NIBBLES) ? 1 : 0, (flags & KBBQ_ROWS_TWINS) ? 1 : 0);
+                           (flags & KBBQ_ROWS_NIBBLES) ? 1 : 0, (flags & KBBQ_ROWS_TWINS) ? 1 : 0, nullptr, (flags & KBBQ_ROWS_ERRBIT) ? 1 : 0);
 }
 
 int kbbq_apply_rows_dev(kbbq_ctx* c, const uint8_t* d_seq, const uint8_t* d_qual, const uint32_t* d_meta, int64_t nrows,
@@ -1197,12 +1212,12 @@
                         const int64_t* d_seg, const int64_t* d_perm, uint8_t* d_out)
 {
     if (!c) return fail(KBBQ_E_ARG, "ctx is NULL");
-    int rc = layout_flags_ok("kbbq_apply_rows_dev", flags);
+    int rc = layout_flags_ok("kbbq_apply_rows_dev", flags, true);
     if (rc) return rc;
     const int pairs = (flags & KBBQ_ROWS_PAIRS) ? 1 : 0;
     if (pairs) { rc = check_pairs("kbbq_apply_rows_dev", nrows, S2); if (rc) return rc; }
     return apply_rows(c, "kbbq_apply_rows_dev", d_seq, d_qual, d_meta, nrows, pitch, pairs, R, S2, minscore, d_lut_blob,
-                      d_pair_lut, d_seg, d_out, (flags & KBBQ_ROWS_NIBBLES) ? 1 : 0, d_perm);
+                      d_pair_lut, d_seg, d_out, (flags & KBBQ_ROWS_NIBBLES) ? 1 : 0, d_perm, (flags & KBBQ_ROWS_ERRBIT) ? 1 : 0);
 }
 
 static int band_accumulate_alone(kbbq_ctx* c, const kbbq_band& b, int R, int S2, int minscore, int dinuc_minscore, int64_t* d_tables)
@@ -1250,7 +1265,7 @@
     for (int i = 0; i < nbands; ++i) {
         const kbbq_band& b = bands[i];
         if (b.nrows == 0) continue;
-        int rc = layout_flags_ok("kbbq_accumulate_bands_dev", b.flags);
+        int rc = layout_flags_ok("kbbq_accumulate_bands_dev", b.flags, true);
         if (rc) return rc;
         const int pairs = (b.flags & KBBQ_ROWS_PAIRS) ? 1 : 0, nib = (b.flags & KBBQ_ROWS_NIBBLES) ? 1 : 0;
         K1Setup su; bool fits = false;
@@ -1259,7 +1274,7 @@
             if (pairs) { rc = check_pairs("kbbq_accumulate_bands_dev", b.nrows, S2); if (rc) return rc; }
             rc = accumulate_rows(c, "kbbq_accumulate_bands_dev", b.d_seq, b.d_cseq, b.d_qual, b.d_meta, b.nrows, b.pitch, pairs, R, S2, minscore,
                                  dinuc_minscore, b.d_seg, d_tables, &fits, pairs ? 0 : b.S_band, pairs ? 0 : b.S_min, nib,
-                                 (b.flags & KBBQ_ROWS_TWINS) ? 1 : 0, &su);
+                                 (b.flags & KBBQ_ROWS_TWINS) ? 1 : 0, &su, (b.flags & KBBQ_ROWS_ERRBIT) ? 1 : 0);
             if (rc) return rc;
             can = fits && !su.kj && (nib_of_merge < 0 || nib_of_merge == nib);
         }
@@ -1335,7 +1350,7 @@
     for (int i = 0; i < nbands; ++i) {
         const kbbq_band& b = bands[i];
         if (b.nrows == 0) continue;
-        int rc = layout_flags_ok("kbbq_apply_bands_dev", b.flags);
+        int rc = layout_flags_ok("kbbq_apply_bands_dev", b.flags, true);
         if (rc) return rc;
         const int Sb = std::min(b.pitch, S2);
         const bool can = (int)merged.size() < K2T_MAX_BANDS && R == 1
@@ -1428,12 +1443,14 @@
                      uint8_t* d_lseq, uint8_t* d_lcseq, uint8_t* d_lqual, uint32_t* d_lmeta)
 {
     if (!c) return fail(KBBQ_E_ARG, "ctx is NULL");
-    int rc = layout_flags_ok("kbbq_lay_out_dev", flags);
-    if (rc) return rc;
-    const int pairs = (flags & KBBQ_ROWS_PAIRS) ? 1 : 0, nib = (flags & KBBQ_ROWS_NIBBLES) ? 1 : 0;
+    int rc = layout_flags_ok("kbbq_lay_out_dev", flags, true);
+    if (rc) return rc;
+    const int pairs = (flags & KBBQ_ROWS_PAIRS) ? 1 : 0, nib = (flags & KBBQ_ROWS_NIBBLES) ? 1 : 0, errbit = (flags & KBBQ_ROWS_ERRBIT) ? 1 : 0;
+    if (errbit && (!d_cseq || (pair_pitch(S2) != 16 * 19 && pair_pitch(S2) != 16 * 13)))
+        return fail(KBBQ_E_ARG, "kbbq_lay_out_dev: KBBQ_ROWS_ERRBIT needs the corrected reads and mate-pair rows of 19 or 13 chunks");
     rc = check_planes("kbbq_lay_out_dev", nreads, pitch, d_seq, d_cseq, d_qual);
     if (rc) return rc;
-    if (!d_seq || !d_qual || !d_meta || !d_lseq || !d_lqual || !d_lmeta || (d_cseq && !d_lcseq)) return fail(KBBQ_E_ARG, "kbbq_lay_out_dev: NULL pointer");
+    if (!d_seq || !d_qual || !d_meta || !d_lseq || !d_lqual || !d_lmeta || (d_cseq && !d_lcseq && !errbit)) return fail(KBBQ_E_ARG, "kbbq_lay_out_dev: NULL pointer");
     if (((uintptr_t)d_lseq | (uintptr_t)d_lcseq | (uintptr_t)d_lqual) & 15) return fail(KBBQ_E_ARG, "kbbq_lay_out_dev: planes must be 16-byte aligned");
     if (pairs) {
         rc = check_pairs("kbbq_lay_out_dev", (nreads + 1) / 2, S2);
@@ -1447,7 +1464,7 @@
     p.src[0] = d_seq; p.src[1] = d_cseq; p.src[2] = d_qual; p.dst[0] = d_lseq; p.dst[1] = d_lcseq; p.dst[2] = d_lqual;
     p.meta = d_meta; p.dmeta = d_lmeta; p.perm = reinterpret_cast<const long long*>(d_perm);
     p.nrows = pairs ? (nreads + 1) / 2 : nreads; p.nsrc = nreads; p.pitch = pitch; p.dpitch = pairs ? pair_pitch(S2) : pitch; p.S = pairs ? S2 / 2 : 0;
-    p.pairs = pairs; p.nib = nib; p.status = c->d_status;
+    p.pairs = pairs; p.nib = nib; p.errbit = errbit; p.status = c->d_status;
     const int rpb7 = (p.dpitch / 16) <= 256 ? 256 / (p.dpitch / 16) : 1;
     const int gx = bounded_grid((p.nrows + rpb7 - 1) / rpb7, c, 256);
     p.parts = K7_FRONTS;
@@ -1553,6 +1570,7 @@
                                   uint8_t* d_out_qual, uint32_t* d_out_meta)
 {
     if (!c) return fail(KBBQ_E_ARG, "ctx is NULL");
+    if (layout & KBBQ_ROWS_ERRBIT) return fail(KBBQ_E_ARG, "kbbq_canonical_reads_rows_dev: layout flags 0x%x: KBBQ_ROWS_ERRBIT describes mate-pair rows; the output is one read per row", layout);
     if (layout & ~KBBQ_ROWS_NIBBLES) return fail(KBBQ_E_ARG, "kbbq_canonical_reads_rows_dev: the output is one read per row (layout 0 or KBBQ_ROWS_NIBBLES)");
     if (nreads < 0 || pitch <= 0 || (pitch & 15) || S <= 0 || S > pitch || S > 65535)
         return fail(KBBQ_E_ARG, "kbbq_canonical_reads_dev: bad nreads/pitch/S");
diff --git a/kbbq-py_amd/csrc/kbbq_k2_tile.h b/kbbq-py_amd/csrc/kbbq_k2_tile.h
--- a/kbbq-py_amd/csrc/kbbq_k2_tile.h
+++ b/kbbq-py_amd/csrc/kbbq_k2_tile.h
@@ -250,7 +250,7 @@
 
 typedef unsigned short k2t_u16x2 __attribute__((ext_vector_type(2)));
 
-template <int KJ>
+template <int KJ, bool EB = false>
 __global__ __launch_bounds__(K2T_THREADS) void k2t_apply_pair(K2tParams p)
 {
     extern __shared__ __attribute__((aligned(16))) u32 lds[];
@@ -304,7 +304,7 @@
         mk[s] = mbase[drow];
     }
     u32 before = 4u;
-    if (base_c > 0) before = (u32)sbase[-1] >> 4;
+    if (base_c > 0) before = EB ? ((u32)sbase[-1] >> 4) & 7u : (u32)sbase[-1] >> 4;
     {
         const uint4* src = reinterpret_cast<const uint4*>(p.lut + (size_t)g * (size_t)(33 + p.Qt) * p.rb);
         const int n16 = p.lut_bytes >> 4;
@@ -322,8 +322,9 @@
         const int len = (int)(mk[s] & 0xFFFFu);
         const int nb = act0 ? len - (int)a16[s] : 0;
         u32 code[4], code5[4], hiq = 0u;
-        code[0] = nib_lo(sq[s][0]); code[1] = nib_hi(sq[s][0]); code[2] = nib_lo(sq[s][1]); code[3] = nib_hi(sq[s][1]);
-        const u32 badbits = nib_invalid(sq[s][0]) | nib_invalid(sq[s][1]);
+        code[0] = nib_lo_code<EB>(sq[s][0]); code[1] = nib_hi_code<EB>(sq[s][0]);
+        code[2] = nib_lo_code<EB>(sq[s][1]); code[3] = nib_hi_code<EB>(sq[s][1]);
+        const u32 badbits = nib_bad<EB>(sq[s][0]) | nib_bad<EB>(sq[s][1]);
 #pragma unroll
         for (int wd = 0; wd < 4; ++wd) {
             code5[wd] = (code[wd] << 2) + code[wd];
diff --git a/kbbq-py_amd/csrc/kbbq_kernels_v3.h b/kbbq-py_amd/csrc/kbbq_kernels_v3.h
--- a/kbbq-py_amd/csrc/kbbq_kernels_v3.h
+++ b/kbbq-py_amd/csrc/kbbq_kernels_v3.h
@@ -92,6 +92,14 @@
 __device__ __forceinline__ u32 nib_lo(u32 w) { return w & NIBM; }
 __device__ __forceinline__ u32 nib_hi(u32 w) { return (w >> 4) & NIBM; }
 __device__ __forceinline__ u32 nib_invalid(u32 w) { return (((w & 0x77777777u) + 0x33333333u) | w) & 0x88888888u; }
+#define NIBM3 0x07070707u
+template <bool EB> __device__ __forceinline__ u32 nib_lo_code(u32 w) { return w & (EB ? NIBM3 : NIBM); }
+template <bool EB> __device__ __forceinline__ u32 nib_hi_code(u32 w) { return (w >> 4) & (EB ? NIBM3 : NIBM); }
+template <bool EB> __device__ __forceinline__ u32 nib_bad(u32 w)
+{
+    if constexpr (EB) return ((w & 0x77777777u) + 0x33333333u) & 0x88888888u;
+    else return nib_invalid(w);
+}
 __device__ __forceinline__ u32 chars_to_codes(u32 w, u32& bad)
 {
     const u32 h = (w >> 1) & 0x07070707u;
@@ -125,11 +133,12 @@
 
 struct K1Chunk { u32 s[4], c[4], q[4]; u32 mk; u32 off; int k; int j; int nb; u32 fl, clip, trim; int jj; u32 g0lo, g0hi; };
 
-template <bool SPLIT, int DN, bool NIB, int KJ, bool ALN = false, bool REF = false>
+template <bool SPLIT, int DN, bool NIB, int KJ, bool ALN = false, bool REF = false, bool EB = false>
 __device__ __forceinline__ void k1v3_body(const K1v3Params& p, u32* lds, const int bx, const int gx, const int g)
 {
     static_assert(!ALN || (!NIB && KJ == 0), "the aligned-read form reads character planes");
     static_assert(!REF || ALN, "the reference comparison belongs to the aligned-read form");
+    static_assert(!EB || (NIB && KJ > 0), "the error bit lives in the 4-bit mate-pair rows of the joint-row forms");
     constexpr bool JOINT = KJ > 0;
     constexpr int CYC = (16 * KJ + 31) & ~31;
     constexpr u32 JROW = (u32)(CYC + 32 * DN) * 4u;
@@ -304,7 +313,7 @@
                 }
             }
             const uint8_t* bseq = p.seq + (size_t)read0 * (NIB ? p.pitch >> 1 : p.pitch);
-            const uint8_t* bcseq = p.cseq + (size_t)read0 * (NIB ? p.pitch >> 1 : p.pitch);
+            const uint8_t* bcseq = EB ? nullptr : p.cseq + (size_t)read0 * (NIB ? p.pitch >> 1 : p.pitch);
             const uint8_t* bqual = p.qual + (size_t)read0 * p.pitch;
             const int total = n * p.cpr;
             u32 carry_code = 20u, carry_char = 0u;
@@ -328,7 +337,10 @@
                     if constexpr (REF) { ch.g0lo = bperm(ag0lo, k); ch.g0hi = bperm(ag0hi, k); }
                 }
                 const u32 rowoff = ch.nb > 0 ? __umul24(ch.off, (u32)p.pitch) + (u32)(16 * ch.jj) : 0u;
-                if constexpr (NIB) {
+                if constexpr (EB) {
+                    const uint2 sv = *reinterpret_cast<const uint2*>(bseq + (rowoff >> 1));
+                    ch.s[0] = sv.x; ch.s[1] = sv.y;
+                } else if constexpr (NIB) {
                     const uint2 sv = *reinterpret_cast<const uint2*>(bseq + (rowoff >> 1));
                     const uint2 cv = *reinterpret_cast<const uint2*>(bcseq + (rowoff >> 1));
                     ch.s[0] = sv.x; ch.s[1] = sv.y; ch.c[0] = cv.x; ch.c[1] = cv.y;
@@ -402,7 +414,13 @@
                 } else {
                     qv[0] = ch.q[0]; qv[1] = ch.q[1]; qv[2] = ch.q[2]; qv[3] = ch.q[3];
                 }
-                if constexpr (NIB) {
+                if constexpr (EB) {
+                    code[0] = nib_lo_code<true>(ch.s[0]); code[1] = nib_hi_code<true>(ch.s[0]);
+                    code[2] = nib_lo_code<true>(ch.s[1]); code[3] = nib_hi_code<true>(ch.s[1]);
+                    xw[0] = ch.s[0] & 0x08080808u; xw[1] = ch.s[0] & 0x80808080u;
+                    xw[2] = ch.s[1] & 0x08080808u; xw[3] = ch.s[1] & 0x80808080u;
+                    badbits = nib_bad<true>(ch.s[0]) | nib_bad<true>(ch.s[1]);
+                } else if constexpr (NIB) {
                     code[0] = nib_lo(ch.s[0]); code[1] = nib_hi(ch.s[0]); code[2] = nib_lo(ch.s[1]); code[3] = nib_hi(ch.s[1]);
                     const u32 x0 = ch.s[0] ^ ch.c[0], x1 = ch.s[1] ^ ch.c[1];
                     xw[0] = nib_lo(x0); xw[1] = nib_hi(x0); xw[2] = nib_lo(x1); xw[3] = nib_hi(x1);
@@ -500,18 +518,27 @@
                     u32 inc_a = 1u, inc_b = 1u;
                     auto fetch_at = [&](K1Chunk& ch, const uint8_t* fseq, const uint8_t* fcseq, const uint8_t* fqual, u32 o) {
                         const uint2 sv = *reinterpret_cast<const uint2*>(fseq + (o >> 1));
-                        const uint2 cv = *reinterpret_cast<const uint2*>(fcseq + (o >> 1));
+                        if constexpr (!EB) {
+                            const uint2 cv = *reinterpret_cast<const uint2*>(fcseq + (o >> 1));
+                            ch.c[0] = cv.x; ch.c[1] = cv.y;
+                        }
                         const uint4 qv = *reinterpret_cast<const uint4*>(fqual + o);
-                        ch.s[0] = sv.x; ch.s[1] = sv.y; ch.c[0] = cv.x; ch.c[1] = cv.y;
+                        ch.s[0] = sv.x; ch.s[1] = sv.y;
                         ch.q[0] = qv.x; ch.q[1] = qv.y; ch.q[2] = qv.z; ch.q[3] = qv.w;
                     };
                     auto fetch_u = [&](K1Chunk& ch, int s) { fetch_at(ch, bseq, bcseq, bqual, at + 1024u * (u32)s); };
                     auto process_u = [&](const K1Chunk& ch) {
                         u32 code[4], code5[4], xw[4], hiq = 0u;
-                        code[0] = nib_lo(ch.s[0]); code[1] = nib_hi(ch.s[0]); code[2] = nib_lo(ch.s[1]); code[3] = nib_hi(ch.s[1]);
-                        const u32 x0 = ch.s[0] ^ ch.c[0], x1 = ch.s[1] ^ ch.c[1];
-                        xw[0] = nib_lo(x0); xw[1] = nib_hi(x0); xw[2] = nib_lo(x1); xw[3] = nib_hi(x1);
-                        const u32 badbits = nib_invalid(ch.s[0]) | nib_invalid(ch.s[1]);
+                        code[0] = nib_lo_code<EB>(ch.s[0]); code[1] = nib_hi_code<EB>(ch.s[0]);
+                        code[2] = nib_lo_code<EB>(ch.s[1]); code[3] = nib_hi_code<EB>(ch.s[1]);
+                        if constexpr (EB) {
+                            xw[0] = ch.s[0] & 0x08080808u; xw[1] = ch.s[0] & 0x80808080u;
+                            xw[2] = ch.s[1] & 0x08080808u; xw[3] = ch.s[1] & 0x80808080u;
+                        } else {
+                            const u32 x0 = ch.s[0] ^ ch.c[0], x1 = ch.s[1] ^ ch.c[1];
+                            xw[0] = nib_lo(x0); xw[1] = nib_hi(x0); xw[2] = nib_lo(x1); xw[3] = nib_hi(x1);
+                        }
+                        const u32 badbits = nib_bad<EB>(ch.s[0]) | nib_bad<EB>(ch.s[1]);
 #pragma unroll
                         for (int wd = 0; wd < 4; ++wd) {
                             code5[wd] = (code[wd] << 2) + code[wd];
@@ -567,7 +594,8 @@
                         k += DK + (wrap ? 1 : 0);
                     };
                     if (fed) {
-                        ua.s[0] = ub.s[0]; ua.s[1] = ub.s[1]; ua.c[0] = ub.c[0]; ua.c[1] = ub.c[1];
+                        ua.s[0] = ub.s[0]; ua.s[1] = ub.s[1];
+                        if constexpr (!EB) { ua.c[0] = ub.c[0]; ua.c[1] = ub.c[1]; }
                         ua.q[0] = ub.q[0]; ua.q[1] = ub.q[1]; ua.q[2] = ub.q[2]; ua.q[3] = ub.q[3];
                     } else {
                         fetch_u(ua, 0);
@@ -583,7 +611,7 @@
                     ahead = ((nblk + 1) << 6) <= seg_hi - seg_lo;
                     const long long nread0 = ahead ? seg_lo + (nblk << 6) : read0;
                     m_next = p.meta[nread0 + lane];
-                    fetch_at(ub, p.seq + (size_t)nread0 * (p.pitch >> 1), p.cseq + (size_t)nread0 * (p.pitch >> 1),
+                    fetch_at(ub, p.seq + (size_t)nread0 * (p.pitch >> 1), EB ? nullptr : p.cseq + (size_t)nread0 * (p.pitch >> 1),
                              p.qual + (size_t)nread0 * p.pitch, at);
                     process_u(ua);
                 }
@@ -618,11 +646,11 @@
     flush_dn(); flush_pos();
 }
 
-template <bool SPLIT, int DN = K1V3_DNREP, bool NIB = false, int KJ = 0>
+template <bool SPLIT, int DN = K1V3_DNREP, bool NIB = false, int KJ = 0, bool EB = false>
 __global__ __launch_bounds__(K1V3_THREADS) void k1v3_accumulate(K1v3Params p)
 {
     extern __shared__ __attribute__((aligned(16))) u32 lds[];
-    k1v3_body<SPLIT, DN, NIB, KJ>(p, lds, (int)blockIdx.x, (int)gridDim.x, (int)blockIdx.y);
+    k1v3_body<SPLIT, DN, NIB, KJ, false, false, EB>(p, lds, (int)blockIdx.x, (int)gridDim.x, (int)blockIdx.y);
 }
 
 template <bool SPLIT, int DN>
@@ -698,7 +726,7 @@
     uint8_t* out; u64* status;
 };
 
-template <bool NIB = false>
+template <bool NIB = false, bool EB = false>
 __global__ __launch_bounds__(K2V3_THREADS) __attribute__((amdgpu_waves_per_eu(K2V3_WAVES, 8))) void k2v3_apply(K2v3Params p)
 {
     extern __shared__ __attribute__((aligned(16))) u32 lds[];
@@ -774,8 +802,9 @@
             const int pos0 = 16 * j;
             u32 code[4], code5[4], badbits = 0u, hiq = 0u;
             if constexpr (NIB) {
-                code[0] = nib_lo(ch.s[0]); code[1] = nib_hi(ch.s[0]); code[2] = nib_lo(ch.s[1]); code[3] = nib_hi(ch.s[1]);
-                badbits = nib_invalid(ch.s[0]) | nib_invalid(ch.s[1]);
+                code[0] = nib_lo_code<EB>(ch.s[0]); code[1] = nib_hi_code<EB>(ch.s[0]);
+                code[2] = nib_lo_code<EB>(ch.s[1]); code[3] = nib_hi_code<EB>(ch.s[1]);
+                badbits = nib_bad<EB>(ch.s[0]) | nib_bad<EB>(ch.s[1]);
             }
 #pragma unroll
             for (int wd = 0; wd < 4; ++wd) {
diff --git a/kbbq-py_amd/csrc/kbbq_layout_kernels.h b/kbbq-py_amd/csrc/kbbq_layout_kernels.h
--- a/kbbq-py_amd/csrc/kbbq_layout_kernels.h
+++ b/kbbq-py_amd/csrc/kbbq_layout_kernels.h
@@ -152,6 +152,7 @@
     long long nrows;
     long long nsrc;
     int pitch, dpitch, S, pairs, nib;
+    int errbit;
     int parts;
     u64* status;
 };
@@ -239,6 +240,21 @@
                 }
             }
             *reinterpret_cast<uint4*>(p.dst[2] + (size_t)d * p.dpitch + (size_t)16 * j) = make_uint4(o[2][0], o[2][1], o[2][2], o[2][3]);
+            if (p.errbit) {
+                u32 bad = 0u, w[2][2];
+#pragma unroll
+                for (int pl = 0; pl < 2; ++pl) {
+                    const u32 c0 = chars_to_codes(o[pl][0], bad), c1 = chars_to_codes(o[pl][1], bad);
+                    const u32 c2 = chars_to_codes(o[pl][2], bad), c3 = chars_to_codes(o[pl][3], bad);
+                    w[pl][0] = c0 | (c1 << 4); w[pl][1] = c2 | (c3 << 4);
+                }
+                if (bad) flag(p.status, ST_LUT, 0);
+                const u32 e0 = (((w[0][0] ^ w[1][0]) & 0x77777777u) + 0x77777777u) & 0x88888888u;
+                const u32 e1 = (((w[0][1] ^ w[1][1]) & 0x77777777u) + 0x77777777u) & 0x88888888u;
+                *reinterpret_cast<uint2*>(p.dst[0] + (size_t)d * (p.dpitch >> 1) + (size_t)8 * j) = make_uint2(w[0][0] | e0, w[0][1] | e1);
+                if (p.dst[1]) *reinterpret_cast<uint2*>(p.dst[1] + (size_t)d * (p.dpitch >> 1) + (size_t)8 * j) = make_uint2(w[1][0], w[1][1]);
+                continue;
+            }
 #pragma unroll
             for (int pl = 0; pl < 2; ++pl) {
                 if (!p.src[pl]) continue;
diff --git a/kbbq-py_amd/kbbq/_device.py b/kbbq-py_amd/kbbq/_device.py
--- a/kbbq-py_amd/kbbq/_device.py
+++ b/kbbq-py_amd/kbbq/_device.py
@@ -183,6 +183,7 @@
 class ReadBatch:
 
     nib = False
+    errbit = False
     seg = None
     perm = None
     tally_qual = None
@@ -273,6 +274,7 @@
 class PairBatch:
 
     nib = False
+    errbit = False
     seg = None
     perm = None
     tally_qual = None
@@ -344,6 +346,8 @@
 def _describe(batch, base):
     if batch.nib:
         base += ', 4-bit sequence planes'
+    if batch.errbit:
+        base += ' with the error bit'
     if batch.seg is not None:
         base += ', rows grouped by read group'
     return base
@@ -387,11 +391,13 @@
     return perm, seg
 
 
-def _lay_out_rows(batch, flags, S2, perm, seg):
+def _lay_out_rows(batch, flags, S2, perm, seg, keep_corrected=True):
     pairs, nib = bool(flags & N.ROWS_PAIRS), bool(flags & N.ROWS_NIBBLES)
+    errbit = bool(flags & N.ROWS_ERRBIT)
     if pairs:
-        laid = PairBatch((batch.n + 1) // 2, S2 // 2, with_corrected=batch.cseq is not None, device=batch.seq.device, nib=nib)
-        laid.read_pitch, laid.twins = batch.pitch, bool(flags & N.ROWS_TWINS)
+        laid = PairBatch((batch.n + 1) // 2, S2 // 2, with_corrected=batch.cseq is not None and (keep_corrected or not errbit),
+                         device=batch.seq.device, nib=nib)
+        laid.read_pitch, laid.twins, laid.errbit = batch.pitch, bool(flags & N.ROWS_TWINS), errbit
     elif isinstance(batch, PairBatch):
         laid = PairBatch(batch.n, batch.S, with_corrected=batch.cseq is not None, device=batch.seq.device, nib=nib)
         laid.read_pitch, laid.twins = batch.read_pitch, batch.twins
@@ -422,7 +428,18 @@
     return (N.ROWS_PAIRS if pairs else 0) | (N.ROWS_NIBBLES if packed else 0) | (N.ROWS_TWINS if twins else 0)
 
 
-def lay_out(batch, R, S=None, packed=True, pairs=None, stats=None):
+ERRBIT_CHUNKS = (19, 13)
+
+
+def errbit_flag(flags, S, corrected, errbit=None):
+    can = (bool(corrected) and (flags & N.ROWS_PAIRS) and (flags & N.ROWS_NIBBLES)
+           and int(N.load().kbbq_pair_pitch(2 * int(S))) // 16 in ERRBIT_CHUNKS)
+    if errbit and not can:
+        raise ValueError('the error bit needs corrected reads on 4-bit mate-pair rows of 2 x 150 or 2 x 100 bp')
+    return N.ROWS_ERRBIT if (can and errbit is not False) else 0
+
+
+def lay_out(batch, R, S=None, packed=True, pairs=None, stats=None, errbit=None, keep_corrected=True):
     if batch.nib or batch.seg is not None or isinstance(batch, PairBatch):
         raise ValueError('lay_out takes input-order rows of characters')
     if batch.n == 0:
@@ -430,6 +447,7 @@
     st = stats or meta_stats(batch)
     S_ = st['longest']
     flags = layout_flags(st, batch.n, batch.pitch, packed, pairs)
+    flags |= errbit_flag(flags, S_, batch.cseq is not None, errbit)
     pairs = bool(flags & N.ROWS_PAIRS)
     perm = seg = None
     if R > 1:
@@ -437,19 +455,20 @@
     if not flags and perm is None:
         return batch
     ctx = context(batch.seq.device.index)
-    laid = _lay_out_rows(batch, flags, 2 * S_, perm, seg)
+    laid = _lay_out_rows(batch, flags, 2 * S_, perm, seg, keep_corrected)
     if packed:
         try:
             ctx.status()
         except N.LutNeedsCheckedApply:
-            if not (flags & ~N.ROWS_NIBBLES) and perm is None:
+            flags &= ~(N.ROWS_NIBBLES | N.ROWS_ERRBIT)
+            if not flags and perm is None:
                 return batch
-            laid = _lay_out_rows(batch, flags & ~N.ROWS_NIBBLES, 2 * S_, perm, seg)
+            laid = _lay_out_rows(batch, flags, 2 * S_, perm, seg)
     return laid
 
 
 def laid_from_reader(text, other, infer_rg_flag, first, n, pitch, R, packed=True, pairs=None, slab=1 << 17, device=None, pair_S=None,
-                     keep_pinned=False, with_out=False):
+                     keep_pinned=False, with_out=False, errbit=None, keep_corrected=True):
     torch = _torch()
     if n == 0:
         return None
@@ -458,6 +477,7 @@
     if pair_S is not None and S_ != pair_S and pairs is None:
         pairs = False
     flags = layout_flags(st, n, pitch, packed, pairs)
+    flags |= errbit_flag(flags, S_, other is not None, errbit)
     two = bool(flags & N.ROWS_PAIRS)
     nrows = (n + 1) // 2 if two else n
     perm = seg = None
@@ -470,16 +490,17 @@
         if not flags and perm is None:
             return None
         nib = bool(flags & N.ROWS_NIBBLES)
+        corrected = other is not None and (keep_corrected or not (flags & N.ROWS_ERRBIT))
         if two:
-            laid = PairBatch(nrows, S_, with_corrected=other is not None, device=device, nib=nib)
-            laid.read_pitch, laid.twins = pitch, bool(flags & N.ROWS_TWINS)
+            laid = PairBatch(nrows, S_, with_corrected=corrected, device=device, nib=nib)
+            laid.read_pitch, laid.twins, laid.errbit = pitch, bool(flags & N.ROWS_TWINS), bool(flags & N.ROWS_ERRBIT)
         else:
-            laid = ReadBatch(n, pitch, with_corrected=other is not None, device=device, nib=nib)
+            laid = ReadBatch(n, pitch, with_corrected=corrected, device=device, nib=nib)
         if with_out:
             laid.out_plane = torch.empty_like(laid.qual)
         dp = laid.pitch
         sp = dp // 2 if nib else dp
-        nseq = 2 if other is not None else 1
+        nseq = 2 if corrected else 1
         step = max(slab // 2 if two else slab, 1)
         row_bytes = nseq * sp + dp + 4
         events, foreign = {}, False
@@ -497,7 +518,7 @@
                     at[0] += cap * width
                     return v
                 h_seq = view(sp)
-                h_cseq = view(sp) if other is not None else None
+                h_cseq = view(sp) if corrected else None
                 h_qual = view(dp)
                 h_meta = buf[at[0]:at[0] + 4 * m].view(torch.int32)
                 foreign |= text.fill_rows(other, first, n, meta, flags, 2 * S_, dp, perm, lo, m, h_seq.numpy(),
@@ -506,7 +527,7 @@
                     break
                 laid.seq[lo:lo + m].copy_(h_seq, non_blocking=True)
                 laid.qual[lo:lo + m].copy_(h_qual, non_blocking=True)
-                if other is not None:
+                if corrected:
                     laid.cseq[lo:lo + m].copy_(h_cseq, non_blocking=True)
                 laid.meta[lo:lo + m].copy_(h_meta, non_blocking=True)
                 events[slot] = torch.cuda.Event()
@@ -517,7 +538,7 @@
             release_pinned('ingest')
         if not foreign:
             break
-        flags &= ~N.ROWS_NIBBLES
+        flags &= ~(N.ROWS_NIBBLES | N.ROWS_ERRBIT)
     laid.h2d_bytes = nrows * row_bytes
     if perm is not None:
         laid.perm = torch.from_numpy(perm).to(laid.seq.device)
@@ -553,7 +574,8 @@
 
 def _row_flags(batch):
     pairs = isinstance(batch, PairBatch)
-    return (N.ROWS_PAIRS if pairs else 0) | (N.ROWS_NIBBLES if batch.nib else 0) | (N.ROWS_TWINS if pairs and batch.twins else 0)
+    return ((N.ROWS_PAIRS if pairs else 0) | (N.ROWS_NIBBLES if batch.nib else 0) | (N.ROWS_TWINS if pairs and batch.twins else 0)
+            | (N.ROWS_ERRBIT if pairs and batch.errbit else 0))
 
 
 LONG_READS = 160
diff --git a/kbbq-py_amd/kbbq/_native.py b/kbbq-py_amd/kbbq/_native.py
--- a/kbbq-py_amd/kbbq/_native.py
+++ b/kbbq-py_amd/kbbq/_native.py
@@ -17,6 +17,7 @@
 APPLY_CHECKED, APPLY_FAST = 0, 1
 ALIGNED_LUT, ALIGNED_F64 = 0, 1
 ROWS_PAIRS, ROWS_NIBBLES, ROWS_TWINS = 1, 2, 4
+ROWS_ERRBIT = 8
 KMER_FIX_N = 1
 KMER_MAX_PASSES = 8
 KMER_FLAG_UNRESOLVED = 2
diff --git a/kbbq-py_amd/kbbq/_stream.py b/kbbq-py_amd/kbbq/_stream.py
--- a/kbbq-py_amd/kbbq/_stream.py
+++ b/kbbq-py_amd/kbbq/_stream.py
@@ -51,7 +51,7 @@
             band = _slab_band(A, B, infer_rg, lo, s_lo, m, longest, shortest, pitch)
             with stage('fill'):
                 laid = dev.laid_from_reader(A, B, infer_rg, lo + s_lo, m, pitch, max(R, 1), packed=longest <= dev.PACKED_READS,
-                                            pair_S=S2 // 2, keep_pinned=True)
+                                            pair_S=S2 // 2, keep_pinned=True, keep_corrected=False)
             try:
                 done = False
                 if laid is not None:
```

Measured after the change: 1232 billion, median of 6. 1.5% higher.
